# N3b3x/openballbot-rl

Hardware: AMD Instinct MI355X
Metric: env-steps/sec at 4096 envs per GPU (flat terrain, random actions) (higher is better)
Workload: dtype f64

## Files before the change

openballbot-rl_amd/ballbot_gym/_native.py:

```python
from __future__ import annotations

import ctypes as C
import os
from pathlib import Path

PKG = Path(__file__).resolve().parent
LIB_PATH = PKG / "_lib" / "libbb_mi355x.so"
CSRC = PKG.parent / "csrc"
INCLUDE = PKG.parent.parent / "include"

NQ, NV, NOBS, HF_N = 17, 15, 15, 293
DONE_TERMINATED, DONE_FAILURE, DONE_DIVERGED, DONE_OVERFLOW = 1, 2, 4, 8
NSTATS = 8
REWARD_DIRECTIONAL, REWARD_DISTANCE, REWARD_NONE = 0, 1, 2
DSBL_PASSIVE, DSBL_GRAVITY = 32, 64


class NativeLibraryError(RuntimeError):
    pass


class BBParams(C.Structure):
    _fields_ = [
        ("max_ep_steps", C.c_int),
        ("max_allowed_tilt", C.c_float),
        ("max_wheel_velocity", C.c_float),
        ("reward_scale", C.c_float),
        ("action_reg_coef", C.c_float),
        ("survival_bonus", C.c_float),
        ("target_dir", C.c_float * 2),
        ("reward_kind", C.c_int),
        ("goal", C.c_float * 2),
        ("goal_scale", C.c_float),
        ("n_terrains", C.c_int),
        ("seed", C.c_uint64),
        ("fp64", C.c_int),
        ("solver_maxiter", C.c_int),
        ("solver_tol", C.c_double),
        ("opt_timestep", C.c_double),
        ("opt_disableflags", C.c_int),
    ]


class PerlinCfg(C.Structure):
    _fields_ = [
        ("scale", C.c_double),
        ("octaves", C.c_int),
        ("persistence", C.c_float),
        ("lacunarity", C.c_float),
        ("amplitude", C.c_double),
    ]


class PPOMlpArgs(C.Structure):
    _fields_ = [(name, C.c_void_p) for name in ("params", "grad", "exp_avg", "exp_avg_sq")] + [
        ("n_params", C.c_int64),
        ("offsets", C.c_int32 * 21),
    ] + [(name, C.c_void_p) for name in ("obs", "actions", "old_logp", "advantages", "returns", "perm",
                                         "mb_counter", "row_counter", "log", "clip", "lr", "step", "coef")] + [
        ("B", C.c_int32),
        ("normalize_advantage", C.c_int32),
        ("obs_dim", C.c_int32),
        ("obs_direct", C.c_int32),
        ("ent_coef", C.c_float),
        ("vf_coef", C.c_float),
    ] + [(name, C.c_double) for name in ("beta1", "beta2", "eps", "weight_decay", "max_grad_norm")] + [
        ("workspace", C.c_void_p),
        ("workspace_bytes", C.c_int64),
        ("phase", C.c_int32),
        ("adv_stats", C.c_void_p),
    ]


class RolloutArgs(C.Structure):
    _fields_ = [
        ("params", C.c_void_p),
        ("offsets", C.c_int32 * 21),
        ("n_params", C.c_int64),
        ("noise", C.c_void_p),
        ("n_steps", C.c_int32),
    ] + [(name, C.c_void_p) for name in ("obs", "last_starts", "ep_ret", "ep_len", "buf_obs", "buf_actions",
                                         "buf_values", "buf_log_prob", "buf_rewards", "buf_starts", "ep_r_out",
                                         "ep_l_out", "buf_terminal_obs", "buf_flags")]


class ViewCfg(C.Structure):
    _fields_ = [
        ("height", C.c_int),
        ("width", C.c_int),
        ("fovy_deg", C.c_float),
        ("azimuth_deg", C.c_float),
        ("elevation_deg", C.c_float),
        ("distance", C.c_float),
        ("lookat_offset", C.c_float * 3),
    ]


ENCODER_FIELDS = ("conv1_w", "conv1_b", "bn1_w", "bn1_b", "bn1_mean", "bn1_var", "bn1_count",
                  "conv2_w", "conv2_b", "bn2_w", "bn2_b", "bn2_mean", "bn2_var", "bn2_count",
                  "fc_w", "fc_b", "bn3_w", "bn3_b", "bn3_mean", "bn3_var", "bn3_count")


class EncoderParams(C.Structure):
    _fields_ = [(name, C.c_void_p) for name in ENCODER_FIELDS]


EXPORTS = [
    "bb_abi_version", "bb_last_error", "bb_default_params", "bb_create", "bb_destroy", "bb_set_hfield",
    "bb_assign_terrain", "bb_reset", "bb_step", "bb_get_state", "bb_set_state", "bb_forward", "bb_get_stats",
    "bb_get_offsets", "bb_get_config", "bb_time_kernel", "bb_kernel_ms", "bb_generate_perlin", "bb_get_hfield",
    "bb_gae", "bb_render_depth", "bb_ppo_loss", "bb_adamw_clip", "bb_ppo_mlp_workspace_bytes", "bb_ppo_mlp_step",
    "bb_ppo_mlp_act", "bb_rollout_track", "bb_depth_encoder_workspace_bytes", "bb_depth_encoder",
    "bb_set_terrain_stream", "bb_get_env_terrain", "bb_kernel_times", "bb_step_multi", "bb_rollout",
    "bb_set_terrain_rng", "bb_get_terrain_rng", "bb_pair_counters", "bb_pair_env_times", "bb_check",
    "bb_reward_terms", "bb_default_view", "bb_render_view", "bb_render_rgbd",
]

ABI_VERSION = 21

_lib = None


HIP_SOURCES = ("bb_kernels.hip", "bb_pair.hip", "bb_terrain.hip", "bb_rollout.hip", "bb_render.hip", "bb_view.hip",
               "bb_rgbd.hip", "bb_ppo.hip", "bb_mlp.hip", "bb_encoder.hip", "bb_episode_log.hip")
SOURCE_FLAGS = {"bb_pair.hip": ["-mllvm", "-disable-machine-licm"]}


def build(force: bool = False, verbose: bool = False) -> Path:
    import subprocess
    from concurrent.futures import ThreadPoolExecutor

    srcs = list(CSRC.glob("*.h")) + list(CSRC.glob("*.hip")) + list(INCLUDE.glob("*.h"))
    if LIB_PATH.exists() and not force and all(LIB_PATH.stat().st_mtime >= s.stat().st_mtime for s in srcs):
        return LIB_PATH
    obj_dir = LIB_PATH.parent / "obj"
    obj_dir.mkdir(parents=True, exist_ok=True)
    flags = ["--offload-arch=gfx950", "-O3", "-std=c++17", "-fPIC"]
    jobs = []
    for f in HIP_SOURCES:
        obj = obj_dir / (f[:-4] + ".o")
        jobs.append((["hipcc", *flags, *SOURCE_FLAGS.get(f, []), "-c", "-o", str(obj), str(CSRC / f)], obj))
    if verbose:
        for cmd, _ in jobs:
            print(" ".join(cmd))

    def run(job):
        return subprocess.run(job[0], capture_output=True, text=True)

    workers = max(1, min(len(jobs), os.cpu_count() or 1, 16))
    with ThreadPoolExecutor(workers) as ex:
        results = list(ex.map(run, jobs))
    for (cmd, _), r in zip(jobs, results):
        if r.returncode != 0:
            raise subprocess.CalledProcessError(r.returncode, cmd, r.stdout, r.stderr + "\n" + " ".join(cmd))
    tmp = LIB_PATH.with_suffix(".so.tmp")
    link = ["hipcc", "--offload-arch=gfx950", "-shared", "-fPIC", "-o", str(tmp), *[str(o) for _, o in jobs]]
    if verbose:
        print(" ".join(link))
    subprocess.run(link, check=True)
    os.replace(tmp, LIB_PATH)
    return LIB_PATH


def lib():
    global _lib
    if _lib is None:
        _lib = _load(LIB_PATH)
    return _lib


def use_diagnostic_library(path) -> None:
    global _lib
    _lib = _load(Path(path))


def _load(path: Path):
    if not path.exists():
        raise NativeLibraryError(
            f"HIP library {path} not found; run __graft_entry__.build() (hipcc --offload-arch=gfx950)")
    try:
        L = C.CDLL(str(path))
    except OSError as e:
        raise NativeLibraryError(f"cannot load {path}: {e}") from e
    vp, fp, dp = C.c_void_p, C.POINTER(C.c_float), C.POINTER(C.c_double)
    L.bb_abi_version.restype = C.c_int
    L.bb_last_error.argtypes = [C.c_char_p, C.c_int]
    L.bb_default_params.argtypes = [C.POINTER(BBParams)]
    L.bb_default_params.restype = None
    L.bb_create.argtypes = [C.c_int, C.c_int, C.POINTER(BBParams), C.POINTER(vp)]
    L.bb_destroy.argtypes = [vp]
    L.bb_set_hfield.argtypes = [vp, C.c_int, fp, C.c_float]
    L.bb_assign_terrain.argtypes = [vp, vp, vp]
    L.bb_reset.argtypes = [vp, vp, vp, vp]
    L.bb_step.argtypes = [vp, vp, vp, vp, vp, vp, vp, C.c_int, vp]
    L.bb_step_multi.argtypes = [vp, vp, C.c_int, vp, vp, vp, vp, vp, C.c_int, vp]
    L.bb_rollout.argtypes = [vp, C.POINTER(RolloutArgs), vp]
    L.bb_reward_terms.argtypes = [vp, vp, vp, C.c_int, vp, C.c_int64, vp, vp]
    L.bb_get_state.argtypes = [vp, dp, dp, dp, C.POINTER(C.c_int32)]
    L.bb_set_state.argtypes = [vp, dp, dp, dp, C.POINTER(C.c_int32)]
    L.bb_forward.argtypes = [vp, dp, dp, C.POINTER(C.c_int32)]
    L.bb_get_stats.argtypes = [vp, C.POINTER(C.c_int64), C.c_int]
    L.bb_pair_counters.argtypes = [vp, C.POINTER(C.c_int64), C.c_int]
    L.bb_pair_env_times.argtypes = [vp, C.POINTER(C.c_uint64)]
    L.bb_check.argtypes = [vp, vp]
    L.bb_set_terrain_stream.argtypes = [vp, C.POINTER(C.c_int32), C.c_int, C.c_int, C.POINTER(C.c_int32)]
    L.bb_set_terrain_rng.argtypes = [vp, C.POINTER(C.c_uint64), C.POINTER(C.c_int32)]
    L.bb_get_terrain_rng.argtypes = [vp, C.POINTER(C.c_uint64), C.POINTER(C.c_int32)]
    L.bb_get_env_terrain.argtypes = [vp, C.POINTER(C.c_int32), C.POINTER(C.c_int32)]
    L.bb_get_offsets.argtypes = [vp, fp]
    L.bb_get_config.argtypes = [vp, C.POINTER(C.c_int32)]
    L.bb_time_kernel.argtypes = [vp, C.c_int]
    L.bb_generate_perlin.argtypes = [vp, C.c_int, C.c_int, C.POINTER(C.c_int32), C.POINTER(PerlinCfg), C.c_float]
    L.bb_get_hfield.argtypes = [vp, C.c_int, fp]
    L.bb_render_depth.argtypes = [vp, vp, vp, C.c_int, C.c_int, C.c_int, C.c_int, vp]
    L.bb_default_view.argtypes = [C.POINTER(ViewCfg)]
    L.bb_default_view.restype = None
    L.bb_render_view.argtypes = [vp, vp, C.c_int, C.POINTER(ViewCfg), vp, vp, vp]
    L.bb_render_rgbd.argtypes = [vp, vp, vp, vp, C.c_int, C.c_int, C.c_int, C.c_int, vp]
    L.bb_ppo_loss.argtypes = [vp] * 8 + [C.c_int, C.c_int, C.c_float, C.c_float, vp, vp, vp, vp]
    L.bb_adamw_clip.argtypes = [vp, vp, vp, vp, C.c_int64, vp, vp, vp] + [C.c_double] * 5 + [vp]
    L.bb_gae.argtypes = [vp, vp, vp, vp, vp, C.c_int, C.c_int, C.c_double, C.c_double, vp, vp, vp]
    L.bb_ppo_mlp_workspace_bytes.argtypes = [C.c_int, C.POINTER(C.c_int64)]
    L.bb_ppo_mlp_step.argtypes = [C.POINTER(PPOMlpArgs), vp]
    L.bb_ppo_mlp_act.argtypes = [vp, C.POINTER(C.c_int32), C.c_int64, vp, C.c_int, vp, C.c_int, vp, vp, vp, vp, vp,
                                 vp]
    L.bb_rollout_track.argtypes = [vp, vp, C.c_int, C.c_int] + [vp] * 8
    L.bb_depth_encoder_workspace_bytes.argtypes = [C.c_int64, C.POINTER(C.c_int64)]
    L.bb_depth_encoder.argtypes = [C.POINTER(EncoderParams), vp, C.c_int64, vp, C.c_int64, C.c_int, C.c_int, C.c_int,
                                   C.c_float, C.c_float, vp, C.c_int64, vp, C.c_int64, vp]
    L.bb_kernel_ms.argtypes = [vp, C.POINTER(C.c_double), C.POINTER(C.c_int32)]
    L.bb_kernel_times.argtypes = [vp, C.POINTER(C.c_double), C.POINTER(C.c_int32)]
    for name in [n for n in EXPORTS if n not in ("bb_default_params", "bb_default_view", "bb_abi_version")]:
        getattr(L, name).restype = C.c_int
    if L.bb_abi_version() != ABI_VERSION:
        raise NativeLibraryError("ABI version mismatch")
    return L


def last_error() -> str:
    buf = C.create_string_buffer(512)
    lib().bb_last_error(buf, 512)
    return buf.value.decode()


def check(rc: int, what: str) -> None:
    if rc != 0:
        raise RuntimeError(f"{what} failed: {last_error()}")


def default_params() -> BBParams:
    p = BBParams()
    lib().bb_default_params(C.byref(p))
    return p
```

openballbot-rl_amd/csrc/bb_kernels.hip:

```cpp
#if defined(BB_FP_CONTRACT_OFF)
#pragma clang fp contract(off)
#elif !defined(BB_FP_CONTRACT_FAST)
#pragma clang fp contract(on)
#endif
#include <hip/hip_runtime.h>

#include <stdarg.h>
#include <stdio.h>
#include <stdlib.h>
#include <string.h>
#include <algorithm>
#include <climits>
#include <vector>

#include "../../include/ballbot_mi355x.h"
#include "bb_model.h"
#include "bb_step.h"
#include "bb_terrain.h"
#include "bb_rollout.h"
#include "bb_episode_log.h"
#include "bb_render.h"
#include "bb_view.h"
#include "bb_rgbd.h"
#include "bb_ppo.h"
#include "bb_mlp.h"
#include "bb_encoder.h"
#include "bb_pairmap.h"

using namespace bb;

#ifdef BB_PHASE_CLOCKS
namespace bb { __device__ unsigned long long bb_phase_cycles[100]; }
#endif

namespace {

constexpr int WAVE = 64;
constexpr int TEAM = 16;
char g_err[512] = "";

int fail(const char* fmt, ...) {
  va_list ap;
  va_start(ap, fmt);
  vsnprintf(g_err, sizeof g_err, fmt, ap);
  va_end(ap);
  return -1;
}
#define HIPCHK(x)                                                                   \
  do {                                                                              \
    hipError_t e_ = (x);                                                            \
    if (e_ != hipSuccess) return fail("%s: %s", #x, hipGetErrorString(e_));         \
  } while (0)

template <typename T>
__host__ __device__ constexpr size_t work_stride() { return (sizeof(EnvWork<T>) + 15) / 16 * 16; }
template <typename T>
size_t lds_bytes(int epw) { return work_stride<T>() * epw; }
template <typename T>
__device__ __forceinline__ EnvWork<T>& team_work(unsigned char* smem, int team) {
  return *reinterpret_cast<EnvWork<T>*>(smem + size_t(team) * work_stride<T>());
}

struct TerrainSrc {
  const int* tstream;
  const int* env_stream;
  int tlen;
  unsigned long long* rng;
  const int* seed_slot;
};

struct Dev {
  int n;
  void* qpos;
  void* qvel;
  void* warm;
  int* steps;
  int* terrain;
  int* pending_terrain;
  int* episodes;
  const struct TerrainSrc* tsrc;
  int* tseed;
  const float* bank;
  const float* size_z;
  const float* offset;
  const float* hmax;
  int n_terrains;
  unsigned long long* stats;
  int* slow_list;
  int* slow_count;
  int* park;
  int* fast_envs;
  int* pred_envs;
  uint8_t* pred_mark;
  void* body_spill;
  void* hand;
  int* perm;
  unsigned long long* ring;
  int* rctr;
  int ring_len;
  unsigned long long* pair_env;
  unsigned long long* pair_busy;
  unsigned long long* cost;
  int* fault;
};

template <typename T>
__device__ __forceinline__ T* body_spill_of(const Dev& d, int e) {
  return reinterpret_cast<T*>(d.body_spill) + size_t(e) * ((MAXB - MAXB_LDS) * NBF);
}

template <typename V>
__device__ __forceinline__ V ld_coh(const V* p) {
  return __hip_atomic_load(p, __ATOMIC_RELAXED, __HIP_MEMORY_SCOPE_AGENT);
}
template <typename V>
__device__ __forceinline__ void st_coh(V* p, V v) {
  __hip_atomic_store(p, v, __ATOMIC_RELAXED, __HIP_MEMORY_SCOPE_AGENT);
}
__device__ __forceinline__ void stores_done() { asm volatile("s_waitcnt vmcnt(0)" ::: "memory"); }

template <typename T, bool COH = false>
__device__ __forceinline__ void load_state(const Dev& d, int e, T* q, T* v, T* w, int& step) {
  const T* Q = (const T*)d.qpos;
  const T* V = (const T*)d.qvel;
  const T* W = (const T*)d.warm;
  if constexpr (COH) {
#pragma unroll
    for (int i = 0; i < NQ; i++) q[i] = ld_coh(Q + i * d.n + e);
#pragma unroll
    for (int i = 0; i < NV; i++) { v[i] = ld_coh(V + i * d.n + e); w[i] = ld_coh(W + i * d.n + e); }
    step = ld_coh(d.steps + e);
  } else {
#pragma unroll
    for (int i = 0; i < NQ; i++) q[i] = Q[i * d.n + e];
#pragma unroll
    for (int i = 0; i < NV; i++) { v[i] = V[i * d.n + e]; w[i] = W[i * d.n + e]; }
    step = d.steps[e];
  }
}
template <typename T, bool COH = false>
__device__ __forceinline__ void store_state(const Dev& d, int e, const T* q, const T* v, const T* w, int step) {
  asm volatile("" : "+v"(e));
  T* Q = (T*)d.qpos;
  T* V = (T*)d.qvel;
  T* W = (T*)d.warm;
  if constexpr (COH) {
#pragma unroll
    for (int i = 0; i < NQ; i++) st_coh(Q + i * d.n + e, q[i]);
#pragma unroll
    for (int i = 0; i < NV; i++) { st_coh(V + i * d.n + e, v[i]); st_coh(W + i * d.n + e, w[i]); }
    st_coh(d.steps + e, step);
  } else {
#pragma unroll
    for (int i = 0; i < NQ; i++) Q[i * d.n + e] = q[i];
#pragma unroll
    for (int i = 0; i < NV; i++) { V[i * d.n + e] = v[i]; W[i * d.n + e] = w[i]; }
    d.steps[e] = step;
  }
}

struct Pcg64 {
  unsigned long long sh, sl, ih, il, buf;
};
constexpr int TERRAIN_SEEDS = 10000;

__device__ __forceinline__ unsigned long long pcg64_next64(Pcg64& g) {
  constexpr unsigned long long MH = 0x2360ED051FC65DA4ull, ML = 0x4385DF649FCCF645ull;
  const unsigned long long lo = g.sl * ML;
  unsigned long long hi = __umul64hi(g.sl, ML) + g.sl * MH + g.sh * ML;
  const unsigned long long lo2 = lo + g.il;
  hi += g.ih + (lo2 < lo ? 1ull : 0ull);
  g.sl = lo2;
  g.sh = hi;
  const unsigned rot = unsigned(hi >> 58);
  const unsigned long long x = hi ^ lo2;
  return (x >> rot) | (x << ((64u - rot) & 63u));
}
__device__ __forceinline__ unsigned pcg64_next32(Pcg64& g) {
  if (g.buf >> 32) {
    const unsigned u = unsigned(g.buf);
    g.buf = u;
    return u;
  }
  const unsigned long long x = pcg64_next64(g);
  g.buf = (1ull << 32) | (x >> 32);
  return unsigned(x);
}
__device__ __forceinline__ int pcg64_terrain_seed(Pcg64& g) {
  constexpr unsigned EXCL = TERRAIN_SEEDS;
  unsigned long long m = (unsigned long long)pcg64_next32(g) * EXCL;
  unsigned left = unsigned(m);
  if (left < EXCL) {
    constexpr unsigned THRESHOLD = (0xFFFFFFFFu - (EXCL - 1u)) % EXCL;
    while (left < THRESHOLD) {
      m = (unsigned long long)pcg64_next32(g) * EXCL;
      left = unsigned(m);
    }
  }
  return int(m >> 32);
}

__device__ __forceinline__ int next_terrain(const Dev& d, int e) {
  const int pin = d.pending_terrain[e];
  if (pin >= 0) return pin;
  const TerrainSrc src = *d.tsrc;
  if (src.rng) {
    const size_t n = size_t(d.n);
    unsigned long long* rng = src.rng;
    Pcg64 g{ld_coh(rng + e), ld_coh(rng + n + e), ld_coh(rng + 2 * n + e), ld_coh(rng + 3 * n + e),
            ld_coh(rng + 4 * n + e)};
    const int s = pcg64_terrain_seed(g);
    st_coh(rng + e, g.sh); st_coh(rng + n + e, g.sl); st_coh(rng + 4 * n + e, g.buf);
    st_coh(d.episodes + e, ld_coh(d.episodes + e) + 1);
    st_coh(d.tseed + e, s);
    int slot = src.seed_slot ? src.seed_slot[s] : s;
    if (unsigned(slot) >= unsigned(d.n_terrains)) {
      atomicAdd(&d.stats[5], 1ull);
      slot = s % d.n_terrains;
    }
    return slot;
  }
  if (!src.tstream) return 0;
  int k = ld_coh(d.episodes + e);
  st_coh(d.episodes + e, k + 1);
  if (k >= src.tlen) {
    atomicAdd(&d.stats[5], 1ull);
    k %= src.tlen;
  }
  const int st = src.env_stream ? src.env_stream[e] : 0;
  return src.tstream[size_t(st) * src.tlen + k];
}

template <typename T>
__device__ __forceinline__ void reset_lane(const ModelT<T>& m, const Dev& d, int e, T* q, T* v, T* w, int& step) {
  const int tid = next_terrain(d, e);
  d.terrain[e] = tid;
  reset_state(m, T(d.offset[tid]), q, v, w);
  step = 0;
}

template <typename T, bool BODY>
__global__ __launch_bounds__(64) void step_kernel(ModelT<T> mg, EnvCfg cfg, Dev d, const float* __restrict__ act,
                                                  float* __restrict__ obs, float* __restrict__ rew,
                                                  uint8_t* __restrict__ done, float* __restrict__ tobs,
                                                  float* __restrict__ pos2d, int auto_reset, int L, int epw,
                                                  const int* __restrict__ elist, const int* __restrict__ ecount) {
  extern __shared__ __align__(16) unsigned char smem[];
  const int nwg = int(gridDim.x), b = int(blockIdx.x);
  int g;
  const int ecnt = elist ? min(*ecount, d.n) : 0;
  if (elist) {
    const int na = (ecnt + epw - 1) / epw, nb = (na + 7) & ~7;
    if (nb > nwg) {
      g = b;
    } else {
      if (b >= nb) return;
      g = (b & 7) * (nb >> 3) + (b >> 3);
    }
    if (g >= na) return;
  } else {
    g = (nwg & 7) ? b : (b & 7) * (nwg >> 3) + (b >> 3);
  }
  __shared__ ModelT<T> ms;
  if (threadIdx.x == 0) ms = mg;
  __syncthreads();
  const ModelT<T>& m = ms;
  const Team tm{L, int(threadIdx.x) & (L - 1)};
  const int team = threadIdx.x / L;
  if (team >= epw) return;
  int e = g * epw + team;
  if (elist) {
    if (e >= ecnt) return;
    e = elist[e];
  }
  if (unsigned(e) >= unsigned(d.n)) return;
  const bool lead = tm.tl == 0;
#ifdef BB_PHASE_CLOCKS
  const unsigned long long t_env0 = clock64();
#endif
  EnvWork<T>& W = team_work<T>(smem, team);
#ifdef BB_PHASE_CLOCKS
  if (lead) W.dbg_nb = 0;
#endif
  if (BODY && lead) W.bspill = body_spill_of<T>(d, e);
  T* q = W.qn;
  T* v = W.vn;
  T* w = W.wn;
  int step;
  load_state(d, e, q, v, w, step);
  float a[3] = {act[3 * e], act[3 * e + 1], act[3 * e + 2]};
  const int tid = d.terrain[e];
  const float* hf = d.bank + size_t(tid) * (HF_N * HF_N);
  float o[15], r, p2[2];
  int iters = 0;
  const TerrainRef<T> tr{hf, T(d.size_z[tid]), T(d.hmax[tid]) * T(d.size_z[tid])};
  int fl = env_step<T, BODY, !BODY>(m, cfg, q, v, w, step, a, tr, W, o, r, p2, &iters, tm);
  if (!BODY && (fl & F_SLOWPATH)) {
    if (lead) {
      const int at = atomicAdd(d.slow_count + 2, 1);
      if (at < d.n) d.slow_list[at] = e;
    }
    return;
  }
  if (!lead) return;
  if (BODY) atomicAdd(&d.stats[3], 1ull);
  if (tobs) {
#pragma unroll
    for (int i = 0; i < 15; i++) tobs[15 * e + i] = o[i];
  }
  if (pos2d) { pos2d[2 * e] = p2[0]; pos2d[2 * e + 1] = p2[1]; }
  const bool reset = auto_reset && (fl & F_TERMINATED);
  if (reset) {
    reset_lane(m, d, e, q, v, w, step);
#pragma unroll
    for (int i = 0; i < 15; i++) o[i] = 0.f;
  }
#pragma unroll
  for (int i = 0; i < 15; i++) obs[15 * e + i] = o[i];
  rew[e] = r;
  done[e] = uint8_t(fl);
  store_state(d, e, q, v, w, step);
  if (reset) atomicAdd(&d.stats[0], 1ull);
  if (fl & F_DIVERGED) atomicAdd(&d.stats[1], 1ull);
  if (fl & F_OVERFLOW) atomicAdd(&d.stats[2], 1ull);
  if (fl & F_SPILL) atomicAdd(&d.stats[6], 1ull);
  atomicAdd(&d.stats[4], (unsigned long long)iters);
#ifdef BB_PHASE_CLOCKS
  {
    const unsigned long long dt = clock64() - t_env0;
    atomicMax(&bb_phase_cycles[BODY ? 34 : 37], dt);
    atomicAdd(&bb_phase_cycles[BODY ? 35 : 38], dt);
    atomicAdd(&bb_phase_cycles[BODY ? 36 : 39], 1ull);
    if (BODY) {
      const int bin = int(dt >> 20) < 9 ? int(dt >> 20) : 9;
      atomicAdd(&bb_phase_cycles[40 + bin], 1ull);
      atomicAdd(&bb_phase_cycles[50 + bin], (unsigned long long)W.dbg_nb);
      atomicAdd(&bb_phase_cycles[60 + bin], (unsigned long long)iters);
      atomicMax(&bb_phase_cycles[70 + bin], (unsigned long long)W.dbg_nb);
    }
  }
#endif
}

#ifndef BB_MULTI_MODE
#define BB_MULTI_MODE 1
#endif
template <typename T>
__device__
#if BB_MULTI_MODE == 0
__noinline__
#else
__forceinline__
#endif
int full_env_step(const ModelT<T>& m, const EnvCfg& cfg, T* q, T* v, T* w, int& step,
                                          const float* a, const TerrainRef<T>& tr, EnvWork<T>& W, float* o,
                                          float& r, float* p2, int* iters, const Team& tm) {
  return env_step<T, true>(m, cfg, q, v, w, step, a, tr, W, o, r, p2, iters, tm);
}

constexpr int F_PARKED = 1 << 17;

constexpr int SC_ROUTE = 8, SC_TOUCHED = 10, ROUTE_PARK = 1;

#ifndef BB_OUT_SKIP
#define BB_OUT_SKIP 0
#endif
template <typename V>
__device__ __forceinline__ void out_st(V* p, V v) {
#ifdef BB_OUT_NT
  __builtin_nontemporal_store(v, p);
#else
  *p = v;
#endif
}

template <typename T, bool HO = true, bool FULLONLY = false, bool FUSE = false>
__device__ __forceinline__ int team_step(const ModelT<T>& m, const EnvCfg& cfg, const Dev& d, int e, int& tid,
                                         T* q, T* v, T* w, int& step, T* bk, const float* a, EnvWork<T>& W, float* o,
                                         float& r, float* tobs_row, float* p2_row, int auto_reset, const Team& tm,
                                         unsigned* cnt, bool full = false) {
  const int L = tm.L;
  const bool lead = tm.tl == 0;
  if constexpr (!FULLONLY) {
    team_sync();
    for (int i = tm.tl; i < NQ + 2 * NV; i += L) bk[i] = q[i];
    team_sync();
  }
  const float* hf = d.bank + size_t(tid) * (HF_N * HF_N);
  float p2[2];
  int iters = 0;
  const TerrainRef<T> tr{hf, T(d.size_z[tid]), T(d.hmax[tid]) * T(d.size_z[tid])};
  const int step0 = step;
  int fl;
#if BB_MULTI_MODE == 2
  fl = F_SLOWPATH;
#else
  if constexpr (FULLONLY) fl = F_SLOWPATH;
  else fl = full ? F_SLOWPATH : env_step<T, false, FUSE>(m, cfg, q, v, w, step, a, tr, W, o, r, p2, &iters, tm);
#endif
  const bool slow = (fl & F_SLOWPATH) != 0;
#if BB_MULTI_MODE == 3
  if (false) {
#else
  if (slow) {
#endif
    if constexpr (!FULLONLY) {
      team_sync();
      for (int i = tm.tl; i < NQ + 2 * NV; i += L) q[i] = bk[i];
      team_sync();
      step = step0;
    }
    if constexpr (!HO) return F_PARKED;
    else fl = full_env_step<T>(m, cfg, q, v, w, step, a, tr, W, o, r, p2, &iters, tm);
  }
  const bool reset = auto_reset && (fl & F_TERMINATED);
  if (lead) {
    cnt[3] += slow;
    if (tobs_row && !(BB_OUT_SKIP & 8)) {
#pragma unroll
      for (int i = 0; i < 15; i++) out_st(tobs_row + i, o[i]);
    }
    if (p2_row && !(BB_OUT_SKIP & 16)) { out_st(p2_row, p2[0]); out_st(p2_row + 1, p2[1]); }
    if (reset) {
      tid = next_terrain(d, e);
      st_coh(d.terrain + e, tid);
    }
  }
  if (reset) {
    tid = __shfl(tid, team_shift_of(L));
    team_sync();
    reset_state(m, T(d.offset[tid]), q, v, w);
    step = 0;
#pragma unroll
    for (int i = 0; i < 15; i++) o[i] = 0.f;
  }
  if (lead) {
    cnt[0] += reset;
    cnt[1] += (fl & F_DIVERGED) != 0;
    cnt[2] += (fl & F_OVERFLOW) != 0;
    cnt[6] += (fl & F_SPILL) != 0;
    cnt[4] += unsigned(iters);
  }
  return fl;
}

__device__ __forceinline__ void counts_clear(unsigned* cnt) {
#pragma unroll
  for (int i = 0; i < 8; i++) cnt[i] = 0u;
}
__device__ __forceinline__ void counts_flush(const Dev& d, const unsigned* cnt) {
#pragma unroll
  for (int i = 0; i < 8; i++)
    if (i != 5 && cnt[i]) atomicAdd(&d.stats[i], (unsigned long long)cnt[i]);
}

#ifdef BB_WPE1
#define BB_WPE __attribute__((amdgpu_waves_per_eu(1, 1)))
#else
#define BB_WPE
#endif
template <typename T, bool HO>
__global__ BB_WPE __launch_bounds__(64) void multi_step_kernel(ModelT<T> mg, EnvCfg cfg, Dev d, const float* __restrict__ act,
                                                        int K, float* __restrict__ obs, float* __restrict__ rew,
                                                        uint8_t* __restrict__ done, float* __restrict__ tobs,
                                                        float* __restrict__ pos2d, int auto_reset, int L, int epw,
                                                        int* __restrict__ park, const int* __restrict__ gate) {
  if (gate && *gate != ROUTE_PARK) return;
  extern __shared__ __align__(16) unsigned char smem[];
  const int nwg = int(gridDim.x), b = int(blockIdx.x);
  const int g = (nwg & 7) ? b : (b & 7) * (nwg >> 3) + (b >> 3);
  __shared__ ModelT<T> ms;
  if (threadIdx.x == 0) ms = mg;
  __syncthreads();
  const ModelT<T>& m = ms;
  const Team tm{L, int(threadIdx.x) & (L - 1)};
  const int team = threadIdx.x / L;
  if (team >= epw) return;
  const int e = g * epw + team;
  if (unsigned(e) >= unsigned(d.n)) return;
  int k0 = 0;
  if (HO && park) {
    k0 = park[e];
    if (k0 >= K) return;
  }
  const bool lead = tm.tl == 0;
  EnvWork<T>& W = team_work<T>(smem, team);
  T* bk = reinterpret_cast<T*>(smem + size_t(epw) * work_stride<T>()) + team * (NQ + 2 * NV);
  __shared__ unsigned s_cnt[WAVE / TEAM][8];
  unsigned* cnt = s_cnt[team];
  if (lead) {
    W.bspill = body_spill_of<T>(d, e);
    counts_clear(cnt);
  }
  T* q = W.qn;
  T* v = W.vn;
  T* w = W.wn;
  int step;
  load_state(d, e, q, v, w, step);
  int tid = d.terrain[e];
  const size_t n = size_t(d.n);
  int parked = K;
#pragma unroll 1
  for (int k = k0; k < K; k++) {
    const size_t row = size_t(k) * n + e;
    const float* ak = act + 3 * row;
    const float a[3] = {ak[0], ak[1], ak[2]};
    float o[15], r;
    const int fl = team_step<T, HO, false, !HO>(m, cfg, d, e, tid, q, v, w, step, bk, a, W, o, r,
                                                tobs ? tobs + 15 * row : nullptr,
                                                pos2d ? pos2d + 2 * row : nullptr, auto_reset, tm, cnt);
    if (!HO && (fl & F_PARKED)) {
      parked = k;
      break;
    }
    if (lead) {
#pragma unroll
      for (int i = 0; i < 15; i++) obs[15 * row + i] = o[i];
      rew[row] = r;
      done[row] = uint8_t(fl);
    }
  }
  team_sync();
  if (lead) {
    store_state(d, e, q, v, w, step);
    counts_flush(d, cnt);
    if (!HO) park[e] = parked;
    if (!HO && gate && parked < K) atomicAdd(d.slow_count + SC_TOUCHED, 1);
  }
}

__device__ __forceinline__ float leaky_f(float z) { return z > 0.f ? z : z * 0.01f; }
__device__ __forceinline__ void team_policy(const float* __restrict__ P, const int* __restrict__ off, const float* x,
                                            float* hA, float* hB, const Team& tm, float mu[3], float& val) {
  constexpr int HIDN = 128, IN = 15;
  const int u0 = 4 * tm.tl;
#pragma unroll 1
  for (int tr = 0; tr < 2; tr++) {
    const int wb = tr ? MLP_VF_W0 : MLP_PI_W0, bb_ = tr ? MLP_VF_B0 : MLP_PI_B0;
    float* hin = hA;
    float* hout = hB;
#pragma unroll 1
    for (int l = 0; l < 4; l++) {
      const float* WT = P + off[wb + l];
      const float* bl = P + off[bb_ + l];
      const float* in = l ? hin : x;
      const int K = l ? HIDN : IN;
      float4 a0 = *reinterpret_cast<const float4*>(bl + u0);
      float4 a1 = *reinterpret_cast<const float4*>(bl + 64 + u0);
#ifdef BB_POLICY_UNROLL
#pragma unroll BB_POLICY_UNROLL
#else
#pragma unroll 8
#endif
      for (int k = 0; k < K; k++) {
        const float hk = in[k];
        const float4 w0 = *reinterpret_cast<const float4*>(WT + k * HIDN + u0);
        const float4 w1 = *reinterpret_cast<const float4*>(WT + k * HIDN + 64 + u0);
        a0.x = fmaf(hk, w0.x, a0.x); a0.y = fmaf(hk, w0.y, a0.y);
        a0.z = fmaf(hk, w0.z, a0.z); a0.w = fmaf(hk, w0.w, a0.w);
        a1.x = fmaf(hk, w1.x, a1.x); a1.y = fmaf(hk, w1.y, a1.y);
        a1.z = fmaf(hk, w1.z, a1.z); a1.w = fmaf(hk, w1.w, a1.w);
      }
      float* out = l ? hout : hin;
      *reinterpret_cast<float4*>(out + u0) = make_float4(leaky_f(a0.x), leaky_f(a0.y), leaky_f(a0.z), leaky_f(a0.w));
      *reinterpret_cast<float4*>(out + 64 + u0) =
          make_float4(leaky_f(a1.x), leaky_f(a1.y), leaky_f(a1.z), leaky_f(a1.w));
      team_sync();
      if (l) { float* t_ = hin; hin = hout; hout = t_; }
    }
    const float4 h0 = *reinterpret_cast<const float4*>(hin + u0);
    const float4 h1 = *reinterpret_cast<const float4*>(hin + 64 + u0);
    auto dot8 = [&](const float* w) {
      const float4 w0 = *reinterpret_cast<const float4*>(w + u0);
      const float4 w1 = *reinterpret_cast<const float4*>(w + 64 + u0);
      float s = 0.f;
      s = fmaf(h0.x, w0.x, s); s = fmaf(h0.y, w0.y, s); s = fmaf(h0.z, w0.z, s); s = fmaf(h0.w, w0.w, s);
      s = fmaf(h1.x, w1.x, s); s = fmaf(h1.y, w1.y, s); s = fmaf(h1.z, w1.z, s); s = fmaf(h1.w, w1.w, s);
      return s;
    };
    if (tr == 0) {
      const float* Wa = P + off[MLP_WA];
#pragma unroll
      for (int c = 0; c < 3; c++) mu[c] = team_sum(tm, dot8(Wa + c * HIDN)) + P[off[MLP_BA] + c];
    } else {
      val = team_sum(tm, dot8(P + off[MLP_WV])) + P[off[MLP_BV]];
    }
    team_sync();
  }
}

struct RolloutCore {
  const float* P;
  int off[MLP_NSLOTS];
  const float* noise;
  int T;
  float* obs;
  uint8_t* last_starts;
  double* ep_ret;
  long long* ep_len;
  float* b_obs;
  float* b_act;
  float* b_val;
  float* b_logp;
  float* b_rew;
  uint8_t* b_starts;
  double* ep_r;
  long long* ep_l;
};
struct RolloutDev : RolloutCore {
  float* b_tobs;
  uint8_t* b_flags;
};
struct RolloutLog {
  float* tobs;
  uint8_t* flags;
};
__device__ __forceinline__ RolloutLog rollout_log_of() { return RolloutLog{nullptr, nullptr}; }
__device__ __forceinline__ RolloutLog rollout_log_of(const RolloutLog& l) { return l; }

template <typename T, bool HO, typename... LG>
__global__ __launch_bounds__(64) void rollout_kernel(ModelT<T> mg, EnvCfg cfg, Dev d, RolloutCore ro, int L, int epw,
                                                     int* __restrict__ park, LG... lg_arg) {
  constexpr bool LOG = sizeof...(LG) != 0;
  const RolloutLog lg = rollout_log_of(lg_arg...);
  extern __shared__ __align__(16) unsigned char smem[];
  const int nwg = int(gridDim.x), b = int(blockIdx.x);
  const int g = (nwg & 7) ? b : (b & 7) * (nwg >> 3) + (b >> 3);
  __shared__ ModelT<T> ms;
  if (threadIdx.x == 0) ms = mg;
  __syncthreads();
  const ModelT<T>& m = ms;
  const Team tm{L, int(threadIdx.x) & (L - 1)};
  const int team = threadIdx.x / L;
  if (team >= epw) return;
  const int e = g * epw + team;
  if (unsigned(e) >= unsigned(d.n)) return;
  int t0 = 0;
  if (HO && park) {
    t0 = park[e];
    if (t0 >= ro.T) return;
  }
  const bool lead = tm.tl == 0;
  EnvWork<T>& W = team_work<T>(smem, team);
  T* bk = reinterpret_cast<T*>(smem + size_t(epw) * work_stride<T>()) + team * (NQ + 2 * NV);
  static_assert(offsetof(EnvWork<T>, bc) == offsetof(EnvWork<T>, g) + sizeof(W.g) &&
                    sizeof(W.g) + sizeof(W.bc) >= 272 * sizeof(float),
                "policy scratch must fit in EnvWork::g + bc");
  float* pol = reinterpret_cast<float*>(W.g);
  float* x = pol;
  float* hA = pol + 16;
  float* hB = pol + 144;
  __shared__ unsigned s_cnt[WAVE / TEAM][8];
  unsigned* cnt = s_cnt[team];
  if (lead) {
    W.bspill = body_spill_of<T>(d, e);
    counts_clear(cnt);
  }
  T* q = W.qn;
  T* v = W.vn;
  T* w = W.wn;
  int step;
  load_state(d, e, q, v, w, step);
  int tid = d.terrain[e];
  const size_t n = size_t(d.n);
  float o[15];
#pragma unroll
  for (int i = 0; i < 15; i++) o[i] = ro.obs[15 * size_t(e) + i];
  uint8_t start = ro.last_starts[e];
  double ret = ro.ep_ret[e];
  long long len = ro.ep_len[e];
  const float* ls = ro.P + ro.off[MLP_LS];
  constexpr float HL2PI = 0.91893853320467274f;
  int parked = ro.T;
#pragma unroll 1
  for (int t = t0; t < ro.T; t++) {
    const size_t row = size_t(t) * n + e;
    team_sync();
    if (tm.tl < 15) x[tm.tl] = o[tm.tl];
    team_sync();
    float mu[3] = {0.f, 0.f, 0.f}, val = 0.f;
#ifndef BB_ROLLOUT_NO_POLICY
    team_policy(ro.P, ro.off, x, hA, hB, tm, mu, val);
#endif
    float a[3], ac[3], lp = 0.f;
#pragma unroll
    for (int j = 0; j < 3; j++) {
      const float ls_j = ls[j];
      a[j] = __fadd_rn(mu[j], __fmul_rn(ro.noise[3 * row + j], expf(ls_j)));
      const float z = __fmul_rn(__fsub_rn(a[j], mu[j]), expf(-ls_j));
      lp += -0.5f * z * z - ls_j - 0.5f * (2.f * HL2PI);
      ac[j] = fminf(fmaxf(a[j], -1.f), 1.f);
    }
    if (lead) {
#pragma unroll
      for (int i = 0; i < 15; i++) ro.b_obs[15 * row + i] = o[i];
#pragma unroll
      for (int j = 0; j < 3; j++) ro.b_act[3 * row + j] = a[j];
      ro.b_val[row] = val;
      ro.b_logp[row] = lp;
      ro.b_starts[row] = start;
    }
    float r, o_prev[15];
    if (!HO) {
#pragma unroll
      for (int i = 0; i < 15; i++) o_prev[i] = o[i];
    }
    const int fl = team_step<T, HO>(m, cfg, d, e, tid, q, v, w, step, bk, ac, W, o, r,
                                    LOG ? lg.tobs + 15 * row : nullptr, nullptr, 1, tm, cnt);
    if (!HO && (fl & F_PARKED)) {
#pragma unroll
      for (int i = 0; i < 15; i++) o[i] = o_prev[i];
      parked = t;
      break;
    }
    const bool dn = (fl & F_TERMINATED) != 0;
    ret += double(r);
    len += 1;
    if (lead) {
      ro.b_rew[row] = r;
      ro.ep_r[row] = dn ? ret : __builtin_nan("");
      ro.ep_l[row] = dn ? len : 0;
      if constexpr (LOG) lg.flags[row] = uint8_t(fl);
    }
    ret = dn ? 0.0 : ret;
    len = dn ? 0 : len;
    start = dn ? 1 : 0;
  }
  team_sync();
  if (lead) {
    store_state(d, e, q, v, w, step);
    counts_flush(d, cnt);
    if (!HO) park[e] = parked;
#pragma unroll
    for (int i = 0; i < 15; i++) ro.obs[15 * size_t(e) + i] = o[i];
    ro.last_starts[e] = start;
    ro.ep_ret[e] = ret;
    ro.ep_len[e] = len;
  }
}

template <typename T>
__global__ __launch_bounds__(64) void reset_kernel(ModelT<T> m, Dev d, const uint8_t* mask, float* obs) {
  const int e = blockIdx.x * WAVE + threadIdx.x;
  if (!mask && e == 0 && d.fault) __hip_atomic_store(d.fault, 0, __ATOMIC_RELAXED, __HIP_MEMORY_SCOPE_SYSTEM);
  if (e >= d.n) return;
  if (mask && !mask[e]) return;
  T q[NQ], v[NV], w[NV];
  int step;
  reset_lane(m, d, e, q, v, w, step);
  store_state(d, e, q, v, w, step);
  if (obs) {
#pragma unroll
    for (int i = 0; i < 15; i++) obs[15 * e + i] = 0.f;
  }
}

template <typename T>
__global__ __launch_bounds__(64) void forward_kernel(ModelT<T> mg, Dev d, const double* ctrl, double* qacc, int* ncon,
                                                     int L, int epw) {
  extern __shared__ __align__(16) unsigned char smem[];
  __shared__ ModelT<T> ms;
  if (threadIdx.x == 0) ms = mg;
  __syncthreads();
  const ModelT<T>& m = ms;
  const Team tm{L, int(threadIdx.x) & (L - 1)};
  const int team = threadIdx.x / L;
  if (team >= epw) return;
  const int e = blockIdx.x * epw + team;
  if (e >= d.n) return;
  EnvWork<T>& W = team_work<T>(smem, team);
  if (tm.tl == 0) W.bspill = body_spill_of<T>(d, e);
  T q[NQ], v[NV], w[NV], c[3];
  int step;
  load_state(d, e, q, v, w, step);
  for (int i = 0; i < 3; i++) c[i] = T(ctrl[3 * e + i]);
  const int tid = d.terrain[e];
  StageOut<T> so;
// ... 2032 lines not shown
```

openballbot-rl_amd/csrc/bb_physics.h:

```cpp
#pragma once

#include <hip/hip_runtime.h>
#include <math.h>
#include <stdint.h>

#define BB_HD __host__ __device__ __forceinline__

namespace bb {

constexpr int NQ = 17, NV = 15, NU = 3;
constexpr int HF_N = 293;
constexpr int MAXG = 50;
constexpr int NH = NV * (NV + 1) / 2;
constexpr int NGF = 4;
constexpr int MAXPAIR = 50;
constexpr int MAXB = 3 + 6 * MAXPAIR;
constexpr int MAXB_LDS = 32;
constexpr int NBF = 8;
constexpr int GF_N = 0, GF_DIST = 3;
constexpr int BF_N = 0, BF_P = 3, BF_DIST = 6, BF_CODE = 7;

constexpr double IMPR_GRAD = 1e6;

template <typename T>
struct ModelT {
  T m0, h0[3], I0O[6];
  T mw, cw[3], Iw[6];
  T gz[3];
  T wq[3][4];
  T axis[3];
  T u[3][3];
  T jpos[3];
  T anchor[3];
  T wheel_r, wheel_hh, armature, damping;
  T mB, IB, ball_r, dz;
  T tower_c[3], tower_r, tower_hh;
  T stick_c[2][3], stick_a[2][3], stick_r, stick_hh;
  T iw_ball, iw_wheel[3];
  T iw_base, iw_cam[2];
  T K, Bd;
  T solimp[5];
  T fr_wheel[2];
  T h, grav;
  T hf_sx, hf_sy, hf_bottom;
  T scale, tol, ls_tol, step_rel2;
  int maxiter, ls_maxiter;
  T qpos0[NQ];
};

template <typename T> BB_HD T dot3(const T* a, const T* b) { return a[0] * b[0] + a[1] * b[1] + a[2] * b[2]; }
template <typename T> BB_HD void cross3(T* r, const T* a, const T* b) {
  T x = a[1] * b[2] - a[2] * b[1], y = a[2] * b[0] - a[0] * b[2], z = a[0] * b[1] - a[1] * b[0];
  r[0] = x; r[1] = y; r[2] = z;
}
template <typename T>
BB_HD T hinge_sel(int w, const T* x) {
  using U = typename std::conditional<sizeof(T) == 8, unsigned long long, unsigned int>::type;
  const U m0 = U(0) - U(w == 0), m1 = U(0) - U(w == 1), m2 = U(0) - U(w == 2);
  const U b = (__builtin_bit_cast(U, x[6]) & m0) | (__builtin_bit_cast(U, x[7]) & m1) | (__builtin_bit_cast(U, x[8]) & m2);
  return __builtin_bit_cast(T, b);
}

template <typename T> BB_HD void mv3(T* r, const T* M, const T* v) {
  T x = M[0] * v[0] + M[1] * v[1] + M[2] * v[2];
  T y = M[3] * v[0] + M[4] * v[1] + M[5] * v[2];
  T z = M[6] * v[0] + M[7] * v[1] + M[8] * v[2];
  r[0] = x; r[1] = y; r[2] = z;
}
template <typename T> BB_HD void mtv3(T* r, const T* M, const T* v) {
  T x = M[0] * v[0] + M[3] * v[1] + M[6] * v[2];
  T y = M[1] * v[0] + M[4] * v[1] + M[7] * v[2];
  T z = M[2] * v[0] + M[5] * v[1] + M[8] * v[2];
  r[0] = x; r[1] = y; r[2] = z;
}
template <typename T> BB_HD void mm3(T* r, const T* A, const T* B) {
  T t[9];
#pragma unroll
  for (int i = 0; i < 3; i++)
#pragma unroll
    for (int j = 0; j < 3; j++) t[3 * i + j] = A[3 * i] * B[j] + A[3 * i + 1] * B[3 + j] + A[3 * i + 2] * B[6 + j];
#pragma unroll
  for (int i = 0; i < 9; i++) r[i] = t[i];
}
template <typename T> BB_HD void symv(T* r, const T* S, const T* v) {
  T x = S[0] * v[0] + S[3] * v[1] + S[4] * v[2];
  T y = S[3] * v[0] + S[1] * v[1] + S[5] * v[2];
  T z = S[4] * v[0] + S[5] * v[1] + S[2] * v[2];
  r[0] = x; r[1] = y; r[2] = z;
}
template <typename T> BB_HD void sym_rot(T* out, const T* R, const T* S) {
  T F[9] = {S[0], S[3], S[4], S[3], S[1], S[5], S[4], S[5], S[2]};
  T A[9], B[9];
  mm3(A, R, F);
#pragma unroll
  for (int i = 0; i < 3; i++)
#pragma unroll
    for (int j = 0; j < 3; j++) B[3 * i + j] = A[3 * i] * R[3 * j] + A[3 * i + 1] * R[3 * j + 1] + A[3 * i + 2] * R[3 * j + 2];
  out[0] = B[0]; out[1] = B[4]; out[2] = B[8]; out[3] = B[1]; out[4] = B[2]; out[5] = B[5];
}
template <typename T> BB_HD T clampT(T x, T lo, T hi) { return x < lo ? lo : (x > hi ? hi : x); }
template <typename T> BB_HD T maxT(T a, T b) { return a > b ? a : b; }
template <typename T> BB_HD T rsqrtT(T x) {
#ifdef __HIP_DEVICE_COMPILE__
  return rsqrt(x);
#else
  return T(1) / sqrt(x);
#endif
}
template <typename T> BB_HD T minT(T a, T b) { return a < b ? a : b; }
template <typename T> BB_HD T rsqrt_ls(T x) {
#ifdef __HIP_DEVICE_COMPILE__
  if constexpr (sizeof(T) == 8) {
    const double r = __builtin_amdgcn_rsq(x);
    return r * fma(-0.5 * x * r, r, 1.5);
  } else {
    return __builtin_amdgcn_rsqf(x);
  }
#else
  return T(1) / sqrt(x);
#endif
}
template <typename T> BB_HD T div_ls(T a, T b) {
#ifdef __HIP_DEVICE_COMPILE__
  if constexpr (sizeof(T) == 8) {
    double r = __builtin_amdgcn_rcp(b);
    r = fma(r, fma(-b, r, 1.0), r);
    return a * r;
  } else {
    return a * __builtin_amdgcn_rcpf(b);
  }
#else
  return a / b;
#endif
}

template <typename T> BB_HD void qmul(T* r, const T* a, const T* b) {
  T w = a[0] * b[0] - a[1] * b[1] - a[2] * b[2] - a[3] * b[3];
  T x = a[0] * b[1] + a[1] * b[0] + a[2] * b[3] - a[3] * b[2];
  T y = a[0] * b[2] - a[1] * b[3] + a[2] * b[0] + a[3] * b[1];
  T z = a[0] * b[3] + a[1] * b[2] - a[2] * b[1] + a[3] * b[0];
  r[0] = w; r[1] = x; r[2] = y; r[3] = z;
}
template <typename T> BB_HD void qnormalize(T* q) {
  T n = sqrt(q[0] * q[0] + q[1] * q[1] + q[2] * q[2] + q[3] * q[3]);
  if (n < T(1e-15)) { q[0] = 1; q[1] = q[2] = q[3] = 0; return; }
  T inv = T(1) / n;
  q[0] *= inv; q[1] *= inv; q[2] *= inv; q[3] *= inv;
}
template <typename T> BB_HD void q2mat(T* m, const T* q) {
  T q00 = q[0] * q[0], q01 = q[0] * q[1], q02 = q[0] * q[2], q03 = q[0] * q[3];
  T q11 = q[1] * q[1], q12 = q[1] * q[2], q13 = q[1] * q[3];
  T q22 = q[2] * q[2], q23 = q[2] * q[3], q33 = q[3] * q[3];
  m[0] = q00 + q11 - q22 - q33; m[4] = q00 - q11 + q22 - q33; m[8] = q00 - q11 - q22 + q33;
  m[1] = 2 * (q12 - q03); m[2] = 2 * (q13 + q02); m[3] = 2 * (q12 + q03);
  m[5] = 2 * (q23 - q01); m[6] = 2 * (q13 - q02); m[7] = 2 * (q23 + q01);
}
template <typename T> BB_HD void quat_integrate(T* q, const T* w, T h) {
  T n = sqrt(dot3(w, w));
  T qr[4] = {1, 0, 0, 0};
  if (n >= T(1e-15)) {
    T ang = h * n, s = sin(ang * T(0.5)) / n;
    qr[0] = cos(ang * T(0.5)); qr[1] = w[0] * s; qr[2] = w[1] * s; qr[3] = w[2] * s;
  }
  qnormalize(q);
  qmul(q, q, qr);
}
template <typename T> BB_HD void integrate_pos(T* q, const T* v, T h) {
  q[0] += h * v[0]; q[1] += h * v[1]; q[2] += h * v[2];
  quat_integrate(q + 3, v + 3, h);
  q[7] += h * v[6]; q[8] += h * v[7]; q[9] += h * v[8];
  q[10] += h * v[9]; q[11] += h * v[10]; q[12] += h * v[11];
  quat_integrate(q + 13, v + 12, h);
}

constexpr BB_HD int hidx(int i, int j) { return i >= j ? i * (i + 1) / 2 + j : j * (j + 1) / 2 + i; }

template <typename T>
struct Kin {
  T Rb[9], RB[9];
  T pb[3], pB[3];
  T c[3];
  T wc[3][3];
  T Rw[3][9];
};

template <typename T>
BB_HD void kinematics_base(const ModelT<T>& m, const T* q, Kin<T>& k) {
  T qb[4] = {q[3], q[4], q[5], q[6]};
  qnormalize(qb);
  q2mat(k.Rb, qb);
  T qB[4] = {q[13], q[14], q[15], q[16]};
  qnormalize(qB);
  q2mat(k.RB, qB);
  k.pb[0] = q[0]; k.pb[1] = q[1]; k.pb[2] = q[2];
  k.pB[0] = q[10]; k.pB[1] = q[11]; k.pB[2] = q[12];
  k.c[0] = k.pB[0] + k.RB[2] * m.dz;
  k.c[1] = k.pB[1] + k.RB[5] * m.dz;
  k.c[2] = k.pB[2] + k.RB[8] * m.dz;
}

template <typename T>
BB_HD void kinematics_wheel(const ModelT<T>& m, const T* q, int w, Kin<T>& k) {
  T th = q[7 + w] - m.qpos0[7 + w];
  T s = sin(th * T(0.5)), cth = cos(th * T(0.5));
  T ql[4] = {cth, m.axis[0] * s, m.axis[1] * s, m.axis[2] * s};
  T qw[4];
  qmul(qw, m.wq[w], ql);
  qnormalize(qw);
  q2mat(k.Rw[w], qw);
  T d[3] = {m.cw[0] - m.jpos[0], m.cw[1] - m.jpos[1], m.cw[2] - m.jpos[2]};
  T t[3];
  mv3(t, k.Rw[w], d);
  k.wc[w][0] = m.anchor[0] + t[0];
  k.wc[w][1] = m.anchor[1] + t[1];
  k.wc[w][2] = m.anchor[2] + t[2];
}

template <typename T>
BB_HD void kinematics(const ModelT<T>& m, const T* q, Kin<T>& k) {
  kinematics_base(m, q, k);
#pragma unroll
  for (int w = 0; w < 3; w++) kinematics_wheel(m, q, w, k);
}

template <typename T>
struct Mass {
  T mt;
  T mr[3];
  T Mtr[9];
  T Mrr[6];
  T Mth[3][3];
  T Mrh[3][3];
  T Mhh[3];
  T mB;
  T MBtr[9];
  T MBrr[3];
};

template <typename T>
BB_HD void mass_wheel(const ModelT<T>& m, const Kin<T>& k, int w, Mass<T>& M, T* Iw, T* mrw, T* IOw) {
  const T* c = k.wc[w];
  sym_rot(Iw, k.Rw[w], m.Iw);
  mrw[0] = m.mw * c[0]; mrw[1] = m.mw * c[1]; mrw[2] = m.mw * c[2];
  T cc = dot3(c, c);
  IOw[0] = Iw[0] + m.mw * (cc - c[0] * c[0]);
  IOw[1] = Iw[1] + m.mw * (cc - c[1] * c[1]);
  IOw[2] = Iw[2] + m.mw * (cc - c[2] * c[2]);
  IOw[3] = Iw[3] - m.mw * c[0] * c[1];
  IOw[4] = Iw[4] - m.mw * c[0] * c[2];
  IOw[5] = Iw[5] - m.mw * c[1] * c[2];
  const T* u = m.u[w];
  T ca[3] = {c[0] - m.anchor[0], c[1] - m.anchor[1], c[2] - m.anchor[2]};
  T vc[3];
  cross3(vc, u, ca);
  T p[3] = {m.mw * vc[0], m.mw * vc[1], m.mw * vc[2]};
  T L[3], t[3];
  symv(L, Iw, u);
  T uIu = dot3(u, L);
  cross3(t, c, p);
  L[0] += t[0]; L[1] += t[1]; L[2] += t[2];
  mv3(M.Mth[w], k.Rb, p);
  M.Mrh[w][0] = L[0]; M.Mrh[w][1] = L[1]; M.Mrh[w][2] = L[2];
  M.Mhh[w] = uIu + m.mw * dot3(vc, vc) + m.armature;
}

template <typename T>
BB_HD void mass_finish(const ModelT<T>& m, const Kin<T>& k, Mass<T>& M, const T (*mrw)[3], const T (*IOw)[6]) {
  T mr[3] = {m.h0[0], m.h0[1], m.h0[2]};
  T IO[6] = {m.I0O[0], m.I0O[1], m.I0O[2], m.I0O[3], m.I0O[4], m.I0O[5]};
#pragma unroll
  for (int w = 0; w < 3; w++) {
#pragma unroll
    for (int i = 0; i < 3; i++) mr[i] += mrw[w][i];
#pragma unroll
    for (int i = 0; i < 6; i++) IO[i] += IOw[w][i];
  }
  M.mt = m.m0 + 3 * m.mw;
  M.mr[0] = mr[0]; M.mr[1] = mr[1]; M.mr[2] = mr[2];
  T S[9] = {0, mr[2], -mr[1], -mr[2], 0, mr[0], mr[1], -mr[0], 0};
  mm3(M.Mtr, k.Rb, S);
#pragma unroll
  for (int i = 0; i < 6; i++) M.Mrr[i] = IO[i];
  const T dz = m.dz;
  M.mB = m.mB;
  T SB[9] = {0, m.mB * dz, 0, -m.mB * dz, 0, 0, 0, 0, 0};
  mm3(M.MBtr, k.RB, SB);
  M.MBrr[0] = m.IB + m.mB * dz * dz;
  M.MBrr[1] = m.IB + m.mB * dz * dz;
  M.MBrr[2] = m.IB;
}

template <typename T>
BB_HD void build_mass(const ModelT<T>& m, const Kin<T>& k, Mass<T>& M, T (&Iw)[3][6]) {
  T mrw[3][3], IOw[3][6];
#pragma unroll
  for (int w = 0; w < 3; w++) mass_wheel(m, k, w, M, Iw[w], mrw[w], IOw[w]);
  mass_finish(m, k, M, mrw, IOw);
}

template <typename T>
BB_HD void mass_mul(const Mass<T>& M, const T* x, T* y) {
  T t[3], r[3];
  mv3(t, M.Mtr, x + 3);
  y[0] = M.mt * x[0] + t[0];
  y[1] = M.mt * x[1] + t[1];
  y[2] = M.mt * x[2] + t[2];
  mtv3(t, M.Mtr, x);
  symv(r, M.Mrr, x + 3);
  y[3] = t[0] + r[0]; y[4] = t[1] + r[1]; y[5] = t[2] + r[2];
#pragma unroll
  for (int w = 0; w < 3; w++) {
    T xh = x[6 + w];
#pragma unroll
    for (int i = 0; i < 3; i++) { y[i] += M.Mth[w][i] * xh; y[3 + i] += M.Mrh[w][i] * xh; }
    y[6 + w] = dot3(M.Mth[w], x) + dot3(M.Mrh[w], x + 3) + M.Mhh[w] * xh;
  }
  mv3(t, M.MBtr, x + 12);
  y[9] = M.mB * x[9] + t[0];
  y[10] = M.mB * x[10] + t[1];
  y[11] = M.mB * x[11] + t[2];
  mtv3(t, M.MBtr, x + 9);
  y[12] = t[0] + M.MBrr[0] * x[12];
  y[13] = t[1] + M.MBrr[1] * x[13];
  y[14] = t[2] + M.MBrr[2] * x[14];
}

template <typename T>
BB_HD void mass_dense(const Mass<T>& M, T* H) {
#pragma unroll
  for (int i = 0; i < NH; i++) H[i] = 0;
#pragma unroll
  for (int i = 0; i < 3; i++) {
    H[hidx(i, i)] = M.mt;
#pragma unroll
    for (int j = 0; j < 3; j++) H[hidx(3 + i, j)] = M.Mtr[3 * j + i];
  }
  H[hidx(3, 3)] = M.Mrr[0]; H[hidx(4, 4)] = M.Mrr[1]; H[hidx(5, 5)] = M.Mrr[2];
  H[hidx(4, 3)] = M.Mrr[3]; H[hidx(5, 3)] = M.Mrr[4]; H[hidx(5, 4)] = M.Mrr[5];
#pragma unroll
  for (int w = 0; w < 3; w++) {
#pragma unroll
    for (int j = 0; j < 3; j++) { H[hidx(6 + w, j)] = M.Mth[w][j]; H[hidx(6 + w, 3 + j)] = M.Mrh[w][j]; }
    H[hidx(6 + w, 6 + w)] = M.Mhh[w];
  }
#pragma unroll
  for (int i = 0; i < 3; i++) {
    H[hidx(9 + i, 9 + i)] = M.mB;
#pragma unroll
    for (int j = 0; j < 3; j++) H[hidx(12 + i, 9 + j)] = M.MBtr[3 * j + i];
    H[hidx(12 + i, 12 + i)] = M.MBrr[i];
  }
}

template <typename T>
BB_HD void inertia_apply(T m, const T* c, const T* Ic, const T* w, const T* v, T* L, T* p) {
  T t[3];
  cross3(t, w, c);
  p[0] = m * (v[0] + t[0]); p[1] = m * (v[1] + t[1]); p[2] = m * (v[2] + t[2]);
  symv(L, Ic, w);
  cross3(t, c, p);
  L[0] += t[0]; L[1] += t[1]; L[2] += t[2];
}
template <typename T>
BB_HD void body_force(T m, const T* c, const T* Ic, const T* Aw, const T* Av, const T* Vw, const T* Vv,
                      T* fa, T* fl) {
  T La[3], pa[3], Lv[3], pv[3], t[3];
  inertia_apply(m, c, Ic, Aw, Av, La, pa);
  inertia_apply(m, c, Ic, Vw, Vv, Lv, pv);
  cross3(t, Vw, Lv); fa[0] = La[0] + t[0]; fa[1] = La[1] + t[1]; fa[2] = La[2] + t[2];
  cross3(t, Vv, pv); fa[0] += t[0]; fa[1] += t[1]; fa[2] += t[2];
  cross3(t, Vw, pv); fl[0] = pa[0] + t[0]; fl[1] = pa[1] + t[1]; fl[2] = pa[2] + t[2];
}

template <typename T>
BB_HD void bias_base_motion(const ModelT<T>& m, const Kin<T>& k, const T* v, T* w0, T* vl, T* a0) {
  w0[0] = v[3]; w0[1] = v[4]; w0[2] = v[5];
  mtv3(vl, k.Rb, v);
  T t[3];
  cross3(t, vl, w0);
  a0[0] = m.grav * k.Rb[6] + t[0];
  a0[1] = m.grav * k.Rb[7] + t[1];
  a0[2] = m.grav * k.Rb[8] + t[2];
}

template <typename T>
BB_HD T bias_wheel(const ModelT<T>& m, const Kin<T>& k, const T* Iw, const T* v, int w, const T* w0, const T* vl,
                   const T* a0, T* fa, T* fl) {
  const T* u = m.u[w];
  T au[3];
  cross3(au, m.anchor, u);
  T qd = v[6 + w];
  T Vw[3] = {w0[0] + qd * u[0], w0[1] + qd * u[1], w0[2] + qd * u[2]};
  T Vv[3] = {vl[0] + qd * au[0], vl[1] + qd * au[1], vl[2] + qd * au[2]};
  T x1[3], x2[3], x3[3];
  cross3(x1, w0, u);
  cross3(x2, w0, au);
  cross3(x3, vl, u);
  T Aw[3] = {qd * x1[0], qd * x1[1], qd * x1[2]};
  T Av[3] = {a0[0] + qd * (x2[0] + x3[0]), a0[1] + qd * (x2[1] + x3[1]), a0[2] + qd * (x2[2] + x3[2])};
  body_force(m.mw, k.wc[w], Iw, Aw, Av, Vw, Vv, fa, fl);
  return dot3(u, fa) + dot3(au, fl);
}

template <typename T>
BB_HD void bias_finish(const ModelT<T>& m, const Kin<T>& k, const T* v, const T (*fw)[6], T* bias) {
  T w0[3], vl[3], a0[3], t[3];
  bias_base_motion(m, k, v, w0, vl, a0);
  const T zero[3] = {0, 0, 0};
  T Fa[3], Fl[3];
  {
    T c0[3] = {m.h0[0] / m.m0, m.h0[1] / m.m0, m.h0[2] / m.m0};
    T cc = dot3(c0, c0);
    T Ic[6] = {m.I0O[0] - m.m0 * (cc - c0[0] * c0[0]), m.I0O[1] - m.m0 * (cc - c0[1] * c0[1]),
               m.I0O[2] - m.m0 * (cc - c0[2] * c0[2]), m.I0O[3] + m.m0 * c0[0] * c0[1],
               m.I0O[4] + m.m0 * c0[0] * c0[2], m.I0O[5] + m.m0 * c0[1] * c0[2]};
    body_force(m.m0, c0, Ic, zero, a0, w0, vl, Fa, Fl);
  }
#pragma unroll
  for (int w = 0; w < 3; w++) {
    Fa[0] += fw[w][0]; Fa[1] += fw[w][1]; Fa[2] += fw[w][2];
    Fl[0] += fw[w][3]; Fl[1] += fw[w][4]; Fl[2] += fw[w][5];
  }
  mv3(bias, k.Rb, Fl);
  bias[3] = Fa[0]; bias[4] = Fa[1]; bias[5] = Fa[2];
  T wB[3] = {v[12], v[13], v[14]};
  T vB[3];
  mtv3(vB, k.RB, v + 9);
  cross3(t, vB, wB);
  T aB[3] = {m.grav * k.RB[6] + t[0], m.grav * k.RB[7] + t[1], m.grav * k.RB[8] + t[2]};
  T cB[3] = {0, 0, m.dz};
  T IcB[6] = {m.IB, m.IB, m.IB, 0, 0, 0};
  T fa[3], fl[3];
  body_force(m.mB, cB, IcB, zero, aB, wB, vB, fa, fl);
  mv3(bias + 9, k.RB, fl);
  bias[12] = fa[0]; bias[13] = fa[1]; bias[14] = fa[2];
}

template <typename T>
BB_HD void bias_forces(const ModelT<T>& m, const Kin<T>& k, const T (&Iw)[3][6], const T* v, T* bias) {
  T w0[3], vl[3], a0[3], fw[3][6];
  bias_base_motion(m, k, v, w0, vl, a0);
#pragma unroll
  for (int w = 0; w < 3; w++) bias[6 + w] = bias_wheel(m, k, Iw[w], v, w, w0, vl, a0, fw[w], fw[w] + 3);
  bias_finish(m, k, v, fw, bias);
}

template <typename T>
BB_HD T impedance(const ModelT<T>& m, T pos) {
  T x = pos / m.solimp[2];
  if (x < 0) x = -x;
  if (x >= T(1) || x <= T(0)) return x >= T(1) ? m.solimp[1] : m.solimp[0];
  T y;
  const T mid = m.solimp[3];
  if (x <= mid) y = x * x / mid;
  else y = T(1) - (T(1) - x) * (T(1) - x) / (T(1) - mid);
  return m.solimp[0] + y * (m.solimp[1] - m.solimp[0]);
}

template <typename T>
BB_HD void frame_from_normal(const T* n, T* t1, T* t2) {
  T y[3] = {0, 0, 0};
  if (fabs(n[1]) < T(0.5)) y[1] = 1; else y[2] = 1;
  T d = dot3(n, y);
  t1[0] = y[0] - d * n[0]; t1[1] = y[1] - d * n[1]; t1[2] = y[2] - d * n[2];
  T inv = rsqrtT(dot3(t1, t1));
  t1[0] *= inv; t1[1] *= inv; t1[2] *= inv;
  cross3(t2, n, t1);
}

template <typename T>
BB_HD void cone_eval(const T* jar, T mu, T f1, T f2, const T* D, T* force, T* C) {
  T U0 = jar[0] * mu, U1 = jar[1] * f1, U2 = jar[2] * f2;
  T N = U0, Tn = sqrt(U1 * U1 + U2 * U2);
  if (N >= mu * Tn || (Tn <= 0 && N >= 0)) {
    force[0] = force[1] = force[2] = 0;
    if (C) { C[0] = C[1] = C[2] = C[3] = C[4] = C[5] = 0; }
  } else if (mu * N + Tn <= 0 || (Tn <= 0 && N < 0)) {
    force[0] = -D[0] * jar[0]; force[1] = -D[1] * jar[1]; force[2] = -D[2] * jar[2];
    if (C) { C[0] = D[0]; C[1] = D[1]; C[2] = D[2]; C[3] = C[4] = C[5] = 0; }
  } else {
    T Dm = D[0] / (mu * mu * (1 + mu * mu));
    T g = N - mu * Tn;
    T iT = T(1) / Tn;
    T gr[3] = {mu, -mu * f1 * U1 * iT, -mu * f2 * U2 * iT};
    T s = -Dm * g;
    force[0] = s * gr[0]; force[1] = s * gr[1]; force[2] = s * gr[2];
    if (C) {
      T k = Dm * g * (-mu) * iT;
      T iT2 = iT * iT;
      C[0] = Dm * gr[0] * gr[0];
      C[1] = Dm * gr[1] * gr[1] + k * f1 * f1 * (T(1) - U1 * U1 * iT2);
      C[2] = Dm * gr[2] * gr[2] + k * f2 * f2 * (T(1) - U2 * U2 * iT2);
      C[3] = Dm * gr[0] * gr[1];
      C[4] = Dm * gr[0] * gr[2];
      C[5] = Dm * gr[1] * gr[2] - k * f1 * f2 * U1 * U2 * iT2;
    }
  }
}

template <typename T>
struct WheelCon {
  T J[3][13];
  T aref[3], D[3];
};

BB_HD constexpr int wheel_col(int i, int w) { return i < 6 ? i : (i == 6 ? 6 + w : i + 2); }

template <typename T>
struct GStore {
  T* base;
  int stride;
  BB_HD T& at(int s, int f) const { return base[(s * NGF + f) * stride]; }
};

template <typename T>
BB_HD void wheel_contact(const ModelT<T>& m, const Kin<T>& k, const T* v, int w, WheelCon<T>& C) {
  T t[3], gp[3], ax[3], axl[3];
  mv3(t, k.Rb, k.wc[w]);
  gp[0] = k.pb[0] + t[0]; gp[1] = k.pb[1] + t[1]; gp[2] = k.pb[2] + t[2];
  mv3(axl, k.Rw[w], m.gz);
  mv3(ax, k.Rb, axl);
  T vec[3] = {k.c[0] - gp[0], k.c[1] - gp[1], k.c[2] - gp[2]};
  T x = clampT(dot3(ax, vec), -m.wheel_hh, m.wheel_hh);
  T dif[3] = {gp[0] + ax[0] * x - k.c[0], gp[1] + ax[1] * x - k.c[1], gp[2] + ax[2] * x - k.c[2]};
  T cd = sqrt(dot3(dif, dif));
  T dist = cd - m.ball_r - m.wheel_r;
  const T act = dist <= 0 ? T(1) : T(0);
  T n[3];
  if (cd > 0) { T ic = T(1) / cd; n[0] = dif[0] * ic; n[1] = dif[1] * ic; n[2] = dif[2] * ic; }
  else { n[0] = 1; n[1] = 0; n[2] = 0; }
  T dn = dot3(n, ax);
  T t1[3] = {ax[0] - dn * n[0], ax[1] - dn * n[1], ax[2] - dn * n[2]};
  T it1 = T(1) / sqrt(dot3(t1, t1));
  t1[0] *= it1; t1[1] *= it1; t1[2] *= it1;
  T t2[3];
  cross3(t2, n, t1);
  T pos[3];
  T sp = m.ball_r + dist * T(0.5);
  pos[0] = k.c[0] + n[0] * sp; pos[1] = k.c[1] + n[1] * sp; pos[2] = k.c[2] + n[2] * sp;
  T lb[3] = {pos[0] - k.pb[0], pos[1] - k.pb[1], pos[2] - k.pb[2]};
  mv3(t, k.Rb, m.anchor);
  T la[3] = {lb[0] - t[0], lb[1] - t[1], lb[2] - t[2]};
  T lB[3] = {pos[0] - k.pB[0], pos[1] - k.pB[1], pos[2] - k.pB[2]};
  T uw[3];
  mv3(uw, k.Rb, m.u[w]);
#pragma unroll
  for (int r = 0; r < 3; r++) {
    const T* d = r == 0 ? n : (r == 1 ? t1 : t2);
    T x1[3], br[3];
    C.J[r][0] = d[0]; C.J[r][1] = d[1]; C.J[r][2] = d[2];
    cross3(x1, lb, d);
    mtv3(br, k.Rb, x1);
    C.J[r][3] = br[0]; C.J[r][4] = br[1]; C.J[r][5] = br[2];
    cross3(x1, la, d);
    C.J[r][6] = dot3(uw, x1);
    C.J[r][7] = -d[0]; C.J[r][8] = -d[1]; C.J[r][9] = -d[2];
    cross3(x1, lB, d);
    mtv3(t, k.RB, x1);
    C.J[r][10] = -t[0]; C.J[r][11] = -t[1]; C.J[r][12] = -t[2];
  }
  T imp = clampT(impedance(m, dist), T(0.0001), T(0.9999));
  T tran = m.iw_ball + m.iw_wheel[w];
  T R0 = maxT(T(1e-15), (1 - imp) * tran / imp);
  T rr = m.fr_wheel[0] / m.fr_wheel[1];
  T R2 = R0 * rr * rr;
  C.D[0] = act / R0; C.D[1] = act / R0; C.D[2] = act / R2;
#pragma unroll
  for (int r = 0; r < 3; r++) {
    T vel = 0;
#pragma unroll
    for (int i = 0; i < 13; i++) vel += C.J[r][i] * v[wheel_col(i, w)];
    C.aref[r] = (C.D[0] > 0 ? T(1) : T(0)) * (-m.Bd * vel - (r == 0 ? m.K * imp * dist : T(0)));
  }
}

template <typename T>
BB_HD T wheel_row_mul(const WheelCon<T>& C, int w, int r, const T* x) {
  T acc = 0;
#pragma unroll
  for (int i = 0; i < 13; i++) acc += C.J[r][i] * x[wheel_col(i, w)];
  return acc;
}

template <typename T>
BB_HD void closest_pt_tri(T* res, const T* p, const T* a, const T* b, const T* c) {
  T ab[3] = {b[0] - a[0], b[1] - a[1], b[2] - a[2]};
  T ac[3] = {c[0] - a[0], c[1] - a[1], c[2] - a[2]};
  T ap[3] = {p[0] - a[0], p[1] - a[1], p[2] - a[2]};
  T d1 = dot3(ab, ap), d2 = dot3(ac, ap);
  if (d1 <= 0 && d2 <= 0) { res[0] = a[0]; res[1] = a[1]; res[2] = a[2]; return; }
  T bp[3] = {p[0] - b[0], p[1] - b[1], p[2] - b[2]};
  T d3 = dot3(ab, bp), d4 = dot3(ac, bp);
  if (d3 >= 0 && d4 <= d3) { res[0] = b[0]; res[1] = b[1]; res[2] = b[2]; return; }
  T vc = d1 * d4 - d3 * d2;
  if (vc <= 0 && d1 >= 0 && d3 <= 0) {
    T vv = d1 / (d1 - d3);
    res[0] = a[0] + vv * ab[0]; res[1] = a[1] + vv * ab[1]; res[2] = a[2] + vv * ab[2];
    return;
  }
  T cp[3] = {p[0] - c[0], p[1] - c[1], p[2] - c[2]};
  T d5 = dot3(ab, cp), d6 = dot3(ac, cp);
  if (d6 >= 0 && d5 <= d6) { res[0] = c[0]; res[1] = c[1]; res[2] = c[2]; return; }
  T vb = d5 * d2 - d1 * d6;
  if (vb <= 0 && d2 >= 0 && d6 <= 0) {
    T ww = d2 / (d2 - d6);
    res[0] = a[0] + ww * ac[0]; res[1] = a[1] + ww * ac[1]; res[2] = a[2] + ww * ac[2];
    return;
  }
  T va = d3 * d6 - d5 * d4;
  if (va <= 0 && (d4 - d3) >= 0 && (d5 - d6) >= 0) {
    T ww = (d4 - d3) / ((d4 - d3) + (d5 - d6));
    res[0] = b[0] + ww * (c[0] - b[0]); res[1] = b[1] + ww * (c[1] - b[1]); res[2] = b[2] + ww * (c[2] - b[2]);
    return;
  }
  T den = T(1) / (va + vb + vc), vv = vb * den, ww = vc * den;
  res[0] = a[0] + ab[0] * vv + ac[0] * ww;
  res[1] = a[1] + ab[1] * vv + ac[1] * ww;
  res[2] = a[2] + ab[2] * vv + ac[2] * ww;
}

template <typename T>
BB_HD bool sphere_prism(const T* c, T r, const T V[3][3], T zb, T* n, T* dist) {
  T zmax = maxT(V[0][2], maxT(V[1][2], V[2][2]));
  T q[3];
  if (c[2] >= zmax) {
    closest_pt_tri(q, c, V[0], V[1], V[2]);
  } else {
    T area = (V[1][0] - V[0][0]) * (V[2][1] - V[0][1]) - (V[2][0] - V[0][0]) * (V[1][1] - V[0][1]);
    T sg = area > 0 ? T(1) : T(-1);
    bool inside = c[2] >= zb;
    T edist[3], eo[3][2];
#pragma unroll
    for (int i = 0; i < 3; i++) {
      const T* P = V[i];
      const T* Q = V[(i + 1) % 3];
      T ex = Q[0] - P[0], ey = Q[1] - P[1];
      T cr = ex * (c[1] - P[1]) - ey * (c[0] - P[0]);
      if (cr * sg < 0) inside = false;
      T nx = ey * sg, ny = -ex * sg, nl = sqrt(nx * nx + ny * ny);
      eo[i][0] = nx / nl; eo[i][1] = ny / nl;
      edist[i] = fabs(cr) / nl;
    }
    T e1[3] = {V[1][0] - V[0][0], V[1][1] - V[0][1], V[1][2] - V[0][2]};
    T e2[3] = {V[2][0] - V[0][0], V[2][1] - V[0][1], V[2][2] - V[0][2]};
    T nt[3];
    cross3(nt, e1, e2);
    if (nt[2] < 0) { nt[0] = -nt[0]; nt[1] = -nt[1]; nt[2] = -nt[2]; }
    T inl = T(1) / sqrt(dot3(nt, nt));
    nt[0] *= inl; nt[1] *= inl; nt[2] *= inl;
    T dtop = dot3(nt, V[0]) - dot3(nt, c);
    if (inside && dtop >= 0) {
      T best = dtop;
      n[0] = nt[0]; n[1] = nt[1]; n[2] = nt[2];
      if (c[2] - zb < best) { best = c[2] - zb; n[0] = 0; n[1] = 0; n[2] = -1; }
#pragma unroll
      for (int i = 0; i < 3; i++)
        if (edist[i] < best) { best = edist[i]; n[0] = eo[i][0]; n[1] = eo[i][1]; n[2] = 0; }
      *dist = -best - r;
      return true;
    }
    T B[3][3] = {{V[0][0], V[0][1], zb}, {V[1][0], V[1][1], zb}, {V[2][0], V[2][1], zb}};
    T best = T(1e30);
#pragma unroll
    for (int f = 0; f < 8; f++) {
      const T* a;
      const T* b;
      const T* cc;
      switch (f) {
        case 0: a = V[0]; b = V[1]; cc = V[2]; break;
        case 1: a = B[0]; b = B[1]; cc = B[2]; break;
        case 2: a = V[0]; b = V[1]; cc = B[1]; break;
        case 3: a = V[0]; b = B[1]; cc = B[0]; break;
        case 4: a = V[1]; b = V[2]; cc = B[2]; break;
        case 5: a = V[1]; b = B[2]; cc = B[1]; break;
        case 6: a = V[2]; b = V[0]; cc = B[0]; break;
        default: a = V[2]; b = B[0]; cc = B[2]; break;
      }
      T qq[3];
      closest_pt_tri(qq, c, a, b, cc);
      T dd[3] = {c[0] - qq[0], c[1] - qq[1], c[2] - qq[2]};
      T d2 = dot3(dd, dd);
      if (d2 < best) { best = d2; q[0] = qq[0]; q[1] = qq[1]; q[2] = qq[2]; }
    }
  }
  T dd[3] = {c[0] - q[0], c[1] - q[1], c[2] - q[2]};
  T d = sqrt(dot3(dd, dd));
  if (d > r) return false;
  if (d > T(1e-12)) { T id = T(1) / d; n[0] = dd[0] * id; n[1] = dd[1] * id; n[2] = dd[2] * id; }
  else {
    T e1[3] = {V[1][0] - V[0][0], V[1][1] - V[0][1], V[1][2] - V[0][2]};
    T e2[3] = {V[2][0] - V[0][0], V[2][1] - V[0][1], V[2][2] - V[0][2]};
    cross3(n, e1, e2);
    if (n[2] < 0) { n[0] = -n[0]; n[1] = -n[1]; n[2] = -n[2]; }
    T inl = T(1) / sqrt(dot3(n, n));
    n[0] *= inl; n[1] *= inl; n[2] *= inl;
  }
  *dist = d - r;
  return true;
}

template <typename T>
BB_HD void ground_contact(const ModelT<T>& m, const T* gc, const T* RB, const T* v, T (&J)[3][6], T (&aref)[3],
                          T& D) {
  const T n[3] = {gc[GF_N], gc[GF_N + 1], gc[GF_N + 2]};
  const T dist = gc[GF_DIST];
  const T sp = m.ball_r + dist * T(0.5);
  const T lv[3] = {m.dz * RB[2] - n[0] * sp, m.dz * RB[5] - n[1] * sp, m.dz * RB[8] - n[2] * sp};
  T t1[3], t2[3];
  frame_from_normal(n, t1, t2);
  const T* F[3] = {n, t1, t2};
#pragma unroll
  for (int r = 0; r < 3; r++) {
    T x1[3], x2[3];
    cross3(x1, lv, F[r]);
    mtv3(x2, RB, x1);
#pragma unroll
    for (int i = 0; i < 3; i++) { J[r][i] = F[r][i]; J[r][3 + i] = x2[i]; }
  }
  const T imp = clampT(impedance(m, dist), T(0.0001), T(0.9999));
  D = minT(T(1e15), imp / ((1 - imp) * m.iw_ball));
#pragma unroll
  for (int r = 0; r < 3; r++) {
    const T vel = J[r][0] * v[9] + J[r][1] * v[10] + J[r][2] * v[11] + J[r][3] * v[12] + J[r][4] * v[13] +
                  J[r][5] * v[14];
    aref[r] = -m.Bd * vel - (r == 0 ? m.K * imp * dist : T(0));
  }
}

template <typename T>
struct Poses {
  T Rb[9], pb[3], RB[9], pB[3];
};

template <typename T>
struct BodyFrame {
  T F[3][3], db[3], dB[3], hw[3], aref[3], D, ball;
  int hinge;
};

template <typename T>
BB_HD void body_V(const BodyFrame<T>& b, const Poses<T>& P, const T* x, T (&V)[3]) {
  T om[3], wx[3];
  mv3(om, P.Rb, x + 3);
  cross3(wx, om, b.db);
  const T xh = b.hinge >= 0 ? hinge_sel(b.hinge, x) : T(0);
  T ob[3], bx[3];
  mv3(ob, P.RB, x + 12);
  cross3(bx, ob, b.dB);
#pragma unroll
  for (int i = 0; i < 3; i++) V[i] = x[i] + wx[i] + b.hw[i] * xh - b.ball * (x[9 + i] + bx[i]);
}

template <typename T>
BB_HD void body_frame(const ModelT<T>& m, const T* bc, const Poses<T>& P, const T* v, BodyFrame<T>& b) {
  const int code = int(bc[BF_CODE]);
  const int b1 = code >> 3, b2 = code & 7;
  const T n[3] = {bc[BF_N], bc[BF_N + 1], bc[BF_N + 2]};
  const T dist = bc[BF_DIST];
  T t1[3], t2[3];
  frame_from_normal(n, t1, t2);
#pragma unroll
  for (int i = 0; i < 3; i++) {
    b.F[0][i] = n[i]; b.F[1][i] = t1[i]; b.F[2][i] = t2[i];
    b.db[i] = bc[BF_P + i] - P.pb[i];
    b.dB[i] = bc[BF_P + i] - P.pB[i];
    b.hw[i] = 0;
  }
  b.hinge = (b2 >= 4 && b2 <= 6) ? b2 - 4 : -1;
  if (b.hinge >= 0) {
    T uw[3], t[3], da[3];
    mv3(uw, P.Rb, m.u[b.hinge]);
    mv3(t, P.Rb, m.anchor);
    da[0] = b.db[0] - t[0]; da[1] = b.db[1] - t[1]; da[2] = b.db[2] - t[2];
    cross3(b.hw, uw, da);
  }
  b.ball = b1 == 7 ? T(1) : T(0);
  const T iw2 = b2 == 1 ? m.iw_base : (b2 <= 3 ? m.iw_cam[b2 - 2] : m.iw_wheel[b2 - 4]);
  const T tran = iw2 + (b1 == 7 ? m.iw_ball : T(0));
  const T imp = clampT(impedance(m, dist), T(0.0001), T(0.9999));
  b.D = T(1) / maxT(T(1e-15), (1 - imp) * tran / imp);
  T V[3];
  body_V(b, P, v, V);
#pragma unroll
  for (int r = 0; r < 3; r++) b.aref[r] = -m.Bd * dot3(b.F[r], V) - (r == 0 ? m.K * imp * dist : T(0));
}

template <typename T>
BB_HD void body_ls_terms(const ModelT<T>& m, const T* bc, const Poses<T>& P, const T* v, const T* a, const T* s,
                         T (&c6)[6], T& D) {
  BodyFrame<T> b;
  body_frame(m, bc, P, v, b);
  T Va[3], Vs[3];
  body_V(b, P, a, Va);
  body_V(b, P, s, Vs);
#pragma unroll
  for (int r = 0; r < 3; r++) {
    c6[r] = dot3(b.F[r], Va) - b.aref[r];
    c6[3 + r] = dot3(b.F[r], Vs);
  }
  D = b.D;
}

template <typename T>
BB_HD int collide_ground(const ModelT<T>& m, const Kin<T>& k, const T* v, const float* hf, T size_z,
                         const GStore<T>& st, int* overflow) {
  const T r = m.ball_r;
  const T* c = k.c;
  const T sx = m.hf_sx, sy = m.hf_sy, zb = m.hf_bottom;
  T xmin = c[0] - r, xmax = c[0] + r, ymin = c[1] - r, ymax = c[1] + r, zmin = c[2] - r, zmax = c[2] + r;
  if (!(xmin <= sx && xmax >= -sx && ymin <= sy && ymax >= -sy && zmin <= size_z && zmax >= -zb)) return 0;
  const int N1 = HF_N - 1;
  int cmin = (int)floor((xmin + sx) / (2 * sx) * N1);
  int cmax = (int)ceil((xmax + sx) / (2 * sx) * N1);
  int rmin = (int)floor((ymin + sy) / (2 * sy) * N1);
  int rmax = (int)ceil((ymax + sy) / (2 * sy) * N1);
  cmin = cmin < 0 ? 0 : cmin;
  cmax = cmax > N1 ? N1 : cmax;
  rmin = rmin < 0 ? 0 : rmin;
  rmax = rmax > N1 ? N1 : rmax;
  const T dx = 2 * sx / N1, dy = 2 * sy / N1;
  (void)v;
  int ng = 0;
  for (int rr = rmin; rr < rmax; rr++) {
    T W[3][3] = {{0, 0, 0}, {0, 0, 0}, {0, 0, 0}};
    int nvert = 0;
    const T y0 = dy * rr - sy, y1 = dy * (rr + 1) - sy;
    for (int cc = cmin; cc <= cmax; cc++) {
      const T x = dx * cc - sx;
      const T z0 = T(hf[rr * HF_N + cc]) * size_z;
      const T z1 = T(hf[(rr + 1) * HF_N + cc]) * size_z;
#pragma unroll
      for (int i = 0; i < 2; i++) {
#pragma unroll
        for (int j = 0; j < 3; j++) { W[0][j] = W[1][j]; W[1][j] = W[2][j]; }
        W[2][0] = x; W[2][1] = i ? y1 : y0; W[2][2] = i ? z1 : z0;
        nvert++;
        if (nvert <= 2) continue;
        if (W[0][2] < zmin && W[1][2] < zmin && W[2][2] < zmin) continue;
        T bx0 = minT(W[0][0], minT(W[1][0], W[2][0])), bx1 = maxT(W[0][0], maxT(W[1][0], W[2][0]));
        T by0 = minT(W[0][1], minT(W[1][1], W[2][1])), by1 = maxT(W[0][1], maxT(W[1][1], W[2][1]));
        T ztop = maxT(W[0][2], maxT(W[1][2], W[2][2]));
        T ex = maxT(T(0), maxT(bx0 - c[0], c[0] - bx1));
        T ey = maxT(T(0), maxT(by0 - c[1], c[1] - by1));
        T ez = maxT(T(0), c[2] - ztop);
        if (ex * ex + ey * ey + ez * ez > r * r) continue;
        T nn[3], dist;
        if (!sphere_prism(c, r, W, -zb, nn, &dist)) continue;
        if (ng >= MAXG) { *overflow = 1; continue; }
#pragma unroll
        for (int i = 0; i < 3; i++) st.at(ng, GF_N + i) = nn[i];
        st.at(ng, GF_DIST) = dist;
        ng++;
      }
    }
  }
  return ng;
}

template <typename T> BB_HD T eps_of();
template <> BB_HD float eps_of<float>() { return 1.1920929e-7f; }
template <> BB_HD double eps_of<double>() { return 2.220446049250313e-16; }
template <typename T> BB_HD T pivot_eps();
template <> BB_HD float pivot_eps<float>() { return 1e-6f; }
template <> BB_HD double pivot_eps<double>() { return 1e-14; }

template <typename T>
BB_HD void chol_packed(T* H) {
// ... 36 lines not shown
```

openballbot-rl_amd/csrc/bb_step.h:

```cpp
#pragma once

#include "bb_team16.h"

namespace bb {

struct EnvCfg {
  int max_ep_steps;
  float max_allowed_tilt;
  float max_wheel_velocity;
  float reward_scale;
  float action_reg_coef;
  float survival_bonus;
  float target[2];
  int reward_kind;
  float goal[2], goal_scale;
};

template <typename T, bool BODY = true, bool FUSE = false>
BB_HD int forward(const ModelT<T>& m, const T* q, const T* v, const T* ctrl, T* acc, const TerrainRef<T>& tr,
                  EnvWork<T>& W, StageOut<T>* so, const Team& tm) {
  team_sync();
  if (v != W.vi) {
#pragma unroll
    for (int i = 0; i < NV; i++) W.vi[i] = v[i];
    team_sync();
  }
#if defined(BB_PHASE_CLOCKS) && defined(__HIP_DEVICE_COMPILE__)
  const unsigned long long f_t0 = clock64();
#endif
  Kin<T>& k = W.u.pre.k;
#ifdef __HIP_DEVICE_COMPILE__
  kinematics_base(m, q, k);
  if (tm.tl < 3) kinematics_wheel(m, q, tm.tl, k);
  team_sync();
#else
  kinematics(m, q, k);
#endif
  Mass<T>& M = W.M;
#ifdef __HIP_DEVICE_COMPILE__
  {
    T (*mrw)[3] = reinterpret_cast<T (*)[3]>(W.H);
    T (*IOw)[6] = reinterpret_cast<T (*)[6]>(W.H + 9);
    T (*fw)[6] = reinterpret_cast<T (*)[6]>(W.H + 27);
    static_assert(NH >= 45, "per-wheel terms do not fit W.H");
    if (tm.tl < 3) {
      const int w = tm.tl;
      mass_wheel(m, k, w, M, W.u.pre.Iw[w], mrw[w], IOw[w]);
      T w0[3], vl[3], a0[3];
      bias_base_motion(m, k, v, w0, vl, a0);
      const T qb = -bias_wheel(m, k, W.u.pre.Iw[w], v, w, w0, vl, a0, fw[w], fw[w] + 3);
      const T cw = w == 0 ? ctrl[0] : (w == 1 ? ctrl[1] : ctrl[2]);
      W.qfs[6 + w] = qb + (-m.damping * v[6 + w] + cw);
      wheel_contact(m, k, v, w, W.wc[w]);
    }
    team_sync();
    mass_finish(m, k, M, mrw, IOw);
    T qfs[NV];
    bias_finish(m, k, v, fw, qfs);
#pragma unroll
    for (int i = 0; i < NV; i++)
      if (i < 6 || i > 8) W.qfs[i] = -qfs[i];
    team_sync();
  }
#else
  build_mass(m, k, M, W.u.pre.Iw);
  {
    T qfs[NV];
    bias_forces(m, k, W.u.pre.Iw, v, qfs);
#pragma unroll
    for (int i = 0; i < NV; i++) qfs[i] = -qfs[i];
#pragma unroll
    for (int w = 0; w < 3; w++) qfs[6 + w] += -m.damping * v[6 + w] + ctrl[w];
#pragma unroll
    for (int i = 0; i < NV; i++) W.qfs[i] = qfs[i];
  }
#pragma unroll
  for (int w = 0; w < 3; w++) wheel_contact(m, k, v, w, W.wc[w]);
#endif
  const GStore<T> st{W.g, 1};
  int overflow = 0;
#if defined(BB_PHASE_CLOCKS) && defined(__HIP_DEVICE_COMPILE__)
  const unsigned long long f_t1 = clock64();
#endif
#ifdef __HIP_DEVICE_COMPILE__
  const int ng = tr.hf ? t16::collide_team(m, k, v, tr.hf, tr.size_z, W.g, &overflow, tm.tl) : 0;
  int nb = 0;
  if constexpr (BODY) {
#if defined(BB_PHASE_CLOCKS)
    const unsigned long long b_t0 = clock64();
#endif
    static_assert(sizeof(W.H) >= t16::CAND_CAP * sizeof(int), "candidate list does not fit W.H");
#ifdef BB_EXP_DUP_BODYCOL
    { int ov2 = 0; (void)t16::collide_body_team(m, k, tr.hf, tr.size_z, tr.hz, W.bc, W.bspill, &ov2, tm.tl,
                                                 reinterpret_cast<int*>(W.H)); }
    asm volatile("" ::: "memory");
#endif
    nb = t16::collide_body_team(m, k, tr.hf, tr.size_z, tr.hz, W.bc, W.bspill, &overflow, tm.tl,
                                reinterpret_cast<int*>(W.H));
#if defined(BB_PHASE_CLOCKS)
    if (tm.tl == 0) {
      atomicAdd(&bb_phase_cycles[12], 1ull);
      atomicAdd(&bb_phase_cycles[13], (unsigned long long)nb);
      atomicAdd(&bb_phase_cycles[14], clock64() - b_t0);
      W.dbg_nb += nb;
    }
#endif
  } else {
    if (t16::body_candidates(m, k, tr.hf, tr.size_z, tr.hz, tm.tl)) return -1;
  }
#else
  const int ng = tr.hf ? collide_ground(m, k, v, tr.hf, tr.size_z, st, &overflow) : 0;
#endif
#if defined(BB_PHASE_CLOCKS) && defined(__HIP_DEVICE_COMPILE__)
  if (tm.tl == 0) {
    const unsigned long long f_t2 = clock64();
    atomicAdd(&bb_phase_cycles[8], f_t1 - f_t0);
    atomicAdd(&bb_phase_cycles[9], f_t2 - f_t1);
    atomicAdd(&bb_phase_cycles[10], 1ull);
  }
#endif
#pragma unroll
  for (int i = 0; i < 9; i++) { W.P.Rb[i] = k.Rb[i]; W.P.RB[i] = k.RB[i]; }
#pragma unroll
  for (int i = 0; i < 3; i++) { W.P.pb[i] = k.pb[i]; W.P.pB[i] = k.pB[i]; }
  if (so) {
    T qb[4] = {q[3], q[4], q[5], q[6]};
    qnormalize(qb);
    so->quat_b[0] = qb[0]; so->quat_b[1] = qb[1]; so->quat_b[2] = qb[2]; so->quat_b[3] = qb[3];
    mv3(so->w_world, k.Rb, v + 3);
    T cl[3] = {M.mr[0] / M.mt, M.mr[1] / M.mt, M.mr[2] / M.mt}, cw[3], t[3];
    mv3(cw, k.Rb, cl);
    cross3(t, so->w_world, cw);
    so->v_com[0] = v[0] + t[0]; so->v_com[1] = v[1] + t[1]; so->v_com[2] = v[2] + t[2];
    so->pb[0] = q[0]; so->pb[1] = q[1]; so->pb[2] = q[2];
    so->ng = ng; so->overflow = overflow;
#ifdef __HIP_DEVICE_COMPILE__
    so->nb = nb;
#else
    so->nb = 0;
#endif
  }
  bool ok = true;
#pragma unroll
  for (int i = 0; i < NV; i++) ok = ok && isfinite(acc[i]);
  if (!ok) {
#pragma unroll
    for (int i = 0; i < NV; i++) acc[i] = 0;
  }
#ifdef __HIP_DEVICE_COMPILE__
  t16::mass_dense_team(W, tm.tl);
  team_sync();
  if constexpr (!BODY) t16::ground_setup(m, W, ng, tm.tl);

#if defined(BB_PHASE_CLOCKS)
  const unsigned long long s_t0 = clock64();
#endif
#ifdef BB_EXP_DUP_SOLVE_FULL
  if constexpr (BODY) {
    T acc2[NV];
#pragma unroll
    for (int i = 0; i < NV; i++) acc2[i] = acc[i];
    (void)t16::solve16<BODY, FUSE>(m, W, ng, nb, acc2, tm.tl);
    asm volatile("" ::: "memory");
    team_sync();
  }
#endif
  const int it = t16::solve16<BODY, FUSE>(m, W, ng, nb, acc, tm.tl);
#if defined(BB_PHASE_CLOCKS)
  if (BODY && tm.tl == 0) {
    atomicAdd(&bb_phase_cycles[15], clock64() - s_t0);
    atomicAdd(&bb_phase_cycles[20], (unsigned long long)it);
  }
  if (tm.tl == 0) {
    atomicMax(&bb_phase_cycles[21], (unsigned long long)it);
    atomicAdd(&bb_phase_cycles[22 + (it / 2 < 9 ? it / 2 : 9)], 1ull);
  }
#endif
#else
  const int it = solve_team(m, W, W.qfs, ng, acc, tm);
#endif
  if (so) so->iters = it;
  return it;
}

template <typename T>
BB_HD bool vec_bad(const T* x, int n) {
  bool bad = false;
#pragma unroll
  for (int i = 0; i < n; i++) bad = bad || !(fabs(x[i]) <= T(1e10));
  return bad;
}

template <typename T, bool BODY = true, bool FUSE = false>
BB_HD int rk4_step(const ModelT<T>& m, T* q, T* v, T* warm, T* ctrl, const TerrainRef<T>& tr,
                   EnvWork<T>& W, StageOut<T>& so, const Team& tm, bool* acc_reset) {
  const T h = m.h;
  T* q0 = W.q0;
  T* v0 = W.v0;
  T* vs = W.vs;
  T* as = W.as;
  team_sync();
#pragma unroll
  for (int i = 0; i < NQ; i++) q0[i] = q[i];
#pragma unroll
  for (int i = 0; i < NV; i++) v0[i] = v[i];
  int iters = 0;
#pragma unroll 1
  for (int stage = 0; stage < 4; stage++) {
    const T a = stage == 3 ? T(1) : T(0.5);
    {
      T qi[NQ], vi[NV];
#pragma unroll
      for (int i = 0; i < NQ; i++) qi[i] = q0[i];
      if (stage == 0) {
#pragma unroll
        for (int i = 0; i < NV; i++) vi[i] = v0[i];
      } else {
        T dv[NV];
#pragma unroll
        for (int i = 0; i < NV; i++) { dv[i] = a * W.vi[i]; vi[i] = v0[i] + h * a * warm[i]; }
        integrate_pos(qi, dv, h);
      }
      team_sync();
#pragma unroll
      for (int i = 0; i < NQ; i++) W.u.pre.qi[i] = qi[i];
#pragma unroll
      for (int i = 0; i < NV; i++) W.vi[i] = vi[i];
    }
    T acc[NV];
#pragma unroll
    for (int i = 0; i < NV; i++) acc[i] = warm[i];
    if (stage == 3) {
#pragma unroll
      for (int i = 0; i < NV; i++) acc[i] = 2 * warm[i] - W.k1[i];
    }
    const int fit = forward<T, BODY, FUSE>(m, W.u.pre.qi, W.vi, ctrl, acc, tr, W, stage == 3 ? &so : (StageOut<T>*)nullptr, tm);
    if (fit < 0) return -1;
    if (stage == 0 && !*acc_reset && team_any(tm, vec_bad(acc, NV))) {
      team_sync();
#pragma unroll
      for (int i = 0; i < NQ; i++) q0[i] = m.qpos0[i];
#pragma unroll
      for (int i = 0; i < NV; i++) { v0[i] = 0; warm[i] = 0; }
      ctrl[0] = ctrl[1] = ctrl[2] = 0;
      *acc_reset = true;
      iters += fit;
      stage = -1;
      continue;
    }
#pragma unroll
    for (int i = 0; i < NV; i++) warm[i] = acc[i];
    iters += fit;
#if defined(BB_SOLVE_STATS) && !defined(__HIP_DEVICE_COMPILE__)
    g_stage_iters[stage] = fit;
#endif
    const T b = (stage == 0 || stage == 3) ? T(1.0 / 6) : T(1.0 / 3);
    team_sync();
    if (stage == 0) {
#pragma unroll
      for (int i = 0; i < NV; i++) { vs[i] = b * W.vi[i]; as[i] = b * warm[i]; W.k1[i] = warm[i]; }
    } else {
#pragma unroll
      for (int i = 0; i < NV; i++) { vs[i] += b * W.vi[i]; as[i] += b * warm[i]; }
    }
  }
  team_sync();
#pragma unroll
  for (int i = 0; i < NV; i++) v[i] = v0[i] + h * as[i];
#pragma unroll
  for (int i = 0; i < NQ; i++) q[i] = q0[i];
  T vv[NV];
#pragma unroll
  for (int i = 0; i < NV; i++) vv[i] = vs[i];
  integrate_pos(q, vv, h);
  return iters;
}

template <typename T>
BB_HD void reset_state(const ModelT<T>& m, T offset, T* q, T* v, T* warm) {
#pragma unroll
  for (int i = 0; i < NQ; i++) q[i] = m.qpos0[i];
  q[2] += offset;
  q[12] += offset;
#pragma unroll
  for (int i = 0; i < NV; i++) { v[i] = 0; warm[i] = 0; }
}

template <typename T>
BB_HD void quat_to_rotvec(const T* q, T* rv) {
  T b = sqrt(q[1] * q[1] + q[2] * q[2] + q[3] * q[3]);
  if (fabs(b) <= T(1e-14) * fabs(q[0])) {
    rv[0] = q[0] < 0 ? T(2 * 3.14159265358979323846) : T(0);
    rv[1] = rv[2] = 0;
    return;
  }
  T f = 2 * atan2(b, q[0]) / b;
  rv[0] = f * q[1]; rv[1] = f * q[2]; rv[2] = f * q[3];
}

BB_HD float clipf(float x, float lo, float hi) { return x < lo ? lo : (x > hi ? hi : x); }

template <typename T>
BB_HD bool state_bad(const T* q, const T* v) {
  return vec_bad(q, NQ) || vec_bad(v, NV);
}

constexpr int F_TERMINATED = 1, F_FAILURE = 2, F_DIVERGED = 4, F_OVERFLOW = 8, F_SPILL = 1 << 9,
              F_SLOWPATH = 1 << 16;

template <typename T, bool BODY = true, bool FUSE = false>
BB_HD int env_step(const ModelT<T>& m, const EnvCfg& cfg, T* q, T* v, T* warm, int& step, const float* action,
                   const TerrainRef<T>& tr, EnvWork<T>& W, float* obs15, float& reward, float* pos2d,
                   int* iters, const Team& tm) {
  const float mwv = cfg.max_wheel_velocity;
  T ctrl[3];
#pragma unroll
  for (int i = 0; i < 3; i++) ctrl[i] = -T(clipf(action[i] * mwv, -mwv, mwv));
  if (vec_bad(ctrl, 3)) ctrl[0] = ctrl[1] = ctrl[2] = 0;
  int flags = 0;
  if (state_bad(q, v)) {
    reset_state(m, T(0), q, v, warm);
    ctrl[0] = ctrl[1] = ctrl[2] = 0;
    flags = F_DIVERGED;
  }
  StageOut<T>& so = W.so;
  bool acc_reset = false;
  int it = rk4_step<T, BODY, FUSE>(m, q, v, warm, ctrl, tr, W, so, tm, &acc_reset);
  if (it < 0) return F_SLOWPATH;
  if (iters) *iters = it;
  if (acc_reset) flags |= F_DIVERGED;
  if (so.overflow) flags |= F_OVERFLOW;
  if (so.nb > MAXB_LDS) flags |= F_SPILL;
  {
#pragma clang fp contract(off)
  T rv[3];
  quat_to_rotvec(so.quat_b, rv);
  float orient[3] = {float(rv[0]), float(rv[1]), float(rv[2])};
  float vel[3], angv[3], motor[3];
#pragma unroll
  for (int i = 0; i < 3; i++) {
    vel[i] = clipf(float(so.w_world[i]), -2.f, 2.f);
    angv[i] = clipf(float(so.v_com[i]), -2.f, 2.f);
    motor[i] = clipf(float(v[1 + i]) / mwv, -2.f, 2.f);
  }
#pragma unroll
  for (int i = 0; i < 3; i++) {
    obs15[i] = action[i]; obs15[3 + i] = angv[i]; obs15[6 + i] = motor[i];
    obs15[9 + i] = orient[i]; obs15[12 + i] = vel[i];
  }
  pos2d[0] = float(so.pb[0]);
  pos2d[1] = float(so.pb[1]);
  float r;
  if (cfg.reward_kind == 0) {
    r = (vel[0] * cfg.target[0] + vel[1] * cfg.target[1]) * cfg.reward_scale;
  } else if (cfg.reward_kind == 1) {
    float dx = cfg.goal[0] - pos2d[0], dy = cfg.goal[1] - pos2d[1];
    r = (-cfg.goal_scale * sqrtf(dx * dx + dy * dy)) * cfg.reward_scale;
  } else {
    r = 0.f;
  }
  float nrm = sqrtf(action[0] * action[0] + action[1] * action[1] + action[2] * action[2]);
  r = r + cfg.action_reg_coef * (nrm * nrm);
  step += 1;
  if (step >= cfg.max_ep_steps) flags |= F_TERMINATED;
  T rx = orient[0], ry = orient[1], rz = orient[2];
  T th = sqrt(rx * rx + ry * ry + rz * rz) * T(0.5);
  T sf = th > T(1e-14) ? sin(th) / th : T(1);
  T qw = th > T(1e-14) ? cos(th) : T(1);
  T qx = sf * rx * T(0.5), qy = sf * ry * T(0.5), qz = sf * rz * T(0.5);
  T nn = qw * qw + qx * qx + qy * qy + qz * qz;
  T R22 = T(1) - 2 * (qx * qx + qy * qy) / nn;
  T ang = acos(clampT(R22, T(-1), T(1))) * T(180 / 3.14159265358979323846);
  if (ang > T(cfg.max_allowed_tilt)) flags |= F_FAILURE | F_TERMINATED;
  else if (cfg.reward_kind != 2) r = r + cfg.survival_bonus;
  reward = r;
  return flags;
  }
}

}
```

openballbot-rl_amd/csrc/bb_team16.h:

```cpp
#pragma once

#include <type_traits>
#include <utility>

#include "bb_bodycon.h"
#include "bb_solve.h"

namespace bb {

constexpr int LTR_SPARE = NV * (NV - 1) / 2, LTR_SLOTS = LTR_SPARE + 1;
BB_HD int ltr_slot(int tl, int k) {
  const int rw = tl < NV ? tl : 0;
  const int base = k < rw ? rw * (rw - 1) / 2 : LTR_SPARE - k;
  return base + k;
}

#ifdef __HIP_DEVICE_COMPILE__
namespace t16 {

constexpr int L = 16;

template <int CTRL>
__device__ __forceinline__ float dpp(float v) {
  return __int_as_float(__builtin_amdgcn_mov_dpp(__float_as_int(v), CTRL, 0xF, 0xF, true));
// ... 112 lines not shown
        BB_FD_I(6, NEG)                                                                                               \
        : BB_FD_A(0), BB_FD_A(1), BB_FD_A(2), BB_FD_A(3), BB_FD_A(4), BB_FD_A(5), BB_FD_A(6)                          \
        : BB_FD_IN, BB_FD_J(0), BB_FD_J(1), BB_FD_J(2), BB_FD_J(3), BB_FD_J(4), BB_FD_J(5), BB_FD_J(6));              \
  if constexpr (N == 8)                                                                                               \
    asm("s_nop 1\n\t" BB_FD_I(0, NEG) BB_FD_I(1, NEG) BB_FD_I(2, NEG) BB_FD_I(3, NEG) BB_FD_I(4, NEG) BB_FD_I(5, NEG) \
        BB_FD_I(6, NEG) BB_FD_I(7, NEG)                                                                               \
        : BB_FD_A(0), BB_FD_A(1), BB_FD_A(2), BB_FD_A(3), BB_FD_A(4), BB_FD_A(5), BB_FD_A(6), BB_FD_A(7)              \
        : BB_FD_IN, BB_FD_J(0), BB_FD_J(1), BB_FD_J(2), BB_FD_J(3), BB_FD_J(4), BB_FD_J(5), BB_FD_J(6), BB_FD_J(7));
template <bool NEG, int N, int J0, int J1, int J2, int J3, int J4, int J5, int J6, int J7, int M>
__device__ __forceinline__ void fmac_chunk(double (&h)[M], double x, double own) {
  static_assert(N >= 1 && N <= 8, "one to eight columns per hazard wait");
  if constexpr (NEG) {
    BB_FD_CHUNK("-")
  } else {
    BB_FD_CHUNK("")
  }
}
#undef BB_FD_CHUNK
#undef BB_FD_IN
#undef BB_FD_J
#undef BB_FD_A
#undef BB_FD_I
#endif

template <int... J>
constexpr int col_at(int i) {
  constexpr int cols[] = {J...};
  return i < int(sizeof...(J)) ? cols[i] : 0;
}
template <bool NEG, int OFF, int... J, typename T, int M>
__device__ __forceinline__ void fmac_cols_from(T (&h)[M], T x, T own) {
  constexpr int n = int(sizeof...(J)) - OFF;
  if constexpr (n > 0) {
#ifndef BB_NO_FMAC_DPP
    if constexpr (sizeof(T) == 8) {
      constexpr int c = n < 8 ? n : 8;
      fmac_chunk<NEG, c, col_at<J...>(OFF), col_at<J...>(OFF + 1), col_at<J...>(OFF + 2), col_at<J...>(OFF + 3),
                 col_at<J...>(OFF + 4), col_at<J...>(OFF + 5), col_at<J...>(OFF + 6), col_at<J...>(OFF + 7)>(h, x, own);
      fmac_cols_from<NEG, OFF + 8, J...>(h, x, own);
      return;
    }
#endif
    if constexpr (OFF == 0) ((h[J] = fma(NEG ? -bcast<J>(x) : bcast<J>(x), own, h[J])), ...);
  }
}
template <int... J, typename T, int M>
__device__ __forceinline__ void fmac_bcast_cols(T (&h)[M], T x, T own) {
  fmac_cols_from<false, 0, J...>(h, x, own);
}
template <int K0, typename T, int M, int... I>
__device__ __forceinline__ void fnmac_run_seq(T (&h)[M], T x, T own, std::integer_sequence<int, I...>) {
  fmac_cols_from<true, 0, (K0 + I)...>(h, x, own);
}
template <int K0, int N, typename T, int M>
__device__ __forceinline__ void fnmac_bcast_run(T (&h)[M], T x, T own) {
  fnmac_run_seq<K0>(h, x, own, std::make_integer_sequence<int, N>{});
}

template <typename T>
__device__ __forceinline__ void cone_sel(const T* jar, T mu, T f1, T f2, const T* D, T Dm, T* force, T* C) {
  const T U0 = jar[0] * mu, U1 = jar[1] * f1, U2 = jar[2] * f2;
  const T t2 = U1 * U1 + U2 * U2;
  const T rt = t2 > 0 ? rsqrt(t2) : T(0);
  const T N = U0, Tn = t2 * rt;
  const bool top = N >= mu * Tn || (Tn <= 0 && N >= 0);
  const bool bot = !top && (mu * N + Tn <= 0 || (Tn <= 0 && N < 0));
  const T g = N - mu * Tn;
  const T iT = Tn > 0 ? rt : T(1);
  const T gr1 = -mu * f1 * U1 * iT, gr2 = -mu * f2 * U2 * iT;
  const T sc = -Dm * g;
  const T k = Dm * g * (-mu) * iT, iT2 = iT * iT;
  T fm[3] = {sc * mu, sc * gr1, sc * gr2};
  T cm[6] = {Dm * mu * mu, Dm * gr1 * gr1 + k * f1 * f1 * (T(1) - U1 * U1 * iT2),
             Dm * gr2 * gr2 + k * f2 * f2 * (T(1) - U2 * U2 * iT2), Dm * mu * gr1, Dm * mu * gr2,
             Dm * gr1 * gr2 - k * f1 * f2 * U1 * U2 * iT2};
#pragma unroll
  for (int r = 0; r < 3; r++) force[r] = top ? T(0) : (bot ? -D[r] * jar[r] : fm[r]);
#pragma unroll
  for (int r = 0; r < 6; r++) C[r] = top ? T(0) : (bot ? (r < 3 ? D[r] : T(0)) : cm[r]);
}

__device__ __forceinline__ int col_dof(int q, int hinge) { return q < 6 ? q : (q == 6 ? (hinge >= 0 ? 6 + hinge : -1) : q + 2); }

template <typename T>
__device__ __forceinline__ T rsqrt_piv(T x) {
  if constexpr (sizeof(T) == 8) {
    const double r = __builtin_amdgcn_rsq(x);
    const double e = fma(-x * r, r, 1.0);
    return fma(r * e, fma(e, 0.375, 0.5), r);
  } else {
    return __builtin_amdgcn_rsqf(x);
  }
}

template <bool FUSE = false, typename T>
__device__ __forceinline__ void chol_rows(T (&h)[NV], T hdi, T (&diag)[NV], int tl) {
  static_for<NV>([&](auto jc) {
    constexpr int j = decltype(jc)::value;
    T piv = bcast<j>(h[j]);
    const T hdj = bcast<j>(hdi);
    const T fl = pivot_eps<T>() * maxT(hdj, T(1e-30));
    piv = fmax(piv, fl);
    const T id = rsqrt_piv(piv);
    diag[j] = id;
    h[j] *= id;
    if constexpr (FUSE && kFmacDpp) {
      fnmac_bcast_run<j + 1, NV - 1 - j>(h, h[j], h[j]);
    } else {
      static_for<NV - 1 - j>([&](auto kc) {
        constexpr int k = j + 1 + decltype(kc)::value;
        const T lkj = bcast<k>(h[j]);
        h[k] -= h[j] * lkj;
      });
    }
  });
}

template <bool FUSE = false, bool SPARE = false, typename T>
__device__ __forceinline__ void chol_solve_rows(const T (&h)[NV], const T (&diag)[NV], T gown, T (&s)[NV], T& sown,
                                                int tl, T* scr) {
  T b = tl < NV ? -gown : T(0);
  T z = 0;
  static_for<NV>([&](auto jc) {
    constexpr int j = decltype(jc)::value;
    if constexpr (FUSE && kFmacDpp) {
      const T t = b * diag[j];
      z = tl == j ? t : z;
      fnmac_bcast<j>(b, t, h[j]);
    } else {
      const T yj = bcast<j>(b) * diag[j];
      z = tl == j ? yj : z;
      b -= h[j] * yj;
    }
  });
  if constexpr (SPARE) {
    static_for<NV - 1>([&](auto kc) {
      constexpr int k = decltype(kc)::value;
      scr[ltr_slot(tl, k)] = h[k];
    });
  } else if (tl < NV) {
    static_for<NV - 1>([&](auto kc) {
      constexpr int k = decltype(kc)::value;
      if (k < tl) scr[tl * (tl - 1) / 2 + k] = h[k];
    });
  }
  team_sync();
  T Lc[NV];
  static_for<NV>([&](auto ic) {
    constexpr int i = decltype(ic)::value;
    Lc[i] = (i > tl) ? scr[i * (i - 1) / 2 + tl] : T(0);
  });
  T own = 0;
  static_for<NV>([&](auto ic) {
    constexpr int i = NV - 1 - decltype(ic)::value;
    const T si = bcast<i>(z) * diag[i];
    s[i] = si;
    z -= Lc[i] * si;
    own = tl == i ? si : own;
  });
  sown = own;
}

template <typename T>
__device__ __forceinline__ void body_load(const EnvWork<T>& W, int b, T (&o)[NBF]) {
  if (b < MAXB_LDS) {
    const T* p = W.bc + b * NBF;
#pragma unroll
    for (int i = 0; i < NBF; i++) o[i] = p[i];
  } else {
    const T* p = W.bspill + (b - MAXB_LDS) * NBF;
#pragma unroll
    for (int i = 0; i < NBF; i++) o[i] = p[i];
  }
}

template <bool BODY, typename T>
__device__ __forceinline__ void ls_terms(const ModelT<T>& m, const EnvWork<T>& W, int c, int ng, int nc, const T* a,
                                         const T* s, T (&c6)[6], T& D) {
#pragma unroll
  for (int r = 0; r < 6; r++) c6[r] = 0;
  D = 0;
  if (c >= nc) return;
  if (c < 3) {
    const WheelCon<T>& C = W.wc[c];
#pragma unroll
    for (int r = 0; r < 3; r++) { c6[r] = wheel_dot(C, c, r, a) - C.aref[r]; c6[3 + r] = wheel_dot(C, c, r, s); }
  } else if (c < 3 + ng) {
    T J[3][6], ar[3];
    ground_contact(m, W.g + (c - 3) * NGF, W.P.RB, W.vi, J, ar, D);
#pragma unroll
    for (int r = 0; r < 3; r++) { c6[r] = ground_dot(J, r, a) - ar[r]; c6[3 + r] = ground_dot(J, r, s); }
  } else if constexpr (BODY) {
    T bcv[NBF];
    body_load(W, c - 3 - ng, bcv);
    body_ls_terms(m, bcv, W.P, W.vi, a, s, c6, D);
  }
}

template <bool BODY, typename T>
__device__ __forceinline__ void ls_term(const ModelT<T>& m, const EnvWork<T>& W, int c, int ng, int nc, const T* a,
                                        const T* s, T kdw, LsTerm<T>& lt) {
  T c6[6], Dc;
  ls_terms<BODY>(m, W, c, ng, nc, a, s, c6, Dc);
  if (c >= nc) {
    lt.none();
    return;
  }
  const bool wheel = c < 3;
  const T D[3] = {wheel ? W.wc[c].D[0] : Dc, wheel ? W.wc[c].D[1] : Dc, wheel ? W.wc[c].D[2] : Dc};
  const T mu = wheel ? m.fr_wheel[0] : T(1), f1 = wheel ? m.fr_wheel[0] : T(1), f2 = wheel ? m.fr_wheel[1] : T(1);
  lt.prep(c6, c6 + 3, mu, f1, f2, D, D[0] * (wheel ? kdw : T(0.5)));
}

constexpr int GC_LDS = 13;
static_assert(GC_LDS * 18 <= MAXB_LDS * NBF, "ground Jacobians do not fit W.bc");

template <typename T>
__device__ __forceinline__ T* ground_ad(EnvWork<T>& W, int c) {
  static_assert(sizeof(Mass<T>) >= GC_LDS * 4 * sizeof(T), "ground aref/D do not fit the mass blocks");
  return reinterpret_cast<T*>(&W.M) + 4 * c;
}

template <typename T>
__device__ __forceinline__ void ground_setup(const ModelT<T>& m, EnvWork<T>& W, int ng, int tl) {
  const int c = tl - 3;
  if (c >= 0 && c < ng && c < GC_LDS) {
    T J[3][6], ar[3], D;
    ground_contact(m, W.g + c * NGF, W.P.RB, W.vi, J, ar, D);
    T* o = W.bc + c * 18;
#pragma unroll
    for (int r = 0; r < 3; r++)
#pragma unroll
      for (int i = 0; i < 6; i++) o[6 * r + i] = J[r][i];
    T* ad = ground_ad(W, c);
#pragma unroll
    for (int r = 0; r < 3; r++) ad[r] = ar[r];
    ad[3] = D;
  }
}

template <bool BODY, typename T>
__device__ __forceinline__ void ground_get(const ModelT<T>& m, EnvWork<T>& W, int c, T (&J)[3][6], T (&ar)[3], T& D) {
  if (!BODY && c < GC_LDS) {
    const T* o = W.bc + c * 18;
#pragma unroll
    for (int r = 0; r < 3; r++)
#pragma unroll
      for (int i = 0; i < 6; i++) J[r][i] = o[6 * r + i];
    const T* ad = ground_ad(W, c);
#pragma unroll
    for (int r = 0; r < 3; r++) ar[r] = ad[r];
    D = ad[3];
  } else {
    ground_contact(m, W.g + c * NGF, W.P.RB, W.vi, J, ar, D);
  }
}

#ifndef BB_NO_CARRY
constexpr bool kCarry = true;
#else
constexpr bool kCarry = false;
#endif

#ifndef BB_NO_LDS_BATCH_LS
constexpr bool kLdsBatchLs = true;
#else
constexpr bool kLdsBatchLs = false;
#endif
#ifndef BB_NO_LDS_BATCH_CP
constexpr bool kLdsBatchCp = true;
#else
constexpr bool kLdsBatchCp = false;
#endif
#ifndef BB_NO_LDS_BATCH_HESS
constexpr bool kLdsBatchHess = true;
#else
constexpr bool kLdsBatchHess = false;
#endif

#ifndef BB_NO_TAIL_UNIFORM
constexpr bool kTailUniform = true;
#else
constexpr bool kTailUniform = false;
#endif
#ifndef BB_NO_LS_SELECT
constexpr bool kLsSelect = true;
#else
constexpr bool kLsSelect = false;
#endif
#ifndef BB_NO_PREP_SELECT
constexpr bool kPrepSelect = true;
#else
constexpr bool kPrepSelect = false;
#endif

template <bool BODY, bool FUSE = false, typename T>
__device__ int solve16(const ModelT<T>& m, EnvWork<T>& W, int ng, int nb, T* a, int tl) {
  if constexpr (!BODY) nb = 0;
  const int ngc = 3 + ng;
  const int nc = ngc + nb;
  const bool rowl = tl < NV;
  const int row = rowl ? tl : NV - 1;
  const T muw = m.fr_wheel[0];
  const T kdw = T(1) / (muw * muw * (1 + muw * muw));
  const T qfs_i = W.qfs[row];
  const int gcol = row - 9;
  static_assert(offsetof(typename EnvWork<T>::U, hes.hg) == offsetof(typename EnvWork<T>::U, hes.wf) + 9 * sizeof(T),
                "wheel f/C scratch needs wf and hg adjacent");
  T* const wCf = &W.u.hes.wf[0][0];
  const bool gsum = ng > 0;
#ifdef BB_HROW_REG
  T hM[NV];
#pragma unroll
  for (int k = 0; k < NV; k++) hM[k] = W.H[hidx(row, k)];
#define BB_HROW(k) hM[k]
#else
#define BB_HROW(k) W.H[hidx(row, k)]
#endif
  PH_DECL
  constexpr bool CARRY = kCarry && !BODY;
  constexpr bool UTAIL = FUSE && !BODY && kTailUniform;
  constexpr bool LSSEL = FUSE && !BODY && kLsSelect;
  constexpr bool PREPSEL = FUSE && !BODY && kPrepSelect;
  T jar0[3] = {0, 0, 0}, mq = 0;
  int it = 0;
  bool held = false;
  for (; it < m.maxiter; it++) {
    team_sync();
    PH_TOP
    int tlx = tl;
    asm volatile("" : "+v"(tlx));
    const bool fresh = !CARRY || it == 0;
    bool more = true;
    if constexpr (UTAIL) more = __ballot(nc > L) != 0;
    (void)more;
    T gg[6], Hg[21];
    auto cone_of = [&](bool wheel, int c, const T (&jar)[3], T Dc, T (&f)[3], T (&Cc)[6]) __attribute__((always_inline)) {
      const T D[3] = {wheel ? W.wc[c].D[0] : Dc, wheel ? W.wc[c].D[1] : Dc, wheel ? W.wc[c].D[2] : Dc};
      const T mu = wheel ? muw : T(1), f1 = wheel ? muw : T(1), f2 = wheel ? m.fr_wheel[1] : T(1);
      const T Dm = D[0] * (wheel ? kdw : T(0.5));
      cone_sel(jar, mu, f1, f2, D, Dm, f, Cc);
    };
    auto wheel_put = [&](int c, const T (&f)[3], const T (&Cc)[6]) __attribute__((always_inline)) {
      T* p = wCf + 9 * c;
#pragma unroll
      for (int r = 0; r < 6; r++) p[r] = Cc[r];
#pragma unroll
      for (int r = 0; r < 3; r++) p[6 + r] = f[r];
    };
    auto cj_of = [&](const T (&Cc)[6], const T (&Jg)[3][6], T (&w)[3][6]) __attribute__((always_inline)) {
#pragma unroll
      for (int i = 0; i < 6; i++) {
        w[0][i] = Cc[0] * Jg[0][i] + Cc[3] * Jg[1][i] + Cc[4] * Jg[2][i];
        w[1][i] = Cc[3] * Jg[0][i] + Cc[1] * Jg[1][i] + Cc[5] * Jg[2][i];
        w[2][i] = Cc[4] * Jg[0][i] + Cc[5] * Jg[1][i] + Cc[2] * Jg[2][i];
      }
    };
    auto partials = [&](const T (&Jg)[3][6], const T (&f)[3], const T (&w)[3][6]) __attribute__((always_inline)) {
#pragma unroll
      for (int i = 0; i < 6; i++) gg[i] -= Jg[0][i] * f[0] + Jg[1][i] * f[1] + Jg[2][i] * f[2];
#pragma unroll
      for (int i = 0; i < 6; i++)
#pragma unroll
        for (int j = 0; j <= i; j++) Hg[i * (i + 1) / 2 + j] += Jg[0][i] * w[0][j] + Jg[1][i] * w[1][j] + Jg[2][i] * w[2][j];
    };
    auto contact_pass = [&]() __attribute__((always_inline)) {
#pragma unroll
      for (int i = 0; i < 6; i++) gg[i] = 0;
#pragma unroll
      for (int i = 0; i < 21; i++) Hg[i] = 0;
      if constexpr (UTAIL) {
        if (tl < ngc) {
          const int c = tl;
          const bool wheel = c < 3;
          T jar[3] = {jar0[0], jar0[1], jar0[2]}, Dc = 0, Jg[3][6];
          if (!wheel) {
            T ar[3];
            ground_get<BODY>(m, W, c - 3, Jg, ar, Dc);
            if (fresh) {
#pragma unroll
              for (int r = 0; r < 3; r++) jar[r] = ground_dot(Jg, r, a) - ar[r];
            }
          } else if (fresh) {
            if constexpr (kLdsBatchCp) {
              wheel_jar3(W.wc[c], c, a, jar);
            } else {
#pragma unroll
              for (int r = 0; r < 3; r++) jar[r] = wheel_dot(W.wc[c], c, r, a) - W.wc[c].aref[r];
            }
          }
          if (fresh) {
#pragma unroll
            for (int r = 0; r < 3; r++) jar0[r] = jar[r];
          }
          T f[3], Cc[6];
          cone_of(wheel, c, jar, Dc, f, Cc);
          if (wheel) {
            wheel_put(c, f, Cc);
          } else {
            T w[3][6];
            cj_of(Cc, Jg, w);
            partials(Jg, f, w);
          }
        }
        if (more) {
          for (int c = tl + L; c < ngc; c += L) {
            T jar[3], Dc = 0, Jg[3][6], ar[3];
            ground_get<BODY>(m, W, c - 3, Jg, ar, Dc);
#pragma unroll
            for (int r = 0; r < 3; r++) jar[r] = ground_dot(Jg, r, a) - ar[r];
            T f[3], Cc[6], w[3][6];
            cone_of(false, c, jar, Dc, f, Cc);
            cj_of(Cc, Jg, w);
            partials(Jg, f, w);
          }
        }
      } else {
        for (int c = tl; c < ngc; c += L) {
          const bool wheel = c < 3;
          T jar[3] = {jar0[0], jar0[1], jar0[2]}, Dc = 0, Jg[3][6];
          if (!wheel) {
            T ar[3];
            ground_get<BODY>(m, W, c - 3, Jg, ar, Dc);
            if (fresh || c != tl) {
#pragma unroll
              for (int r = 0; r < 3; r++) jar[r] = ground_dot(Jg, r, a) - ar[r];
            }
          } else if (fresh) {
            if constexpr (FUSE && kLdsBatchCp) {
              wheel_jar3(W.wc[c], c, a, jar);
            } else {
#pragma unroll
              for (int r = 0; r < 3; r++) jar[r] = wheel_dot(W.wc[c], c, r, a) - W.wc[c].aref[r];
            }
          }
          if (fresh && c == tl) {
#pragma unroll
            for (int r = 0; r < 3; r++) jar0[r] = jar[r];
          }
          T f[3], Cc[6];
          cone_of(wheel, c, jar, Dc, f, Cc);
          if (wheel) {
            wheel_put(c, f, Cc);
          } else {
            T w[3][6];
            cj_of(Cc, Jg, w);
            partials(Jg, f, w);
          }
        }
      }
    };
#ifdef BB_EXP_DUP_CPASS
    {
      contact_pass();
      T z = 0;
      for (int i = 0; i < 6; i++) z += gg[i];
      for (int i = 0; i < 21; i++) z += Hg[i];
      asm volatile("" :: "v"(z) : "memory");
      team_sync();
    }
#endif
    contact_pass();
    T hb[NV], gb = 0;
#pragma unroll
    for (int i = 0; i < NV; i++) hb[i] = 0;
    if constexpr (BODY) {
#ifdef BB_EXP_DUP_FBODY
     for (int rep = 0; rep < 2; rep++) {
      if (rep == 1) { T z = 0; for (int i = 0; i < NV; i++) z += hb[i]; asm volatile("" :: "v"(z), "v"(gb) : "memory");
                      for (int i = 0; i < NV; i++) hb[i] = 0; gb = 0; }
#endif
      const bool r_ang = (row >= 3 && row < 6) || row >= 12, r_ball = row >= 9;
      const int r_h = (row >= 6 && row < 9) ? row - 6 : -2;
      const int r_e = row < 3 ? row : ((row >= 9 && row < 12) ? row - 9 : -1);
      T rc[3] = {0, 0, 0};
      if (r_ang) {
        const T* R = row < 6 ? W.P.Rb : W.P.RB;
        const int k = row < 6 ? row - 3 : row - 12;
        rc[0] = R[k]; rc[1] = R[3 + k]; rc[2] = R[6 + k];
      }
      T Ul[3] = {0, 0, 0}, Yb[3] = {0, 0, 0}, Ub[3] = {0, 0, 0}, YB[3] = {0, 0, 0}, hs[3] = {0, 0, 0};
      for (int b0 = 0; b0 < nb; b0 += L) {
        T A[6] = {0, 0, 0, 0, 0, 0}, ph[3] = {0, 0, 0}, db[3] = {0, 0, 0}, dB[3] = {0, 0, 0}, hw[3] = {0, 0, 0};
        T mb = 0;
        int hinge = -1;
        if (b0 + tl < nb) {
          T bcv[NBF];
          body_load(W, b0 + tl, bcv);
          BodyFrame<T> bf;
          body_frame(m, bcv, W.P, W.vi, bf);
          T V[3], jar[3];
          body_V(bf, W.P, a, V);
#pragma unroll
          for (int r = 0; r < 3; r++) jar[r] = dot3(bf.F[r], V) - bf.aref[r];
          const T D[3] = {bf.D, bf.D, bf.D};
          T f[3], Cc[6];
          cone_sel(jar, T(1), T(1), T(1), D, bf.D * T(0.5), f, Cc);
          T G[3][3];
#pragma unroll
          for (int i = 0; i < 3; i++) {
            G[0][i] = Cc[0] * bf.F[0][i] + Cc[3] * bf.F[1][i] + Cc[4] * bf.F[2][i];
            G[1][i] = Cc[3] * bf.F[0][i] + Cc[1] * bf.F[1][i] + Cc[5] * bf.F[2][i];
            G[2][i] = Cc[4] * bf.F[0][i] + Cc[5] * bf.F[1][i] + Cc[2] * bf.F[2][i];
            ph[i] = bf.F[0][i] * f[0] + bf.F[1][i] * f[1] + bf.F[2][i] * f[2];
          }
          auto Aij = [&](int i, int j) { return bf.F[0][i] * G[0][j] + bf.F[1][i] * G[1][j] + bf.F[2][i] * G[2][j]; };
          A[0] = Aij(0, 0); A[1] = Aij(1, 1); A[2] = Aij(2, 2); A[3] = Aij(0, 1); A[4] = Aij(0, 2); A[5] = Aij(1, 2);
#pragma unroll
          for (int i = 0; i < 3; i++) { db[i] = bf.db[i]; dB[i] = bf.dB[i]; hw[i] = bf.hw[i]; }
          mb = -bf.ball;
          hinge = bf.hinge;
        }
        const int cnt = nb - b0;
        static_for<L>([&](auto jc_) {
          constexpr int j = decltype(jc_)::value;
          if (j < cnt) {
            const int hj = __builtin_amdgcn_update_dpp(0, hinge, 0x150 + j, 0xF, 0xF, false);
            T Ab[6], pb[3], dbb[3], dBb[3], hwb[3];
#pragma unroll
            for (int r = 0; r < 6; r++) Ab[r] = bcast<j>(A[r]);
#pragma unroll
            for (int r = 0; r < 3; r++) {
              pb[r] = bcast<j>(ph[r]); dbb[r] = bcast<j>(db[r]); dBb[r] = bcast<j>(dB[r]); hwb[r] = bcast<j>(hw[r]);
            }
            const T mbb = bcast<j>(mb);
            T w[3], cx[3], wx[3];
#pragma unroll
            for (int r = 0; r < 3; r++) cx[r] = row < 6 ? dbb[r] : dBb[r];
            cross3(wx, rc, cx);
#pragma unroll
            for (int r = 0; r < 3; r++) {
              T x = (r_e == r ? T(1) : T(0)) + (r_ang ? wx[r] : T(0)) + (r_h == hj ? hwb[r] : T(0));
              w[r] = r_ball ? mbb * x : x;
            }
            const T u[3] = {Ab[0] * w[0] + Ab[3] * w[1] + Ab[4] * w[2], Ab[3] * w[0] + Ab[1] * w[1] + Ab[5] * w[2],
                            Ab[4] * w[0] + Ab[5] * w[1] + Ab[2] * w[2]};
            gb -= w[0] * pb[0] + w[1] * pb[1] + w[2] * pb[2];
            T y[3], yB[3];
            cross3(y, dbb, u);
            cross3(yB, dBb, u);
#pragma unroll
            for (int r = 0; r < 3; r++) {
              Ul[r] += u[r];
              Yb[r] += y[r];
              Ub[r] += mbb * u[r];
              YB[r] += mbb * yB[r];
            }
            const T hu = hwb[0] * u[0] + hwb[1] * u[1] + hwb[2] * u[2];
#pragma unroll
            for (int r = 0; r < 3; r++) hs[r] += hj == r ? hu : T(0);
          }
        });
      }
#pragma unroll
      for (int k = 0; k < 3; k++) {
        hb[k] = Ul[k];
        hb[3 + k] = W.P.Rb[k] * Yb[0] + W.P.Rb[3 + k] * Yb[1] + W.P.Rb[6 + k] * Yb[2];
        hb[6 + k] = hs[k];
        hb[9 + k] = Ub[k];
        hb[12 + k] = W.P.RB[k] * YB[0] + W.P.RB[3 + k] * YB[1] + W.P.RB[6 + k] * YB[2];
      }
#ifdef BB_EXP_DUP_FBODY
     }
#endif
    }
    PH(0)
    if (gsum) {
#ifdef BB_EXP_DUP_GSUM
      {
        T z = 0;
#pragma unroll
        for (int i = 0; i < 6; i++) z += tsum(gg[i] * T(0.5));
#pragma unroll
        for (int i = 0; i < 21; i++) z += tsum(Hg[i] * T(0.5));
        asm volatile("" :: "v"(z) : "memory");
      }
#endif
      tsum_n(gg);
      tsum_n(Hg);
    }
    team_sync();
    PH(1)
    T h[NV];
#pragma unroll
    for (int k = 0; k < NV; k++) h[k] = BB_HROW(k);
    if (fresh) {
      T Ma = 0;
#pragma unroll
      for (int k = 0; k < NV; k++) Ma += h[k] * a[k];
      mq = rowl ? Ma - qfs_i : T(0);
    }
    T gi = mq;
    static_for<3>([&](auto wc_) {
      constexpr int w = decltype(wc_)::value;
      const int p = wheel_pos(row, w);
      const WheelCon<T>& C = W.wc[w];
      const T* q = wCf + 9 * w + 6;
      if constexpr (FUSE) {
        const int pc = p >= 0 ? p : 0;
        const T t = C.J[0][pc] * q[0] + C.J[1][pc] * q[1] + C.J[2][pc] * q[2];
        gi -= p >= 0 ? t : T(0);
      } else if (p >= 0) {
        gi -= C.J[0][p] * q[0] + C.J[1][p] * q[1] + C.J[2][p] * q[2];
      }
    });
    if (gsum) {
#pragma unroll
// ... 7 lines not shown
      w0 = C[0] * j0 + C[3] * j1 + C[4] * j2;
      w1 = C[3] * j0 + C[1] * j1 + C[5] * j2;
      w2 = C[4] * j0 + C[5] * j1 + C[2] * j2;
    };
    auto wheel_blocks = [&](T (&hh)[NV]) {
      if constexpr (sizeof(T) == 8 && FUSE && kFmacDpp && kLdsBatchHess) {
        T jc[3][3], Cw[3][6];
        static_for<3>([&](auto wc_) {
          constexpr int w = decltype(wc_)::value;
          const int p = wheel_pos(row, w);
          const int pc = p >= 0 ? p : 0;
#pragma unroll
          for (int r = 0; r < 3; r++) jc[w][r] = W.wc[w].J[r][pc];
#pragma unroll
          for (int k = 0; k < 6; k++) Cw[w][k] = wCf[9 * w + k];
        });
        BB_ISSUE_FENCE();
        static_for<3>([&](auto wc_) {
          constexpr int w = decltype(wc_)::value;
          const int p = wheel_pos(row, w);
          const T j0 = p >= 0 ? jc[w][0] : T(0), j1 = p >= 0 ? jc[w][1] : T(0), j2 = p >= 0 ? jc[w][2] : T(0);
          T u0, u1, u2;
          cw(Cw[w], j0, j1, j2, u0, u1, u2);
          fmac_bcast_cols<0, 1, 2, 3, 4, 5, 6 + w, 9, 10, 11, 12, 13, 14>(hh, j0, u0);
          fmac_bcast_cols<0, 1, 2, 3, 4, 5, 6 + w, 9, 10, 11, 12, 13, 14>(hh, j1, u1);
          fmac_bcast_cols<0, 1, 2, 3, 4, 5, 6 + w, 9, 10, 11, 12, 13, 14>(hh, j2, u2);
        });
        return;
      }
      static_for<3>([&](auto wc_) {
        constexpr int w = decltype(wc_)::value;
        const int p = wheel_pos(row, w);
        const WheelCon<T>& C = W.wc[w];
        if constexpr (sizeof(T) == 8) {
          const int pc = p >= 0 ? p : 0;
          const T j0 = p >= 0 ? C.J[0][pc] : T(0), j1 = p >= 0 ? C.J[1][pc] : T(0), j2 = p >= 0 ? C.J[2][pc] : T(0);
          T u0, u1, u2;
          cw(wCf + 9 * w, j0, j1, j2, u0, u1, u2);
          if constexpr (FUSE && kFmacDpp) {
            fmac_bcast_cols<0, 1, 2, 3, 4, 5, 6 + w, 9, 10, 11, 12, 13, 14>(hh, j0, u0);
            fmac_bcast_cols<0, 1, 2, 3, 4, 5, 6 + w, 9, 10, 11, 12, 13, 14>(hh, j1, u1);
            fmac_bcast_cols<0, 1, 2, 3, 4, 5, 6 + w, 9, 10, 11, 12, 13, 14>(hh, j2, u2);
          } else if (p >= 0) {
#pragma unroll
            for (int q = 0; q < 13; q++) {
              T& e = hh[wheel_col(q, w)];
              e = fma(C.J[0][q], u0, e);
              e = fma(C.J[1][q], u1, e);
              e = fma(C.J[2][q], u2, e);
            }
          }
        } else if (p >= 0) {
          T w0, w1, w2;
          cw(wCf + 9 * w, C.J[0][p], C.J[1][p], C.J[2][p], w0, w1, w2);
#pragma unroll
          for (int q = 0; q < 13; q++) hh[wheel_col(q, w)] += w0 * C.J[0][q] + w1 * C.J[1][q] + w2 * C.J[2][q];
        }
      });
    };
#ifdef BB_EXP_DUP_HESS
    {
      T h2[NV];
#pragma unroll
      for (int k = 0; k < NV; k++) h2[k] = h[k] * T(0.5);
      wheel_blocks(h2);
      T acc = 0;
#pragma unroll
      for (int k = 0; k < NV; k++) acc += h2[k];
      asm volatile("" :: "v"(acc) : "memory");
    }
#endif
    wheel_blocks(h);
    if (gsum) {
#pragma unroll
      for (int ai = 0; ai < 6; ai++)
#pragma unroll
        for (int b = 0; b < 6; b++) {
          const T v = Hg[ai >= b ? ai * (ai + 1) / 2 + b : b * (b + 1) / 2 + ai];
          h[9 + b] += row == 9 + ai ? v : T(0);
        }
    }
    if constexpr (BODY) {
#pragma unroll
      for (int k = 0; k < NV; k++) h[k] += hb[k];
    }
    T hdi = 0;
#pragma unroll
    for (int k = 0; k < NV; k++) hdi = row == k ? h[k] : hdi;
    PH(3)
    T diag[NV], s[NV], sown;
#ifdef BB_EXP_DUP_CHOL
    {
      T h2[NV], d2[NV];
#pragma unroll
      for (int k = 0; k < NV; k++) h2[k] = h[k];
      chol_rows<FUSE>(h2, hdi, d2, tl);
      asm volatile("" :: "v"(d2[NV - 1]), "v"(h2[NV - 2]) : "memory");
    }
#endif
    chol_rows<FUSE>(h, hdi, diag, tl);
    PH(4)
#ifdef BB_EXP_DUP_TRSV
    {
      T s2[NV], so2;
      chol_solve_rows<FUSE, FUSE>(h, diag, gi, s2, so2, tl, &W.u.hes.cj[0][0][0]);
      asm volatile("" :: "v"(s2[0]), "v"(so2) : "memory");
      team_sync();
    }
#endif
    static_assert(sizeof(W.u.hes.cj) >= LTR_SLOTS * sizeof(T), "L's transpose and its spare slot do not fit cj");
    chol_solve_rows<FUSE, FUSE>(h, diag, gi, s, sown, tlx, &W.u.hes.cj[0][0][0]);
    T d0 = tsum(sown * gi);
    bool fin = true;
#pragma unroll
    for (int i = 0; i < NV; i++) fin = fin && isfinite(s[i]);
    if (!fin || !(d0 < 0)) {
      sown = rowl ? -gi / maxT(W.H[hidx(row, row)], T(1e-30)) : T(0);
      static_for<NV>([&](auto kc) {
        constexpr int k = decltype(kc)::value;
        s[k] = bcast<k>(sown);
      });
      d0 = tsum(sown * gi);
      if (!(d0 < 0)) break;
    }
    PH(5)
    T Ms = 0;
#pragma unroll
    for (int k = 0; k < NV; k++) Ms += BB_HROW(k) * s[k];
    const T sMs = tsum(sown * Ms), gs = tsum(sown * mq);
    LsTerm<T> lt;
    T x[3] = {0, 0, 0};
    if constexpr (PREPSEL) {
      const bool act = tl < ngc, wheel = tl < 3;
      T Dc[3] = {0, 0, 0};
      if (wheel) {
        const WheelCon<T>& C = W.wc[tl];
        if constexpr (kLdsBatchLs) {
          wheel_dot3(C, tl, s, x, C.D, Dc);
        } else {
#pragma unroll
          for (int r = 0; r < 3; r++) { x[r] = wheel_dot(C, tl, r, s); Dc[r] = C.D[r]; }
        }
      } else if (act) {
        T Jg[3][6], ar[3], D;
        ground_get<BODY>(m, W, tl - 3, Jg, ar, D);
#pragma unroll
        for (int r = 0; r < 3; r++) { x[r] = ground_dot(Jg, r, s); Dc[r] = D; }
      }
      const T one = act ? T(1) : T(0);
      const T mu = wheel ? muw : one, f1 = wheel ? muw : one, f2 = wheel ? m.fr_wheel[1] : one;
      const T j0[3] = {act ? jar0[0] : T(0), act ? jar0[1] : T(0), act ? jar0[2] : T(0)};
      lt.prep_sel(j0, x, mu, f1, f2, Dc, Dc[0] * (wheel ? kdw : T(0.5)));
    } else if (tl < ngc) {
      const bool wheel = tl < 3;
      T Dc[3];
      if (wheel) {
        const WheelCon<T>& C = W.wc[tl];
        if constexpr (FUSE && kLdsBatchLs) {
          wheel_dot3(C, tl, s, x, C.D, Dc);
        } else {
#pragma unroll
          for (int r = 0; r < 3; r++) { x[r] = wheel_dot(C, tl, r, s); Dc[r] = C.D[r]; }
        }
      } else {
        T Jg[3][6], ar[3], D;
        ground_get<BODY>(m, W, tl - 3, Jg, ar, D);
#pragma unroll
        for (int r = 0; r < 3; r++) { x[r] = ground_dot(Jg, r, s); Dc[r] = D; }
      }
      const T mu = wheel ? muw : T(1), f1 = wheel ? muw : T(1), f2 = wheel ? m.fr_wheel[1] : T(1);
      lt.prep(jar0, x, mu, f1, f2, Dc, Dc[0] * (wheel ? kdw : T(0.5)));
    } else {
      ls_term<BODY>(m, W, tl, ng, nc, a, s, kdw, lt);
    }
    LineSearch<T> lsr;
    bool ls_ok = false;
#ifdef BB_EXP_DUP_LS
    auto line_search = [&](LineSearch<T>& lsr, bool& ls_ok) {
      lsr.init(d0);
      ls_ok = false;
      for (int ls = 1; ls <= m.ls_maxiter; ls++) {
        const T alpha = lsr.alpha;
        T d1p = 0, d2p = 0, dmp = 0;
        lt.eval(alpha, d1p, d2p, dmp);
        for (int c = tl + L; c < nc; c += L) {
          LsTerm<T> lc;
          ls_term<BODY>(m, W, c, ng, nc, a, s, kdw, lc);
          lc.eval(alpha, d1p, d2p, dmp);
        }
        const T d1 = gs + alpha * sMs + tsum(d1p);
        const T d2 = sMs + tsum(d2p);
        const T dmag = fabs(gs) + fabs(alpha * sMs) + tsum(dmp);
        if (fabs(d1) <= m.ls_tol * fabs(d0) || fabs(d1) <= T(32) * eps_of<T>() * dmag) { ls_ok = true; break; }
        if (!(d1 == d1)) break;
        lsr.update(d1, d2);
        const bool up = lsr.alpha > lsr.prev;
        const T big = T(1e30);
        const T kv = tmin(lsr.crosses(lt.kink) ? (up ? lt.kink : -lt.kink) : big);
        const T ks = up ? kv : -kv;
        lsr.dx = kv < big ? fabs(ks - lsr.prev) : lsr.dx;
        lsr.alpha = kv < big ? ks : lsr.alpha;
      }
    };
    {
      LineSearch<T> l2;
      bool ok2;
      line_search(l2, ok2);
      asm volatile("" :: "v"(l2.alpha), "v"(int(ok2)) : "memory");
    }
    PH(8)
    line_search(lsr, ls_ok);
#else
    lsr.init(d0);
    PH(8)
    if constexpr (LSSEL) {
      bool done = false;
      for (int ls = 1; ls <= m.ls_maxiter && !done; ls++) {
        const T alpha = lsr.alpha;
        T p[3] = {0, 0, 0};
        lt.eval(alpha, p[0], p[1], p[2]);
        if (more) {
          for (int c = tl + L; c < nc; c += L) {
            LsTerm<T> lc;
            ls_term<BODY>(m, W, c, ng, nc, a, s, kdw, lc);
            lc.eval(alpha, p[0], p[1], p[2]);
          }
        }
        tsum_n(p);
        const T d1 = ls_exits(lsr, ls_ok, done, p[0], p[2], gs, sMs, d0, m.ls_tol);
        if (__ballot(!done) == 0) break;
        ls_next(lsr, done, d1, sMs + p[1], [&](const LineSearch<T>& n, bool up) {
          return tmin(n.crosses_sel(lt.kink) ? (up ? lt.kink : -lt.kink) : T(1e30));
        });
      }
    } else {
    for (int ls = 1; ls <= m.ls_maxiter; ls++) {
      const T alpha = lsr.alpha;
      T d1p = 0, d2p = 0, dmp = 0;
      lt.eval(alpha, d1p, d2p, dmp);
      if (more) {
        for (int c = tl + L; c < nc; c += L) {
          LsTerm<T> lc;
          ls_term<BODY>(m, W, c, ng, nc, a, s, kdw, lc);
          lc.eval(alpha, d1p, d2p, dmp);
        }
      }
      const T d1 = gs + alpha * sMs + tsum(d1p);
      if (fabs(d1) <= m.ls_tol * fabs(d0)) { ls_ok = true; break; }
      const T dmag = fabs(gs) + fabs(alpha * sMs) + tsum(dmp);
      if (fabs(d1) <= T(32) * eps_of<T>() * dmag) { ls_ok = true; break; }
      if (!(d1 == d1)) break;
      const T d2 = sMs + tsum(d2p);
      lsr.update(d1, d2);
      const bool up = lsr.alpha > lsr.prev;
      const T big = T(1e30);
      const T kv = tmin(lsr.crosses(lt.kink) ? (up ? lt.kink : -lt.kink) : big);
      const T ks = up ? kv : -kv;
      lsr.dx = kv < big ? fabs(ks - lsr.prev) : lsr.dx;
      lsr.alpha = kv < big ? ks : lsr.alpha;
    }
    }
#endif
    if (!ls_ok) lsr.alpha = lsr.fallback();
    PH(9)
    const T alpha = lsr.alpha;
    if (!(alpha > 0)) break;
    T dc = lt.cost(alpha) - lt.cost(T(0));
    if (more) {
      for (int c = tl + L; c < nc; c += L) {
        LsTerm<T> lc;
        ls_term<BODY>(m, W, c, ng, nc, a, s, kdw, lc);
        dc += lc.cost(alpha) - lc.cost(T(0));
      }
    }
    const T dcost = alpha * (gs + T(0.5) * alpha * sMs) + tsum(dc);
    T sn = 0, an2 = 0;
#pragma unroll
    for (int i = 0; i < NV; i++) { a[i] += alpha * s[i]; sn += s[i] * s[i]; an2 += a[i] * a[i]; }
    if constexpr (CARRY) {
#pragma unroll
      for (int r = 0; r < 3; r++) jar0[r] += alpha * x[r];
      mq = rowl ? mq + alpha * Ms : T(0);
    }
    PH(6)
    if (alpha * alpha * sn <= T(1e-30) + m.step_rel2 * (1 + an2)) { it++; break; }
    if (-m.scale * dcost < m.tol) {
      const bool far = m.scale * m.scale * gn >= T(IMPR_GRAD * IMPR_GRAD) * m.tol * m.tol;
      if (!far || held) { it++; break; }
      held = true;
    }
  }
  PH(7)
#undef BB_HROW
  if constexpr (BODY) {
    PH_FLUSH_BODY((Team{L, tl}))
  } else {
    PH_FLUSH((Team{L, tl}))
  }
  return it;
}

template <typename T>
__device__ __forceinline__ int collide_team(const ModelT<T>& m, const Kin<T>& k, const T* v, const float* hf,
                                            T size_z, T* g, int* overflow, int tl) {
  const T r = m.ball_r;
  const T* c = k.c;
  const T sx = m.hf_sx, sy = m.hf_sy, zb = m.hf_bottom;
  const T xmin = c[0] - r, xmax = c[0] + r, ymin = c[1] - r, ymax = c[1] + r, zmin = c[2] - r, zmax = c[2] + r;
  if (!(xmin <= sx && xmax >= -sx && ymin <= sy && ymax >= -sy && zmin <= size_z && zmax >= -zb)) return 0;
  const int N1 = HF_N - 1;
  int cmin = (int)floor((xmin + sx) / (2 * sx) * N1);
  int cmax = (int)ceil((xmax + sx) / (2 * sx) * N1);
  int rmin = (int)floor((ymin + sy) / (2 * sy) * N1);
  int rmax = (int)ceil((ymax + sy) / (2 * sy) * N1);
  cmin = cmin < 0 ? 0 : cmin;
  cmax = cmax > N1 ? N1 : cmax;
  rmin = rmin < 0 ? 0 : rmin;
  rmax = rmax > N1 ? N1 : rmax;
  const int ncol = cmax - cmin + 1;
  const int np = 2 * ncol - 2;
  const int total = (rmax - rmin) * (np > 0 ? np : 0);
  const T dx = 2 * sx / N1, dy = 2 * sy / N1;
  (void)v;
  const int team_shift = team_shift_of(L);
  int ng = 0;
  auto heights = [&](int P, float (&h)[3]) {
    if (P < total) {
      const int rr = rmin + P / np, p = P % np;
#pragma unroll
      for (int t = 0; t < 3; t++) {
        const int vt = p + t;
        h[t] = hf[(rr + (vt & 1)) * HF_N + cmin + (vt >> 1)];
      }
    }
  };
  float hnext[3] = {0.f, 0.f, 0.f};
  heights(tl, hnext);
  for (int base = 0; base < total; base += L) {
    const int P = base + tl;
    bool hit = false;
    T nn[3] = {0, 0, 1}, dist = 0;
    const float hcur[3] = {hnext[0], hnext[1], hnext[2]};
    heights(P + L, hnext);
    if (P < total) {
      const int rr = rmin + P / np, p = P % np;
      T V[3][3];
#pragma unroll
      for (int t = 0; t < 3; t++) {
        const int vt = p + t, cc = cmin + (vt >> 1), ri = rr + (vt & 1);
        V[t][0] = dx * cc - sx;
        V[t][1] = dy * ri - sy;
        V[t][2] = T(hcur[t]) * size_z;
        (void)ri; (void)cc;
      }
      if (!(V[0][2] < zmin && V[1][2] < zmin && V[2][2] < zmin)) {
        const T bx0 = minT(V[0][0], minT(V[1][0], V[2][0])), bx1 = maxT(V[0][0], maxT(V[1][0], V[2][0]));
        const T by0 = minT(V[0][1], minT(V[1][1], V[2][1])), by1 = maxT(V[0][1], maxT(V[1][1], V[2][1]));
        const T ztop = maxT(V[0][2], maxT(V[1][2], V[2][2]));
        const T ex = maxT(T(0), maxT(bx0 - c[0], c[0] - bx1));
        const T ey = maxT(T(0), maxT(by0 - c[1], c[1] - by1));
        const T ez = maxT(T(0), c[2] - ztop);
        if (ex * ex + ey * ey + ez * ez <= r * r) hit = sphere_prism(c, r, V, -zb, nn, &dist);
      }
    }
    const unsigned long long bal = __ballot(hit);
    const unsigned bits = unsigned(bal >> team_shift) & 0xFFFFu;
    const int slot = ng + __popc(bits & ((1u << tl) - 1u));
    if (hit) {
      if (slot < MAXG) {
        T* gs = g + slot * NGF;
#pragma unroll
        for (int i = 0; i < 3; i++) gs[GF_N + i] = nn[i];
        gs[GF_DIST] = dist;
      }
    }
    ng += __popc(bits);
  }
  if (ng > MAXG) { ng = MAXG; *overflow = 1; }
  return ng;
}

template <typename T>
__device__ __forceinline__ void put_body(T* bc, T* spill, int slot, const T* n, const T* pos, T dist, int b1, int b2) {
  T* s = body_slot(bc, spill, slot);
#pragma unroll
  for (int i = 0; i < 3; i++) { s[BF_N + i] = n[i]; s[BF_P + i] = pos[i]; }
  s[BF_DIST] = dist;
  s[BF_CODE] = T(8 * b1 + b2);
}

template <typename T>
struct Reach {
  T c[3], a[3], hh, r, ia[2];
  bool par[2];
};

template <typename T>
__device__ __forceinline__ void make_reach(const Seg<T>& g, Reach<T>& R) {
#pragma unroll
  for (int i = 0; i < 3; i++) { R.c[i] = g.c[i]; R.a[i] = g.a[i]; }
  R.hh = g.hh; R.r = g.r;
#pragma unroll
  for (int ax = 0; ax < 2; ax++) {
    R.par[ax] = fabs(g.a[ax]) < T(1e-12);
    R.ia[ax] = R.par[ax] ? T(0) : T(1) / g.a[ax];
  }
}

template <typename T>
__device__ __forceinline__ bool prism_may_hit(const Reach<T>& g, const T (&V)[3][3]) {
  T t0 = -g.hh, t1 = g.hh;
  bool out = false;
#pragma unroll
  for (int ax = 0; ax < 2; ax++) {
    const T lo = minT(V[0][ax], minT(V[1][ax], V[2][ax])) - g.r;
    const T hi = maxT(V[0][ax], maxT(V[1][ax], V[2][ax])) + g.r;
    if (g.par[ax]) {
      out = out || g.c[ax] < lo || g.c[ax] > hi;
    } else {
      const T ta = (lo - g.c[ax]) * g.ia[ax], tb = (hi - g.c[ax]) * g.ia[ax];
      t0 = maxT(t0, minT(ta, tb));
      t1 = minT(t1, maxT(ta, tb));
    }
  }
  if (out || t0 > t1) return false;
  const T ztop = maxT(V[0][2], maxT(V[1][2], V[2][2]));
  const T zmin = g.c[2] + minT(t0 * g.a[2], t1 * g.a[2]) - g.r;
  return zmin <= ztop;
}

template <typename T>
__device__ bool body_candidates(const ModelT<T>& m, const Kin<T>& k, const float* hf, T size_z, T hz, int tl) {
  bool cand = false;
  bool reach = false;
  if (tl < 6) {
    Seg<T> g;
    body_geom(m, k, tl, g);
    if (tl < 3) {
      T dist, n[3], pos[3];
      cand = tl == 0 ? sphere_cylinder(k.c, m.ball_r, g, dist, n, pos) : sphere_capsule(k.c, m.ball_r, g, dist, n, pos);
    }
    if (hf) {
      const T sx = m.hf_sx, sy = m.hf_sy, zb = m.hf_bottom;
      T lo[3], hi[3];
#pragma unroll
      for (int i = 0; i < 3; i++) {
        const T ai = fabs(g.a[i]);
        const T rad = T(1) - ai * ai;
        const T ext = tl == 0 ? g.hh * ai + g.r * sqrt(rad > 0 ? rad : T(0)) : g.hh * ai + g.r;
        lo[i] = g.c[i] - ext; hi[i] = g.c[i] + ext;
      }
      reach = lo[2] <= hz && lo[0] <= sx && hi[0] >= -sx && lo[1] <= sy && hi[1] >= -sy && lo[2] <= size_z &&
              hi[2] >= -zb;
    }
  }
  unsigned todo = unsigned(__ballot(reach) >> team_shift_of(L)) & 0x3Fu;
  if (hf) {
    const T sx = m.hf_sx, sy = m.hf_sy;
    const int N1 = HF_N - 1;
    while (todo) {
      const int gi = __builtin_ctz(todo);
      todo &= todo - 1;
      Seg<T> g;
      body_geom(m, k, gi, g);
      Reach<T> gr;
      make_reach(g, gr);
      T lo[3], hi[3];
#pragma unroll
      for (int i = 0; i < 3; i++) {
        const T ai = fabs(g.a[i]);
        const T rad = T(1) - ai * ai;
        const T ext = gi == 0 ? g.hh * ai + g.r * sqrt(rad > 0 ? rad : T(0)) : g.hh * ai + g.r;
        lo[i] = g.c[i] - ext; hi[i] = g.c[i] + ext;
      }
      int cmin = (int)floor((lo[0] + sx) / (2 * sx) * N1), cmax = (int)ceil((hi[0] + sx) / (2 * sx) * N1);
      int rmin = (int)floor((lo[1] + sy) / (2 * sy) * N1), rmax = (int)ceil((hi[1] + sy) / (2 * sy) * N1);
      cmin = cmin < 0 ? 0 : cmin; cmax = cmax > N1 ? N1 : cmax;
      rmin = rmin < 0 ? 0 : rmin; rmax = rmax > N1 ? N1 : rmax;
      if (rmax <= rmin || cmax <= cmin) continue;
      const T dx = 2 * sx / N1, dy = 2 * sy / N1;
      const int nc = cmax - cmin, total = (rmax - rmin) * nc;
      for (int i = tl; i < total && !cand; i += L) {
        const int ri = rmin + i / nc, ci = cmin + i % nc;
        const T x0 = dx * ci - sx, x1 = dx * (ci + 1) - sx, y0 = dy * ri - sy, y1 = dy * (ri + 1) - sy;
        const T z00 = T(hf[ri * HF_N + ci]) * size_z, z10 = T(hf[(ri + 1) * HF_N + ci]) * size_z;
        const T z01 = T(hf[ri * HF_N + ci + 1]) * size_z, z11 = T(hf[(ri + 1) * HF_N + ci + 1]) * size_z;
        const T A[3][3] = {{x0, y0, z00}, {x0, y1, z10}, {x1, y0, z01}};
        const T B[3][3] = {{x0, y1, z10}, {x1, y0, z01}, {x1, y1, z11}};
        const bool ta = !(z00 < lo[2] && z10 < lo[2] && z01 < lo[2]) && prism_may_hit(gr, A);
        const bool tb = !(z10 < lo[2] && z01 < lo[2] && z11 < lo[2]) && prism_may_hit(gr, B);
        cand = ta || tb;
      }
    }
  }
  const unsigned bits = unsigned(__ballot(cand) >> team_shift_of(L)) & 0xFFFFu;
  return bits != 0;
}

constexpr int CAND_CAP = 80;


template <typename T>
__device__ int collide_body_team(const ModelT<T>& m, const Kin<T>& k, const float* hf, T size_z, T hz, T* bc,
                                 T* spill, int* overflow, int tl, int* cand) {
  const int team_shift = team_shift_of(L);
  const unsigned below = (1u << tl) - 1u;
  int nb = 0;
  auto compact = [&](bool hit) -> int {
    const unsigned bits = unsigned(__ballot(hit) >> team_shift) & 0xFFFFu;
    const int slot = nb + __popc(bits & below);
    nb += int(__popc(bits));
    return slot;
  };
  {
    bool hit = false;
    T dist = 0, n[3] = {0, 0, 1}, pos[3] = {0, 0, 0};
    if (tl < 3) {
      Seg<T> g;
      body_geom(m, k, tl, g);
      hit = tl == 0 ? sphere_cylinder(k.c, m.ball_r, g, dist, n, pos) : sphere_capsule(k.c, m.ball_r, g, dist, n, pos);
    }
    const int slot = compact(hit);
    if (hit) put_body(bc, spill, slot, n, pos, dist, 7, tl + 1);
  }
  if (hf) {
    const T sx = m.hf_sx, sy = m.hf_sy, zb = m.hf_bottom;
    const int N1 = HF_N - 1;
    const T dx = 2 * sx / N1, dy = 2 * sy / N1;
    int nc = 0;
    int pair_n[6] = {0, 0, 0, 0, 0, 0};
    auto vertices = [&](int rr, int p, T (&V)[3][3]) {
#pragma unroll
      for (int t = 0; t < 3; t++) {
        const int vt = p + t, cc = (vt >> 1), ri = rr + (vt & 1);
        V[t][0] = dx * cc - sx;
        V[t][1] = dy * ri - sy;
        V[t][2] = T(hf[ri * HF_N + cc]) * size_z;
      }
    };
    auto flush = [&]() {
      team_sync();
      for (int base = 0; base < nc; base += L) {
        bool hit = false;
        T dist = 0, n[3] = {0, 0, 1}, pos[3] = {0, 0, 0};
        int b2 = 0;
#if defined(BB_PHASE_CLOCKS) && defined(__HIP_DEVICE_COMPILE__)
        int sat_path = -1;
        const unsigned long long sat_c0 = clock64();
#endif
        if (base + tl < nc) {
          const int code = cand[base + tl];
          const int gi = code >> 26, rr = (code >> 13) & 0x1FFF, p = code & 0x1FFF;
          Seg<T> g;
          body_geom(m, k, gi, g);
          T V[3][3];
          vertices(rr, p, V);
          PrismG<T> Pr;
          prism_build(Pr, V, -zb);
#ifdef BB_EXP_DUP_SAT
          {
            T d2 = 0, n2[3], p2[3];
            const bool h2 = gi == 0 ? cylinder_prism(g, Pr, d2, n2, p2) : capsule_prism(g, Pr, d2, n2, p2);
            asm volatile("" :: "v"(d2), "v"(n2[0]), "v"(p2[0]), "v"(int(h2)) : "memory");
          }
#endif
#if defined(BB_PHASE_CLOCKS) && defined(__HIP_DEVICE_COMPILE__)
          sat_path = gi == 0 ? 3 : capsule_prism_path(g, Pr);
#endif
#ifdef BB_EXP_DUP_CYL
          if (gi == 0) {
            const T d2 = cylinder_prism_dup_call(g.c[0], g.c[1], g.c[2], g.a[0], g.a[1], g.a[2], g.hh, g.r, V[0][0],
                                                 V[0][1], V[0][2], V[1][0], V[1][1], V[1][2], V[2][0], V[2][1],
                                                 V[2][2], -zb);
            asm volatile("" :: "v"(d2) : "memory");
          }
#endif
          hit = gi == 0 ? cylinder_prism(g, Pr, dist, n, pos) : capsule_prism(g, Pr, dist, n, pos);
          b2 = gi + 1;
        }
#if defined(BB_PHASE_CLOCKS) && defined(__HIP_DEVICE_COMPILE__)
        {
          const int sh = team_shift_of(L);
          auto lanes = [&](bool c) { return __popc(unsigned(__ballot(c) >> sh) & 0xFFFFu); };
          const int nl = lanes(sat_path >= 0), ncy = lanes(sat_path == 3), neo = lanes(sat_path == 0),
                    nin = lanes(sat_path == 1), nap = lanes(sat_path == 2), nah = lanes(sat_path == 2 && hit);
          if (tl == 0) {
            atomicAdd(&bb_phase_cycles[90], 1ull);
            atomicAdd(&bb_phase_cycles[91], (unsigned long long)nl);
            atomicAdd(&bb_phase_cycles[92], (unsigned long long)ncy);
            atomicAdd(&bb_phase_cycles[93], (unsigned long long)neo);
            atomicAdd(&bb_phase_cycles[94], (unsigned long long)nin);
            atomicAdd(&bb_phase_cycles[95], (unsigned long long)nap);
            atomicAdd(&bb_phase_cycles[96], (unsigned long long)nah);
            atomicAdd(&bb_phase_cycles[97], (unsigned long long)(nap > 0));
            atomicAdd(&bb_phase_cycles[98], (unsigned long long)(nin + ncy > 0));
            atomicAdd(&bb_phase_cycles[99], clock64() - sat_c0);
          }
        }
#endif
        bool keep = hit;
#pragma unroll
        for (int g = 0; g < 6; g++) {
          const unsigned gb = unsigned(__ballot(hit && b2 == g + 1) >> team_shift) & 0xFFFFu;
          if (hit && b2 == g + 1) keep = pair_n[g] + __popc(gb & below) < MAXPAIR;
          if (pair_n[g] + __popc(gb) > MAXPAIR) *overflow |= 2;
          pair_n[g] = minT(pair_n[g] + int(__popc(gb)), MAXPAIR);
        }
        const int slot = compact(keep);
        if (keep) put_body(bc, spill, slot, n, pos, dist, 0, b2);
      }
      team_sync();
      nc = 0;
    };
    for (int gi = 0; gi < 6; gi++) {
      Seg<T> g;
      body_geom(m, k, gi, g);
      Reach<T> gr;
      make_reach(g, gr);
      const bool cyl = gi == 0;
      T lo[3], hi[3];
#pragma unroll
      for (int i = 0; i < 3; i++) {
        const T ai = fabs(g.a[i]);
        const T rad = T(1) - ai * ai;
        const T ext = cyl ? g.hh * ai + g.r * sqrt(rad > 0 ? rad : T(0)) : g.hh * ai + g.r;
        lo[i] = g.c[i] - ext; hi[i] = g.c[i] + ext;
      }
      if (!(lo[2] <= hz)) continue;
      if (!(lo[0] <= sx && hi[0] >= -sx && lo[1] <= sy && hi[1] >= -sy && lo[2] <= size_z && hi[2] >= -zb)) continue;
      int cmin = (int)floor((lo[0] + sx) / (2 * sx) * N1), cmax = (int)ceil((hi[0] + sx) / (2 * sx) * N1);
      int rmin = (int)floor((lo[1] + sy) / (2 * sy) * N1), rmax = (int)ceil((hi[1] + sy) / (2 * sy) * N1);
      cmin = cmin < 0 ? 0 : cmin; cmax = cmax > N1 ? N1 : cmax;
      rmin = rmin < 0 ? 0 : rmin; rmax = rmax > N1 ? N1 : rmax;
      const int np = 2 * (cmax - cmin + 1) - 2;
      const int total = (rmax - rmin) * (np > 0 ? np : 0);
#ifdef BB_EXP_DUP_PRUNE
      for (int base = 0; base < total; base += L) {
        const int P = base + tl;
        bool ch = false;
        if (P < total) {
          const int rr = rmin + P / np, p = 2 * cmin + P % np;
          T V[3][3];
          vertices(rr, p, V);
          ch = !(V[0][2] < lo[2] && V[1][2] < lo[2] && V[2][2] < lo[2]) && prism_may_hit(gr, V);
        }
        const unsigned long long bal = __ballot(ch);
        asm volatile("" :: "s"(bal) : "memory");
      }
#endif
      auto heights = [&](int P, float (&h)[3]) {
        if (P < total) {
          const int rr = rmin + P / np, p = 2 * cmin + P % np;
#pragma unroll
          for (int t = 0; t < 3; t++) {
            const int vt = p + t;
            h[t] = hf[(rr + (vt & 1)) * HF_N + (vt >> 1)];
          }
        }
      };
      float hnext[3] = {0.f, 0.f, 0.f};
      heights(tl, hnext);
      for (int base = 0; base < total; base += L) {
        const int P = base + tl;
        bool cand_hit = false;
        int code = 0;
        const float hcur[3] = {hnext[0], hnext[1], hnext[2]};
        heights(P + L, hnext);
        if (P < total) {
          const int rr = rmin + P / np, p = 2 * cmin + P % np;
          T V[3][3];
#pragma unroll
          for (int t = 0; t < 3; t++) {
            const int vt = p + t;
            V[t][0] = dx * (vt >> 1) - sx;
            V[t][1] = dy * (rr + (vt & 1)) - sy;
            V[t][2] = T(hcur[t]) * size_z;
          }
          cand_hit = !(V[0][2] < lo[2] && V[1][2] < lo[2] && V[2][2] < lo[2]) && prism_may_hit(gr, V);
          code = (gi << 26) | (rr << 13) | p;
        }
        const unsigned long long bal = __ballot(cand_hit);
        const unsigned bits = unsigned(bal >> team_shift) & 0xFFFFu;
        if (cand_hit) cand[nc + __popc(bits & ((1u << tl) - 1u))] = code;
        nc += int(__popc(bits));
#if defined(BB_PHASE_CLOCKS) && defined(__HIP_DEVICE_COMPILE__)
        if (tl == 0) atomicAdd(&bb_phase_cycles[19], (unsigned long long)__popc(bits));
#endif
        if (nc > CAND_CAP - L) flush();
      }
#if defined(BB_PHASE_CLOCKS) && defined(__HIP_DEVICE_COMPILE__)
      if (tl == 0) {
        atomicAdd(&bb_phase_cycles[16], 1ull);
        atomicAdd(&bb_phase_cycles[17], (unsigned long long)total);
        atomicAdd(&bb_phase_cycles[18], (unsigned long long)((total + L - 1) / L));
      }
#endif
    }
    if (nc > 0) flush();
  }
  return nb;
}

template <typename T>
__device__ __forceinline__ void mass_dense_team(EnvWork<T>& W, int tl) {
  for (int e = tl; e < NH; e += L) {
    int i, j;
    tri_unpack(e, i, j);
    W.H[e] = mass_entry(W.M, i, j);
  }
}

}
#endif
}
```

Before: 13.40 million.

## Split base/ball kinematics, bias and integration across team halves; precompute model constants

```diff
diff --git a/openballbot-rl_amd/ballbot_gym/_native.py b/openballbot-rl_amd/ballbot_gym/_native.py
--- a/openballbot-rl_amd/ballbot_gym/_native.py
+++ b/openballbot-rl_amd/ballbot_gym/_native.py
@@ -6,6 +6,8 @@
 
 PKG = Path(__file__).resolve().parent
 LIB_PATH = PKG / "_lib" / "libbb_mi355x.so"
+SERIAL_LIB_PATH = PKG / "_lib" / "libbb_mi355x_serial.so"
+SERIAL_FLAGS = ["-DBB_NO_TWIN_KIN", "-DBB_NO_TWIN_POS", "-DBB_NO_TWIN_BIAS", "-DBB_NO_MODEL_ONCE"]
 CSRC = PKG.parent / "csrc"
 INCLUDE = PKG.parent.parent / "include"
 
@@ -131,7 +133,8 @@
     from concurrent.futures import ThreadPoolExecutor
 
     srcs = list(CSRC.glob("*.h")) + list(CSRC.glob("*.hip")) + list(INCLUDE.glob("*.h"))
-    if LIB_PATH.exists() and not force and all(LIB_PATH.stat().st_mtime >= s.stat().st_mtime for s in srcs):
+    if (LIB_PATH.exists() and SERIAL_LIB_PATH.exists() and not force
+            and all(min(LIB_PATH.stat().st_mtime, SERIAL_LIB_PATH.stat().st_mtime) >= s.stat().st_mtime for s in srcs)):
         return LIB_PATH
     obj_dir = LIB_PATH.parent / "obj"
     obj_dir.mkdir(parents=True, exist_ok=True)
@@ -140,6 +143,9 @@
     for f in HIP_SOURCES:
         obj = obj_dir / (f[:-4] + ".o")
         jobs.append((["hipcc", *flags, *SOURCE_FLAGS.get(f, []), "-c", "-o", str(obj), str(CSRC / f)], obj))
+    serial_obj = obj_dir / "serial" / "bb_kernels.o"
+    serial_obj.parent.mkdir(exist_ok=True)
+    jobs.append((["hipcc", *flags, *SERIAL_FLAGS, "-c", "-o", str(serial_obj), str(CSRC / "bb_kernels.hip")], serial_obj))
     if verbose:
         for cmd, _ in jobs:
             print(" ".join(cmd))
@@ -153,12 +159,14 @@
     for (cmd, _), r in zip(jobs, results):
         if r.returncode != 0:
             raise subprocess.CalledProcessError(r.returncode, cmd, r.stdout, r.stderr + "\n" + " ".join(cmd))
-    tmp = LIB_PATH.with_suffix(".so.tmp")
-    link = ["hipcc", "--offload-arch=gfx950", "-shared", "-fPIC", "-o", str(tmp), *[str(o) for _, o in jobs]]
-    if verbose:
-        print(" ".join(link))
-    subprocess.run(link, check=True)
-    os.replace(tmp, LIB_PATH)
+    objs = [o for _, o in jobs[:-1]]
+    for out, these in ((LIB_PATH, objs), (SERIAL_LIB_PATH, [serial_obj if o.name == "bb_kernels.o" else o for o in objs])):
+        tmp = out.with_suffix(".so.tmp")
+        link = ["hipcc", "--offload-arch=gfx950", "-shared", "-fPIC", "-o", str(tmp), *[str(o) for o in these]]
+        if verbose:
+            print(" ".join(link))
+        subprocess.run(link, check=True)
+        os.replace(tmp, out)
     return LIB_PATH
 
 
diff --git a/openballbot-rl_amd/csrc/bb_kernels.hip b/openballbot-rl_amd/csrc/bb_kernels.hip
--- a/openballbot-rl_amd/csrc/bb_kernels.hip
+++ b/openballbot-rl_amd/csrc/bb_kernels.hip
@@ -59,6 +59,19 @@
 template <typename T>
 __device__ __forceinline__ EnvWork<T>& team_work(unsigned char* smem, int team) {
   return *reinterpret_cast<EnvWork<T>*>(smem + size_t(team) * work_stride<T>());
+}
+
+#ifndef BB_NO_MODEL_ONCE
+template <typename T> using ModelStage = ModelDev<T>;
+#else
+template <typename T> struct ModelStage { ModelT<T> m; };
+#endif
+template <typename T>
+__device__ __forceinline__ void stage_model(ModelStage<T>& ms, const ModelT<T>& mg) {
+  ms.m = mg;
+#ifndef BB_NO_MODEL_ONCE
+  model_once(mg, ms.once);
+#endif
 }
 
 struct TerrainSrc {
@@ -261,10 +274,10 @@
   } else {
     g = (nwg & 7) ? b : (b & 7) * (nwg >> 3) + (b >> 3);
   }
-  __shared__ ModelT<T> ms;
-  if (threadIdx.x == 0) ms = mg;
+  __shared__ ModelStage<T> ms;
+  if (threadIdx.x == 0) stage_model(ms, mg);
   __syncthreads();
-  const ModelT<T>& m = ms;
+  const ModelT<T>& m = ms.m;
   const Team tm{L, int(threadIdx.x) & (L - 1)};
   const int team = threadIdx.x / L;
   if (team >= epw) return;
@@ -469,10 +482,10 @@
   extern __shared__ __align__(16) unsigned char smem[];
   const int nwg = int(gridDim.x), b = int(blockIdx.x);
   const int g = (nwg & 7) ? b : (b & 7) * (nwg >> 3) + (b >> 3);
-  __shared__ ModelT<T> ms;
-  if (threadIdx.x == 0) ms = mg;
+  __shared__ ModelStage<T> ms;
+  if (threadIdx.x == 0) stage_model(ms, mg);
   __syncthreads();
-  const ModelT<T>& m = ms;
+  const ModelT<T>& m = ms.m;
   const Team tm{L, int(threadIdx.x) & (L - 1)};
   const int team = threadIdx.x / L;
   if (team >= epw) return;
diff --git a/openballbot-rl_amd/csrc/bb_physics.h b/openballbot-rl_amd/csrc/bb_physics.h
--- a/openballbot-rl_amd/csrc/bb_physics.h
+++ b/openballbot-rl_amd/csrc/bb_physics.h
@@ -48,6 +48,55 @@
   T qpos0[NQ];
 };
 
+#ifndef BB_NO_TWIN_KIN
+#define BB_TWIN_KIN 1
+#else
+#define BB_TWIN_KIN 0
+#endif
+#ifndef BB_NO_TWIN_POS
+#define BB_TWIN_POS 1
+#else
+#define BB_TWIN_POS 0
+#endif
+#ifndef BB_NO_TWIN_BIAS
+#define BB_TWIN_BIAS 1
+#else
+#define BB_TWIN_BIAS 0
+#endif
+#if !defined(BB_NO_MODEL_ONCE) && defined(__HIP_DEVICE_COMPILE__)
+#define BB_ONCE 1
+#else
+#define BB_ONCE 0
+#endif
+constexpr int TWIN_L = 16;
+
+template <typename T>
+struct ModelOnce {
+  T bc[2][3];
+  T bI[2][6];
+  T bm[2];
+  T au[3][3];
+  T dcj[3];
+  T mt;
+  T sbd;
+  T MBrr[2];
+  T kdw;
+  T rr;
+  T dx, dy;
+};
+template <typename T>
+struct ModelDev {
+  ModelT<T> m;
+  ModelOnce<T> once;
+};
+#if BB_ONCE
+template <typename T>
+__device__ __forceinline__ const ModelOnce<T>& once_of(const ModelT<T>& m) {
+  static_assert(offsetof(ModelDev<T>, m) == 0, "the model leads ModelDev");
+  return reinterpret_cast<const ModelDev<T>*>(&m)->once;
+}
+#endif
+
 template <typename T> BB_HD T dot3(const T* a, const T* b) { return a[0] * b[0] + a[1] * b[1] + a[2] * b[2]; }
 template <typename T> BB_HD void cross3(T* r, const T* a, const T* b) {
   T x = a[1] * b[2] - a[2] * b[1], y = a[2] * b[0] - a[0] * b[2], z = a[0] * b[1] - a[1] * b[0];
@@ -134,6 +183,51 @@
 #endif
 }
 
+template <typename T> BB_HD void once_base_com(const ModelT<T>& m, T* c0, T* Ic) {
+  c0[0] = m.h0[0] / m.m0; c0[1] = m.h0[1] / m.m0; c0[2] = m.h0[2] / m.m0;
+  T cc = dot3(c0, c0);
+  Ic[0] = m.I0O[0] - m.m0 * (cc - c0[0] * c0[0]); Ic[1] = m.I0O[1] - m.m0 * (cc - c0[1] * c0[1]);
+  Ic[2] = m.I0O[2] - m.m0 * (cc - c0[2] * c0[2]); Ic[3] = m.I0O[3] + m.m0 * c0[0] * c0[1];
+  Ic[4] = m.I0O[4] + m.m0 * c0[0] * c0[2]; Ic[5] = m.I0O[5] + m.m0 * c0[1] * c0[2];
+}
+template <typename T> BB_HD void once_ball_com(const ModelT<T>& m, T* cB, T* IcB) {
+  cB[0] = 0; cB[1] = 0; cB[2] = m.dz;
+  IcB[0] = m.IB; IcB[1] = m.IB; IcB[2] = m.IB; IcB[3] = 0; IcB[4] = 0; IcB[5] = 0;
+}
+template <typename T> BB_HD void once_au(const ModelT<T>& m, int w, T* au) { cross3(au, m.anchor, m.u[w]); }
+template <typename T> BB_HD void once_dcj(const ModelT<T>& m, T* d) {
+  d[0] = m.cw[0] - m.jpos[0]; d[1] = m.cw[1] - m.jpos[1]; d[2] = m.cw[2] - m.jpos[2];
+}
+template <typename T> BB_HD void once_mass(const ModelT<T>& m, T& mt, T& sbd, T* MBrr) {
+  const T dz = m.dz;
+  mt = m.m0 + 3 * m.mw;
+  sbd = m.mB * dz;
+  MBrr[0] = m.IB + m.mB * dz * dz;
+  MBrr[1] = m.IB;
+}
+template <typename T> BB_HD T once_kdw(const ModelT<T>& m) {
+  const T muw = m.fr_wheel[0];
+  return T(1) / (muw * muw * (1 + muw * muw));
+}
+template <typename T> BB_HD T once_rr(const ModelT<T>& m) { return m.fr_wheel[0] / m.fr_wheel[1]; }
+template <typename T> BB_HD void once_pitch(const ModelT<T>& m, T& dx, T& dy) {
+  const T sx = m.hf_sx, sy = m.hf_sy;
+  const int N1 = HF_N - 1;
+  dx = 2 * sx / N1; dy = 2 * sy / N1;
+}
+template <typename T> BB_HD void model_once(const ModelT<T>& m, ModelOnce<T>& o) {
+  once_base_com(m, o.bc[0], o.bI[0]);
+  once_ball_com(m, o.bc[1], o.bI[1]);
+  o.bm[0] = m.m0; o.bm[1] = m.mB;
+#pragma unroll
+  for (int w = 0; w < 3; w++) once_au(m, w, o.au[w]);
+  once_dcj(m, o.dcj);
+  once_mass(m, o.mt, o.sbd, o.MBrr);
+  o.kdw = once_kdw(m);
+  o.rr = once_rr(m);
+  once_pitch(m, o.dx, o.dy);
+}
+
 template <typename T> BB_HD void qmul(T* r, const T* a, const T* b) {
   T w = a[0] * b[0] - a[1] * b[1] - a[2] * b[2] - a[3] * b[3];
   T x = a[0] * b[1] + a[1] * b[0] + a[2] * b[3] - a[3] * b[2];
@@ -171,6 +265,20 @@
   q[7] += h * v[6]; q[8] += h * v[7]; q[9] += h * v[8];
   q[10] += h * v[9]; q[11] += h * v[10]; q[12] += h * v[11];
   quat_integrate(q + 13, v + 12, h);
+}
+template <typename T> BB_HD void integrate_pos_lin(T* q, const T* v, T h) {
+  q[0] += h * v[0]; q[1] += h * v[1]; q[2] += h * v[2];
+  q[7] += h * v[6]; q[8] += h * v[7]; q[9] += h * v[8];
+  q[10] += h * v[9]; q[11] += h * v[10]; q[12] += h * v[11];
+}
+BB_HD constexpr int half_qpos(bool hi) { return hi ? 10 : 0; }
+BB_HD constexpr int half_quat(bool hi) { return hi ? 13 : 3; }
+BB_HD constexpr int half_vlin(bool hi) { return hi ? 9 : 0; }
+BB_HD constexpr int half_vang(bool hi) { return hi ? 12 : 3; }
+template <typename T> BB_HD void integrate_quat_half(const T* qs, const T* ws, T h, T* qo) {
+  qo[0] = qs[0]; qo[1] = qs[1]; qo[2] = qs[2]; qo[3] = qs[3];
+  const T w[3] = {ws[0], ws[1], ws[2]};
+  quat_integrate(qo, w, h);
 }
 
 constexpr BB_HD int hidx(int i, int j) { return i >= j ? i * (i + 1) / 2 + j : j * (j + 1) / 2 + i; }
@@ -200,7 +308,26 @@
 }
 
 template <typename T>
-BB_HD void kinematics_wheel(const ModelT<T>& m, const T* q, int w, Kin<T>& k) {
+BB_HD void kinematics_half(const ModelT<T>& m, const T* q, bool hi, Kin<T>& k, T* qn) {
+  qn[0] = hi ? q[13] : q[3]; qn[1] = hi ? q[14] : q[4]; qn[2] = hi ? q[15] : q[5]; qn[3] = hi ? q[16] : q[6];
+  qnormalize(qn);
+  T R[9];
+  q2mat(R, qn);
+  const T p[3] = {hi ? q[10] : q[0], hi ? q[11] : q[1], hi ? q[12] : q[2]};
+  T* Rk = hi ? k.RB : k.Rb;
+  T* pk = hi ? k.pB : k.pb;
+#pragma unroll
+  for (int i = 0; i < 9; i++) Rk[i] = R[i];
+  pk[0] = p[0]; pk[1] = p[1]; pk[2] = p[2];
+  if (hi) {
+    k.c[0] = p[0] + R[2] * m.dz;
+    k.c[1] = p[1] + R[5] * m.dz;
+    k.c[2] = p[2] + R[8] * m.dz;
+  }
+}
+
+template <typename T>
+BB_HD void kinematics_wheel(const ModelT<T>& m, const T* q, int w, Kin<T>& k, const ModelOnce<T>* mo = nullptr) {
   T th = q[7 + w] - m.qpos0[7 + w];
   T s = sin(th * T(0.5)), cth = cos(th * T(0.5));
   T ql[4] = {cth, m.axis[0] * s, m.axis[1] * s, m.axis[2] * s};
@@ -208,7 +335,9 @@
   qmul(qw, m.wq[w], ql);
   qnormalize(qw);
   q2mat(k.Rw[w], qw);
-  T d[3] = {m.cw[0] - m.jpos[0], m.cw[1] - m.jpos[1], m.cw[2] - m.jpos[2]};
+  T d[3];
+  if (mo) { d[0] = mo->dcj[0]; d[1] = mo->dcj[1]; d[2] = mo->dcj[2]; }
+  else once_dcj(m, d);
   T t[3];
   mv3(t, k.Rw[w], d);
   k.wc[w][0] = m.anchor[0] + t[0];
@@ -265,7 +394,8 @@
 }
 
 template <typename T>
-BB_HD void mass_finish(const ModelT<T>& m, const Kin<T>& k, Mass<T>& M, const T (*mrw)[3], const T (*IOw)[6]) {
+BB_HD void mass_finish(const ModelT<T>& m, const Kin<T>& k, Mass<T>& M, const T (*mrw)[3], const T (*IOw)[6],
+                       const ModelOnce<T>* mo = nullptr) {
   T mr[3] = {m.h0[0], m.h0[1], m.h0[2]};
   T IO[6] = {m.I0O[0], m.I0O[1], m.I0O[2], m.I0O[3], m.I0O[4], m.I0O[5]};
 #pragma unroll
@@ -275,19 +405,21 @@
 #pragma unroll
     for (int i = 0; i < 6; i++) IO[i] += IOw[w][i];
   }
-  M.mt = m.m0 + 3 * m.mw;
+  T mt, sbd, MBrr[2];
+  if (mo) { mt = mo->mt; sbd = mo->sbd; MBrr[0] = mo->MBrr[0]; MBrr[1] = mo->MBrr[1]; }
+  else once_mass(m, mt, sbd, MBrr);
+  M.mt = mt;
   M.mr[0] = mr[0]; M.mr[1] = mr[1]; M.mr[2] = mr[2];
   T S[9] = {0, mr[2], -mr[1], -mr[2], 0, mr[0], mr[1], -mr[0], 0};
   mm3(M.Mtr, k.Rb, S);
 #pragma unroll
   for (int i = 0; i < 6; i++) M.Mrr[i] = IO[i];
-  const T dz = m.dz;
   M.mB = m.mB;
-  T SB[9] = {0, m.mB * dz, 0, -m.mB * dz, 0, 0, 0, 0, 0};
+  T SB[9] = {0, sbd, 0, -sbd, 0, 0, 0, 0, 0};
   mm3(M.MBtr, k.RB, SB);
-  M.MBrr[0] = m.IB + m.mB * dz * dz;
-  M.MBrr[1] = m.IB + m.mB * dz * dz;
-  M.MBrr[2] = m.IB;
+  M.MBrr[0] = MBrr[0];
+  M.MBrr[1] = MBrr[0];
+  M.MBrr[2] = MBrr[1];
 }
 
 template <typename T>
@@ -385,10 +517,11 @@
 
 template <typename T>
 BB_HD T bias_wheel(const ModelT<T>& m, const Kin<T>& k, const T* Iw, const T* v, int w, const T* w0, const T* vl,
-                   const T* a0, T* fa, T* fl) {
+                   const T* a0, T* fa, T* fl, const ModelOnce<T>* mo = nullptr) {
   const T* u = m.u[w];
   T au[3];
-  cross3(au, m.anchor, u);
+  if (mo) { const T* a = mo->au[w]; au[0] = a[0]; au[1] = a[1]; au[2] = a[2]; }
+  else once_au(m, w, au);
   T qd = v[6 + w];
   T Vw[3] = {w0[0] + qd * u[0], w0[1] + qd * u[1], w0[2] + qd * u[2]};
   T Vv[3] = {vl[0] + qd * au[0], vl[1] + qd * au[1], vl[2] + qd * au[2]};
@@ -403,17 +536,22 @@
 }
 
 template <typename T>
-BB_HD void bias_finish(const ModelT<T>& m, const Kin<T>& k, const T* v, const T (*fw)[6], T* bias) {
+BB_HD void bias_finish(const ModelT<T>& m, const Kin<T>& k, const T* v, const T (*fw)[6], T* bias,
+                       const ModelOnce<T>* mo = nullptr) {
   T w0[3], vl[3], a0[3], t[3];
   bias_base_motion(m, k, v, w0, vl, a0);
   const T zero[3] = {0, 0, 0};
   T Fa[3], Fl[3];
   {
-    T c0[3] = {m.h0[0] / m.m0, m.h0[1] / m.m0, m.h0[2] / m.m0};
-    T cc = dot3(c0, c0);
-    T Ic[6] = {m.I0O[0] - m.m0 * (cc - c0[0] * c0[0]), m.I0O[1] - m.m0 * (cc - c0[1] * c0[1]),
-               m.I0O[2] - m.m0 * (cc - c0[2] * c0[2]), m.I0O[3] + m.m0 * c0[0] * c0[1],
-               m.I0O[4] + m.m0 * c0[0] * c0[2], m.I0O[5] + m.m0 * c0[1] * c0[2]};
+    T c0[3], Ic[6];
+    if (mo) {
+#pragma unroll
+      for (int i = 0; i < 3; i++) c0[i] = mo->bc[0][i];
+#pragma unroll
+      for (int i = 0; i < 6; i++) Ic[i] = mo->bI[0][i];
+    } else {
+      once_base_com(m, c0, Ic);
+    }
     body_force(m.m0, c0, Ic, zero, a0, w0, vl, Fa, Fl);
   }
 #pragma unroll
@@ -428,12 +566,54 @@
   mtv3(vB, k.RB, v + 9);
   cross3(t, vB, wB);
   T aB[3] = {m.grav * k.RB[6] + t[0], m.grav * k.RB[7] + t[1], m.grav * k.RB[8] + t[2]};
-  T cB[3] = {0, 0, m.dz};
-  T IcB[6] = {m.IB, m.IB, m.IB, 0, 0, 0};
+  T cB[3], IcB[6];
+  once_ball_com(m, cB, IcB);
   T fa[3], fl[3];
   body_force(m.mB, cB, IcB, zero, aB, wB, vB, fa, fl);
   mv3(bias + 9, k.RB, fl);
   bias[12] = fa[0]; bias[13] = fa[1]; bias[14] = fa[2];
+}
+
+template <typename T>
+BB_HD void bias_finish_half(const ModelT<T>& m, const Kin<T>& k, const T* v, const T (*fw)[6], bool hi, T* out,
+                            const ModelOnce<T>* mo = nullptr) {
+  const T* R = hi ? k.RB : k.Rb;
+  const T* vlin = v + half_vlin(hi);
+  const T* vang = v + half_vang(hi);
+  T w0[3] = {vang[0], vang[1], vang[2]}, vl[3], t[3];
+  mtv3(vl, R, vlin);
+  cross3(t, vl, w0);
+  T a0[3] = {m.grav * R[6] + t[0], m.grav * R[7] + t[1], m.grav * R[8] + t[2]};
+  const T zero[3] = {0, 0, 0};
+  T Fa[3], Fl[3];
+  T c[3], Ic[6], mass;
+  if (mo) {
+    const int b = hi ? 1 : 0;
+#pragma unroll
+    for (int i = 0; i < 3; i++) c[i] = mo->bc[b][i];
+#pragma unroll
+    for (int i = 0; i < 6; i++) Ic[i] = mo->bI[b][i];
+    mass = mo->bm[b];
+  } else {
+    T c0[3], Ic0[6], cB[3], IcB[6];
+    once_base_com(m, c0, Ic0);
+    once_ball_com(m, cB, IcB);
+#pragma unroll
+    for (int i = 0; i < 3; i++) c[i] = hi ? cB[i] : c0[i];
+#pragma unroll
+    for (int i = 0; i < 6; i++) Ic[i] = hi ? IcB[i] : Ic0[i];
+    mass = hi ? m.mB : m.m0;
+  }
+  body_force(mass, c, Ic, zero, a0, w0, vl, Fa, Fl);
+  if (!hi) {
+#pragma unroll
+    for (int w = 0; w < 3; w++) {
+      Fa[0] += fw[w][0]; Fa[1] += fw[w][1]; Fa[2] += fw[w][2];
+      Fl[0] += fw[w][3]; Fl[1] += fw[w][4]; Fl[2] += fw[w][5];
+    }
+  }
+  mv3(out, R, Fl);
+  out[3] = Fa[0]; out[4] = Fa[1]; out[5] = Fa[2];
 }
 
 template <typename T>
@@ -514,7 +694,8 @@
 };
 
 template <typename T>
-BB_HD void wheel_contact(const ModelT<T>& m, const Kin<T>& k, const T* v, int w, WheelCon<T>& C) {
+BB_HD void wheel_contact(const ModelT<T>& m, const Kin<T>& k, const T* v, int w, WheelCon<T>& C,
+                         const ModelOnce<T>* mo = nullptr) {
   T t[3], gp[3], ax[3], axl[3];
   mv3(t, k.Rb, k.wc[w]);
   gp[0] = k.pb[0] + t[0]; gp[1] = k.pb[1] + t[1]; gp[2] = k.pb[2] + t[2];
@@ -562,7 +743,7 @@
   T imp = clampT(impedance(m, dist), T(0.0001), T(0.9999));
   T tran = m.iw_ball + m.iw_wheel[w];
   T R0 = maxT(T(1e-15), (1 - imp) * tran / imp);
-  T rr = m.fr_wheel[0] / m.fr_wheel[1];
+  T rr = mo ? mo->rr : once_rr(m);
   T R2 = R0 * rr * rr;
   C.D[0] = act / R0; C.D[1] = act / R0; C.D[2] = act / R2;
 #pragma unroll
diff --git a/openballbot-rl_amd/csrc/bb_step.h b/openballbot-rl_amd/csrc/bb_step.h
--- a/openballbot-rl_amd/csrc/bb_step.h
+++ b/openballbot-rl_amd/csrc/bb_step.h
@@ -3,6 +3,12 @@
 #include "bb_team16.h"
 
 namespace bb {
+
+#if defined(BB_ISA_MARKS) && defined(__HIP_DEVICE_COMPILE__)
+#define BB_PRE(k) asm volatile("; PRE_MARK " #k);
+#else
+#define BB_PRE(k)
+#endif
 
 struct EnvCfg {
   int max_ep_steps;
@@ -30,8 +36,23 @@
 #endif
   Kin<T>& k = W.u.pre.k;
 #ifdef __HIP_DEVICE_COMPILE__
-  kinematics_base(m, q, k);
-  if (tm.tl < 3) kinematics_wheel(m, q, tm.tl, k);
+  BB_PRE(2)
+  const ModelOnce<T>* mo = nullptr;
+#if BB_ONCE
+  if constexpr (FUSE) mo = &once_of(m);
+#endif
+  const bool twin = FUSE && tm.L == TWIN_L;
+  const bool hi = (tm.tl & 8) != 0;
+  (void)twin; (void)hi;
+#if BB_TWIN_KIN
+  if (twin) {
+    T qn[4];
+    kinematics_half(m, q, hi, k, qn);
+    if (so && !hi) { so->quat_b[0] = qn[0]; so->quat_b[1] = qn[1]; so->quat_b[2] = qn[2]; so->quat_b[3] = qn[3]; }
+  } else
+#endif
+    kinematics_base(m, q, k);
+  if (tm.tl < 3) kinematics_wheel(m, q, tm.tl, k, mo);
   team_sync();
 #else
   kinematics(m, q, k);
@@ -43,23 +64,37 @@
     T (*IOw)[6] = reinterpret_cast<T (*)[6]>(W.H + 9);
     T (*fw)[6] = reinterpret_cast<T (*)[6]>(W.H + 27);
     static_assert(NH >= 45, "per-wheel terms do not fit W.H");
+    BB_PRE(3)
     if (tm.tl < 3) {
       const int w = tm.tl;
       mass_wheel(m, k, w, M, W.u.pre.Iw[w], mrw[w], IOw[w]);
       T w0[3], vl[3], a0[3];
       bias_base_motion(m, k, v, w0, vl, a0);
-      const T qb = -bias_wheel(m, k, W.u.pre.Iw[w], v, w, w0, vl, a0, fw[w], fw[w] + 3);
+      const T qb = -bias_wheel(m, k, W.u.pre.Iw[w], v, w, w0, vl, a0, fw[w], fw[w] + 3, mo);
       const T cw = w == 0 ? ctrl[0] : (w == 1 ? ctrl[1] : ctrl[2]);
       W.qfs[6 + w] = qb + (-m.damping * v[6 + w] + cw);
-      wheel_contact(m, k, v, w, W.wc[w]);
-    }
-    team_sync();
-    mass_finish(m, k, M, mrw, IOw);
-    T qfs[NV];
-    bias_finish(m, k, v, fw, qfs);
-#pragma unroll
-    for (int i = 0; i < NV; i++)
-      if (i < 6 || i > 8) W.qfs[i] = -qfs[i];
+      wheel_contact(m, k, v, w, W.wc[w], mo);
+    }
+    team_sync();
+    BB_PRE(4)
+    mass_finish(m, k, M, mrw, IOw, mo);
+    BB_PRE(5)
+#if BB_TWIN_BIAS
+    if (twin) {
+      T b6[6];
+      bias_finish_half(m, k, W.vi, fw, hi, b6, mo);
+      T* qo = W.qfs + half_vlin(hi);
+#pragma unroll
+      for (int i = 0; i < 6; i++) qo[i] = -b6[i];
+    } else
+#endif
+    {
+      T qfs[NV];
+      bias_finish(m, k, v, fw, qfs, mo);
+#pragma unroll
+      for (int i = 0; i < NV; i++)
+        if (i < 6 || i > 8) W.qfs[i] = -qfs[i];
+    }
     team_sync();
   }
 #else
@@ -83,7 +118,8 @@
   const unsigned long long f_t1 = clock64();
 #endif
 #ifdef __HIP_DEVICE_COMPILE__
-  const int ng = tr.hf ? t16::collide_team(m, k, v, tr.hf, tr.size_z, W.g, &overflow, tm.tl) : 0;
+  BB_PRE(6)
+  const int ng = tr.hf ? t16::collide_team(m, k, v, tr.hf, tr.size_z, W.g, &overflow, tm.tl, mo) : 0;
   int nb = 0;
   if constexpr (BODY) {
 #if defined(BB_PHASE_CLOCKS)
@@ -106,7 +142,7 @@
     }
 #endif
   } else {
-    if (t16::body_candidates(m, k, tr.hf, tr.size_z, tr.hz, tm.tl)) return -1;
+    if (t16::body_candidates(m, k, tr.hf, tr.size_z, tr.hz, tm.tl, mo)) return -1;
   }
 #else
   const int ng = tr.hf ? collide_ground(m, k, v, tr.hf, tr.size_z, st, &overflow) : 0;
@@ -119,14 +155,21 @@
     atomicAdd(&bb_phase_cycles[10], 1ull);
   }
 #endif
+  BB_PRE(7)
 #pragma unroll
   for (int i = 0; i < 9; i++) { W.P.Rb[i] = k.Rb[i]; W.P.RB[i] = k.RB[i]; }
 #pragma unroll
   for (int i = 0; i < 3; i++) { W.P.pb[i] = k.pb[i]; W.P.pB[i] = k.pB[i]; }
   if (so) {
-    T qb[4] = {q[3], q[4], q[5], q[6]};
-    qnormalize(qb);
-    so->quat_b[0] = qb[0]; so->quat_b[1] = qb[1]; so->quat_b[2] = qb[2]; so->quat_b[3] = qb[3];
+    bool have_qb = false;
+#if BB_TWIN_KIN && defined(__HIP_DEVICE_COMPILE__)
+    have_qb = FUSE && tm.L == TWIN_L;
+#endif
+    if (!have_qb) {
+      T qb[4] = {q[3], q[4], q[5], q[6]};
+      qnormalize(qb);
+      so->quat_b[0] = qb[0]; so->quat_b[1] = qb[1]; so->quat_b[2] = qb[2]; so->quat_b[3] = qb[3];
+    }
     mv3(so->w_world, k.Rb, v + 3);
     T cl[3] = {M.mr[0] / M.mt, M.mr[1] / M.mt, M.mr[2] / M.mt}, cw[3], t[3];
     mv3(cw, k.Rb, cl);
@@ -165,7 +208,9 @@
     team_sync();
   }
 #endif
+  BB_PRE(8)
   const int it = t16::solve16<BODY, FUSE>(m, W, ng, nb, acc, tm.tl);
+  BB_PRE(9)
 #if defined(BB_PHASE_CLOCKS)
   if (BODY && tm.tl == 0) {
     atomicAdd(&bb_phase_cycles[15], clock64() - s_t0);
@@ -208,10 +253,41 @@
 #pragma unroll 1
   for (int stage = 0; stage < 4; stage++) {
     const T a = stage == 3 ? T(1) : T(0.5);
+    BB_PRE(1)
     {
       T qi[NQ], vi[NV];
 #pragma unroll
       for (int i = 0; i < NQ; i++) qi[i] = q0[i];
+#if BB_TWIN_POS && defined(__HIP_DEVICE_COMPILE__)
+      if (FUSE && tm.L == TWIN_L) {
+        const bool hi = (tm.tl & 8) != 0;
+        T qh[4];
+        if (stage == 0) {
+#pragma unroll
+          for (int i = 0; i < NV; i++) vi[i] = v0[i];
+#pragma unroll
+          for (int i = 0; i < 4; i++) qh[i] = q0[half_quat(hi) + i];
+        } else {
+          T dv[NV];
+#pragma unroll
+          for (int i = 0; i < NV; i++) { dv[i] = a * W.vi[i]; vi[i] = v0[i] + h * a * warm[i]; }
+          integrate_pos_lin(qi, dv, h);
+          const T* wp = W.vi + half_vang(hi);
+          const T wh[3] = {a * wp[0], a * wp[1], a * wp[2]};
+          integrate_quat_half(q0 + half_quat(hi), wh, h, qh);
+        }
+        team_sync();
+#pragma unroll
+        for (int i = 0; i < NQ; i++)
+          if (i < 3 || (i >= 7 && i < 13)) W.u.pre.qi[i] = qi[i];
+        T* qo = W.u.pre.qi + half_quat(hi);
+#pragma unroll
+        for (int i = 0; i < 4; i++) qo[i] = qh[i];
+#pragma unroll
+        for (int i = 0; i < NV; i++) W.vi[i] = vi[i];
+      } else
+#endif
+      {
       if (stage == 0) {
 #pragma unroll
         for (int i = 0; i < NV; i++) vi[i] = v0[i];
@@ -226,6 +302,7 @@
       for (int i = 0; i < NQ; i++) W.u.pre.qi[i] = qi[i];
 #pragma unroll
       for (int i = 0; i < NV; i++) W.vi[i] = vi[i];
+      }
     }
     T acc[NV];
 #pragma unroll
@@ -265,8 +342,28 @@
     }
   }
   team_sync();
+  BB_PRE(10)
 #pragma unroll
   for (int i = 0; i < NV; i++) v[i] = v0[i] + h * as[i];
+#if BB_TWIN_POS && defined(__HIP_DEVICE_COMPILE__)
+  if (FUSE && tm.L == TWIN_L) {
+    const bool hi = (tm.tl & 8) != 0;
+#pragma unroll
+    for (int i = 0; i < NQ; i++)
+      if (i < 3 || (i >= 7 && i < 13)) q[i] = q0[i];
+    T vv[NV];
+#pragma unroll
+    for (int i = 0; i < NV; i++) vv[i] = vs[i];
+    integrate_pos_lin(q, vv, h);
+    T qh[4];
+    integrate_quat_half(q0 + half_quat(hi), vs + half_vang(hi), h, qh);
+    T* qo = q + half_quat(hi);
+#pragma unroll
+    for (int i = 0; i < 4; i++) qo[i] = qh[i];
+    team_sync();
+    return iters;
+  }
+#endif
 #pragma unroll
   for (int i = 0; i < NQ; i++) q[i] = q0[i];
   T vv[NV];
@@ -326,6 +423,7 @@
   StageOut<T>& so = W.so;
   bool acc_reset = false;
   int it = rk4_step<T, BODY, FUSE>(m, q, v, warm, ctrl, tr, W, so, tm, &acc_reset);
+  BB_PRE(11)
   if (it < 0) return F_SLOWPATH;
   if (iters) *iters = it;
   if (acc_reset) flags |= F_DIVERGED;
diff --git a/openballbot-rl_amd/csrc/bb_team16.h b/openballbot-rl_amd/csrc/bb_team16.h
--- a/openballbot-rl_amd/csrc/bb_team16.h
+++ b/openballbot-rl_amd/csrc/bb_team16.h
@@ -438,7 +438,12 @@
   const bool rowl = tl < NV;
   const int row = rowl ? tl : NV - 1;
   const T muw = m.fr_wheel[0];
-  const T kdw = T(1) / (muw * muw * (1 + muw * muw));
+  T kdw;
+#if BB_ONCE
+  if constexpr (FUSE) kdw = once_of(m).kdw;
+  else
+#endif
+    kdw = once_kdw(m);
   const T qfs_i = W.qfs[row];
   const int gcol = row - 9;
   static_assert(offsetof(typename EnvWork<T>::U, hes.hg) == offsetof(typename EnvWork<T>::U, hes.wf) + 9 * sizeof(T),
@@ -1052,7 +1057,8 @@
 
 template <typename T>
 __device__ __forceinline__ int collide_team(const ModelT<T>& m, const Kin<T>& k, const T* v, const float* hf,
-                                            T size_z, T* g, int* overflow, int tl) {
+                                            T size_z, T* g, int* overflow, int tl,
+                                            const ModelOnce<T>* mo = nullptr) {
   const T r = m.ball_r;
   const T* c = k.c;
   const T sx = m.hf_sx, sy = m.hf_sy, zb = m.hf_bottom;
@@ -1070,7 +1076,9 @@
   const int ncol = cmax - cmin + 1;
   const int np = 2 * ncol - 2;
   const int total = (rmax - rmin) * (np > 0 ? np : 0);
-  const T dx = 2 * sx / N1, dy = 2 * sy / N1;
+  T dx, dy;
+  if (mo) { dx = mo->dx; dy = mo->dy; }
+  else once_pitch(m, dx, dy);
   (void)v;
   const int team_shift = team_shift_of(L);
   int ng = 0;
@@ -1180,7 +1188,8 @@
 }
 
 template <typename T>
-__device__ bool body_candidates(const ModelT<T>& m, const Kin<T>& k, const float* hf, T size_z, T hz, int tl) {
+__device__ bool body_candidates(const ModelT<T>& m, const Kin<T>& k, const float* hf, T size_z, T hz, int tl,
+                                const ModelOnce<T>* mo = nullptr) {
   bool cand = false;
   bool reach = false;
   if (tl < 6) {
@@ -1228,7 +1237,9 @@
       cmin = cmin < 0 ? 0 : cmin; cmax = cmax > N1 ? N1 : cmax;
       rmin = rmin < 0 ? 0 : rmin; rmax = rmax > N1 ? N1 : rmax;
       if (rmax <= rmin || cmax <= cmin) continue;
-      const T dx = 2 * sx / N1, dy = 2 * sy / N1;
+      T dx, dy;
+      if (mo) { dx = mo->dx; dy = mo->dy; }
+      else once_pitch(m, dx, dy);
       const int nc = cmax - cmin, total = (rmax - rmin) * nc;
       for (int i = tl; i < total && !cand; i += L) {
         const int ri = rmin + i / nc, ci = cmin + i % nc;
@@ -1276,7 +1287,8 @@
   if (hf) {
     const T sx = m.hf_sx, sy = m.hf_sy, zb = m.hf_bottom;
     const int N1 = HF_N - 1;
-    const T dx = 2 * sx / N1, dy = 2 * sy / N1;
+    T dx, dy;
+    once_pitch(m, dx, dy);
     int nc = 0;
     int pair_n[6] = {0, 0, 0, 0, 0, 0};
     auto vertices = [&](int rr, int p, T (&V)[3][3]) {
```

After: 13.60 million, median of 6. +1.5%, better.
